# csmile-1006/ARP

Measured on AMD Instinct MI355X. Metric: frames/sec CLIP reward-labelled (256x256 ViT-B/32), higher is better.
Workload: dtype f16; 1 GPU; CLIP ViT-B/32 reward labelling, batch 1024 synthetic 256x256x3 uint8 frames per GPU resident in HBM (BASELINE.json configs[1]), random-init weights, text tower cached; parallelism=shard1 (no collective), streams_per_gpu=2

## Files before the change

arp_amd/_ffi.py:

```python
import ctypes as C
import os

_HERE = os.path.dirname(os.path.abspath(__file__))
LIB_PATH = os.path.join(_HERE, "libarp_hip.so")
if os.environ.get("ARP_LIB"):
    LIB_PATH = os.environ["ARP_LIB"] if os.path.isabs(os.environ["ARP_LIB"]) else os.path.join(os.path.dirname(_HERE), os.environ["ARP_LIB"])

MODE_F32, MODE_BF16, MODE_F16, MODE_F16X3, MODE_F16C = 0, 1, 2, 3, 4
ACT_NONE, ACT_QGELU, ACT_RELU, ACT_TANH, ACT_GELU_TANH = 0, 1, 2, 3, 4
ATTN_OUT_PLAIN, ATTN_OUT_E4M3, ATTN_OUT_F16C, ATTN_OUT_SPLIT3 = 0, 1, 2, 3
LN_OUT_F32, LN_OUT_BF16, LN_OUT_F16, LN_OUT_E4M3, LN_OUT_SPLIT3, LN_OUT_F16C, LN_OUT_F16C2 = 0, 1, 2, 3, 4, 5, 6
ASM_LNPRE, ASM_LAT_LN1, ASM_LAT_STATS = 0, 1, 2


class ArpError(RuntimeError):
    pass


class ClipCfg(C.Structure):
    _fields_ = [(n, C.c_int32) for n in (
        "patch", "width", "layers", "heads", "embed", "img_res", "txt_width", "txt_layers", "txt_heads", "ctx",
        "vocab", "mode", "device", "max_batch", "attn_impl", "n_streams")]


class DtCfg(C.Structure):
    _fields_ = [(n, C.c_int32) for n in (
        "emb", "depth", "heads", "mlp_ratio", "n_actions", "window", "enc_tokens", "enc_dim", "use_adapter", "mode",
        "device", "world", "rank")] + [(n, C.c_float) for n in ("lambda_ret", "weight_decay", "clip_norm", "b1", "b2", "eps")] + [("alibi_bias", C.c_int32), ("model", C.c_int32)]


DT_MODELS = {"ARPDT": 0, "BC": 1}


class FtCfg(C.Structure):
    _fields_ = [(n, C.c_int32) for n in ("layers", "width_v", "width_t", "embed", "hidden", "n_actions", "mode", "device", "use_vip", "use_id")] + [
        (n, C.c_float) for n in ("gamma", "logit_scale", "weight_decay", "b1", "b2", "eps")] + [("goal_conditioned", C.c_int32)]


class GemmSite(C.Structure):
    _fields_ = [("name", C.c_char_p)] + [(n, C.c_int32) for n in ("mode", "force", "M", "N", "K", "lda", "ldr", "ldo")] + [
        (n, C.c_void_p) for n in ("A", "W", "bias", "resid", "out", "ln_stats", "ln_c")] + [("ln_parts", C.c_int32), ("ln_eps", C.c_float)] + [
        ("xb_out", C.c_void_p), ("ldxb", C.c_int32), ("split3", C.c_int32), ("stats_out", C.c_void_p)] + [
        (n, C.c_int32) for n in ("plan", "sd", "sw")] + [("x4_out", C.c_void_p), ("dx4_out", C.c_void_p), ("ld4", C.c_int32)]


class EncCfg(C.Structure):
    _fields_ = [(n, C.c_int32) for n in ("patch", "width", "layers", "heads", "mlp_ratio", "img_res", "mode", "device", "max_frames",
                                          "attn_impl")]


os.environ.setdefault("GPU_MAX_HW_QUEUES", "8")


def _load():
    if not os.path.exists(LIB_PATH):
        raise ImportError(
            f"{LIB_PATH} is missing: the HIP extension is not built. Run `make -C arp_amd/csrc` "
            "(or `python -c 'import __graft_entry__ as g; g.build()'`). There is no CPU fallback.")
    return C.CDLL(LIB_PATH, mode=C.RTLD_GLOBAL)


lib = _load()

_vp, _i, _f = C.c_void_p, C.c_int, C.c_float
_fp = C.POINTER(C.c_float)
_u8p = C.POINTER(C.c_uint8)
_i32p = C.POINTER(C.c_int32)
_i64p = C.POINTER(C.c_int64)

SIGNATURES = {
    "arp_last_error": (C.c_char_p, []),
    "arp_version": (_i, []),
    "arp_debug_live": (_i, [_i64p]),
    "arp_device_count": (_i, []),
    "arp_dev_malloc": (_i, [C.POINTER(_vp), C.c_size_t]),
    "arp_dev_free": (_i, [_vp]),
    "arp_memcpy_h2d": (_i, [_vp, _vp, C.c_size_t]),
    "arp_memcpy_d2h": (_i, [_vp, _vp, C.c_size_t]),
    "arp_set_device": (_i, [_i]),
    "arp_dev_synchronize": (_i, []),
    "arp_host_register": (_i, [_vp, C.c_size_t]),
    "arp_host_unregister": (_i, [_vp]),
    "arp_clip_create": (_i, [C.POINTER(ClipCfg), C.POINTER(_vp)]),
    "arp_clip_destroy": (_i, [_vp]),
    "arp_clip_load_weight": (_i, [_vp, C.c_char_p, _fp, _i64p, _i]),
    "arp_clip_set_fp8_mlp": (_i, [_vp, _i]),
    "arp_clip_finalize_weights": (_i, [_vp]),
    "arp_clip_set_text": (_i, [_vp, _i32p, _i]),
    "arp_clip_get_text_features": (_i, [_vp, _fp]),
    "arp_clip_label": (_i, [_vp, _u8p, _i, _i, _i, _i, _fp]),
    "arp_clip_label_submit": (_i, [_vp, _i, _u8p, _i, _i, _i, _i]),
    "arp_clip_label_collect": (_i, [_vp, _i, _fp]),
    "arp_clip_label_dev_async": (_i, [_vp, _vp, _i, _i, _i, _i, _vp]),
    "arp_clip_sync": (_i, [_vp]),
    "arp_clip_set_streams": (_i, [_vp, _i]),
    "arp_clip_encode_image": (_i, [_vp, _u8p, _i, _i, _i, _i, _i, _fp]),
    "arp_preprocess": (_i, [_u8p, _i, _i, _i, _i, _i, _fp]),
    "arp_bicubic_coeffs": (_i, [_i, _i, _i32p, _i32p, _i32p, _i]),
    "arp_clip_clock_probe": (_i, [_vp, _i]),
    "arp_clip_clock_read": (_i, [_vp, C.POINTER(C.c_double)]),
    "arp_clip_profile_enable": (_i, [_vp, _i]),
    "arp_clip_profile_reset": (_i, [_vp]),
    "arp_clip_profile_json": (_i, [_vp, C.c_char_p, _i]),
    "arp_event_create": (_i, [C.POINTER(_vp)]),
    "arp_event_destroy": (_i, [_vp]),
    "arp_clip_event_record": (_i, [_vp, _vp]),
    "arp_event_elapsed_ms": (_i, [_vp, _vp, _fp]),
    "arp_dt_create": (_i, [C.POINTER(DtCfg), C.POINTER(_vp)]),
    "arp_dt_destroy": (_i, [_vp]),
    "arp_dt_num_params": (_i, [_vp, _i64p, _i32p]),
    "arp_dt_param_info": (_i, [_vp, _i, C.c_char_p, _i, _i64p, _i32p]),
    "arp_dt_set_tensor": (_i, [_vp, C.c_char_p, _i, _fp]),
    "arp_dt_get_tensor": (_i, [_vp, C.c_char_p, _i, _fp]),
    "arp_dt_set_step": (_i, [_vp, C.c_int64]),
    "arp_dt_get_step": (_i, [_vp, _i64p]),
    "arp_dt_set_batch": (_i, [_vp, _fp, _i32p, _fp, _i]),
    "arp_dt_forward": (_i, [_vp, _fp, _fp, _fp]),
    "arp_dt_backward": (_i, [_vp]),
    "arp_dt_train_step": (_i, [_vp, _f, _fp]),
    "arp_dt_train_step_async": (_i, [_vp, _f]),
    "arp_dt_val_step": (_i, [_vp, _fp]),
    "arp_dt_upload_batch_async": (_i, [_vp, _i, _fp, _i32p, _fp, _i]),
    "arp_dt_upload_batch_images_async": (_i, [_vp, _i, _fp, _i32p, _fp, _i]),
    "arp_dt_select_batch": (_i, [_vp, _i]),
    "arp_dt_bucket_plan": (_i, [C.POINTER(DtCfg), _i64p, _i64p]),
    "arp_dt_sync": (_i, [_vp]),
    "arp_dt_event_record": (_i, [_vp, _vp]),
    "arp_dt_comm_unique_id": (_i, [_vp]),
    "arp_dt_comm_init": (_i, [_vp, _vp, _i, _i]),
    "arp_dt_broadcast_state": (_i, [_vp]),
    "arp_dt_set_adapter_corrections": (_i, [_vp, _i]),
    "arp_dt_debug_read": (C.c_int64, [_vp, C.c_char_p, _vp, C.c_int64]),
    "arp_dt_comm_info": (_i, [_vp, _i32p]),
    "arp_dt_comm_selfcheck": (_i, [_vp, C.POINTER(C.c_double)]),
    "arp_dt_profile_enable": (_i, [_vp, _i]),
    "arp_dt_profile_reset": (_i, [_vp]),
    "arp_dt_profile_json": (_i, [_vp, C.c_char_p, _i]),
    "arp_clip_encode_image_multiscale": (_i, [_vp, _u8p, _i, _i, _i, _fp, _fp]),
    "arp_clip_encode_image_multiscale_pil": (_i, [_vp, _u8p, _i, _i, _i, _i, _fp, _fp]),
    "arp_clip_set_prompt_reduce": (_i, [_vp, _i]),
    "arp_clip_encode_text_multiscale": (_i, [_vp, _i32p, _i, _fp, _fp]),
    "arp_clip_encode_image_multiscale_dev": (_i, [_vp, _u8p, _i, _i, _i, _vp, _vp]),
    "arp_clip_encode_text_multiscale_dev": (_i, [_vp, _i32p, _i, _vp, _vp]),
    "arp_ft_set_batch_dev": (_i, [_vp, _vp, _vp, _vp, _vp, _fp, _i32p, _i]),
    "arp_ft_create": (_i, [C.POINTER(FtCfg), C.POINTER(_vp)]),
    "arp_ft_destroy": (_i, [_vp]),
    "arp_ft_num_params": (_i, [_vp, _i64p, _i32p]),
    "arp_ft_param_info": (_i, [_vp, _i, C.c_char_p, _i, _i64p, _i32p]),
    "arp_ft_set_tensor": (_i, [_vp, C.c_char_p, _i, _fp]),
    "arp_ft_get_tensor": (_i, [_vp, C.c_char_p, _i, _fp]),
    "arp_ft_set_step": (_i, [_vp, C.c_int64]),
    "arp_ft_get_step": (_i, [_vp, _i64p]),
    "arp_ft_dropped_gradients": (_i, [_vp, C.POINTER(C.c_uint64)]),
    "arp_ft_set_batch": (_i, [_vp, _fp, _fp, _fp, _fp, _fp, _i32p, _i]),
    "arp_ft_forward": (_i, [_vp, _fp, _fp, _fp]),
    "arp_ft_encode": (_i, [_vp, _i, _fp, _fp, _i, _fp]),
    "arp_ft_reward_set_text": (_i, [_vp, _vp, _i32p, _i]),
    "arp_ft_reward_set_reduce": (_i, [_vp, _i]),
    "arp_ft_reward_dev_async": (_i, [_vp, _vp, _vp, _i, _i, _i, _i, _i, _vp]),
    "arp_ft_reward": (_i, [_vp, _vp, _u8p, _i, _i, _i, _i, _i, _fp]),
    "arp_ft_reward_set_rows": (_i, [_vp, _i]),
    "arp_ft_reward_stats": (_i, [_vp, _i64p]),
    "arp_op_ft_rows_gemm": (_i, [_i, _i, _fp, _i, _fp, _i, _fp, _fp, _i, _i, _i, _i, _i, _i, _i]),
    "arp_op_ft_reward":(_i, [_fp, _fp, _f, _fp, _i, _i, _f, _fp, _i, _i]),
    "arp_ft_backward": (_i, [_vp]),
# ... 107 lines not shown
```

arp_amd/csrc/arp_clip.hip:

```cpp
#include <algorithm>
#include <cmath>
#include <cstdio>
#include <cstdlib>
#include <cstring>
#include <map>
#include <memory>
#include <string>
#include <vector>

#include "../../include/arp_hip.h"
#include "attention.h"
#include "enc_internal.h"
#include "common.h"
#include "gemm.h"
#include "gemm256.h"
#include "clip_internal.h"
#include "tower.h"
#include "preprocess.h"
#include "preprocess_host.h"
#include "rowops.h"
#include "runtime.h"

namespace arp {

static thread_local std::string g_err;
void set_error(const std::string& msg) { g_err = msg; }
int fail(const std::string& msg) {
    g_err = msg;
    return -1;
}

struct HostTensor {
    std::vector<float> data;
    std::vector<int64_t> shape;
};

}

using namespace arp;

struct ClipModel {
    arp_clip_cfg cfg;
    bool finalized = false;

    TowerW vis, txt;
    void* conv_w = nullptr;
    float *cls = nullptr, *pos = nullptr, *lnpre_w = nullptr, *lnpre_b = nullptr, *lnpost_w = nullptr, *lnpost_b = nullptr;
    void* proj_t = nullptr;
    float *tok_emb = nullptr, *tpos = nullptr, *lnf_w = nullptr, *lnf_b = nullptr;
    void* tproj_t = nullptr;
    TowerW txt32;
    void* tproj_t32 = nullptr;
    float* lut = nullptr;

    int gemm_force = 0;
    bool ln_fold = false;
    bool fp8_mlp = false;
    bool fp8_attn = false;
    bool qkv_fused = true;
    bool cls_only_last = true;
    bool lat_fold = true;
    bool skinny = true;
    int lat_rows = 1024;
    bool lat_graph = true;
    bool lat_pinned = true;

    int ntok() const { return (cfg.img_res / cfg.patch) * (cfg.img_res / cfg.patch) + 1; }
    size_t esz() const { return cfg.mode == ARP_MODE_F32 ? 4 : 2; }
};

struct arp_clip : ClipModel {
    Stream stream;
    std::map<std::string, HostTensor> staged;
    std::vector<DevBuf> owned;

    arp_clip* primary = nullptr;
    arp_clip* shared() { return primary ? primary : this; }
    float logit_scale = 0.f;
    DevBuf txt_feat;
    int n_prompts = 0;
    DevBuf txt_mean;
    int prompt_reduce = 0;
    DevBuf clock_buf;
    unsigned long long* clock_acc = nullptr;
    std::map<long long, std::unique_ptr<ResizePlan>> plans;

    DevBuf ms_keep;
    DevBuf ms_res, crop_buf;
    uint64_t res_gen = 0;

    int ws_frames = 0;
    DevBuf patches, pe, x, h, qkv, ao, fc, cls_h, feat, frames_in, rewards;
    Profiler prof;
    float* ms_out = nullptr;
    int ms_ld = 0;
    const int* ms_rows = nullptr;
    int pre_bilinear = 0;
    std::vector<std::unique_ptr<arp_clip>> siblings;
    Event ev_fork;
    std::vector<Event> ev_join;
    Stream copy_stream;
    std::vector<Event> ev_copy;
    struct LabelSlot {
        DevBuf frames, rewards;
        PinBuf host;
        Event done;
        int n = 0;
        bool busy = false;
    } lslot[2];
    bool shared_chip = false;
    DevBuf stats;
    DevBuf part;
    DevBuf lat_stats;
    bool lat_f0 = false;
    bool lat_h0 = false;
    bool lat_now = false;
    struct LatGraph {
        const uint8_t* frames;
        float* rewards;
        int n, H, W, crop;
        hipGraph_t graph;
        hipGraphExec_t exec;
    };
    std::vector<LatGraph> lat_graphs;
    PinBuf pin_frames, pin_rewards;

    arp_clip() = default;
    explicit arp_clip(const ClipModel& m) : ClipModel(m) {}
};
static_assert(!std::is_copy_constructible_v<arp_clip> && std::is_copy_constructible_v<ClipModel>);

namespace arp {

static TowerCtx ctx_of(arp_clip* c) {
    TowerCtx t;
    t.stream = c->stream;
    t.prof = &c->prof;
    t.attn_impl = c->cfg.attn_impl;
    t.gemm_force = c->gemm_force;
    t.qkv_fused = c->qkv_fused;
    t.shared_chip = c->shared_chip;
    t.clock_acc = c->shared()->clock_acc;
    t.fp8_mlp = c->fp8_mlp; t.fp8_attn = c->fp8_attn;
    t.ms_out = c->ms_out; t.ms_ld = c->ms_ld; t.ms_rows = c->ms_rows;
    t.skinny = c->lat_now; t.h_ready0 = c->lat_now && c->lat_h0; t.lat_stats = c->lat_stats.as<float>(); t.lat_fold0 = c->lat_now && c->lat_f0; t.part = c->part.as<float>(); t.part_floats = c->part.bytes / 4;
    return t;
}

static int upload_f32(arp_clip* c, const std::vector<float>& v, float** out) {
    return upload_owned(c->owned, v.data(), v.size() * 4, std::max<size_t>(v.size() * 4, 16), reinterpret_cast<void**>(out));
}

static int upload_mat(arp_clip* c, const float* src, int rows, int cols, bool transpose, void** out, int wmode = -1) {
    const int mode = wmode >= 0 ? wmode : c->cfg.mode;
    const size_t esz = mode == ARP_MODE_F32 ? 4 : 2;
    const size_t n = (size_t)rows * cols;
    std::vector<float> tmp;
    const float* s = src;
    if (transpose) {
        tmp.resize(n);
        for (int r = 0; r < rows; ++r)
            for (int q = 0; q < cols; ++q) tmp[(size_t)q * rows + r] = src[(size_t)r * cols + q];
        s = tmp.data();
    }
    const size_t alloc = std::max<size_t>(n * esz, 16);
    if (mode == ARP_MODE_BF16) {
        std::vector<bf16_t> hb(n);
        for (size_t i = 0; i < n; ++i) hb[i] = host_f2bf(s[i]);
        return upload_owned(c->owned, hb.data(), n * 2, alloc, out);
    }
    if (mode == ARP_MODE_F16) {
        std::vector<f16_t> hb(n);
        for (size_t i = 0; i < n; ++i) hb[i] = host_f2h(s[i]);
        return upload_owned(c->owned, hb.data(), n * 2, alloc, out);
    }
    return upload_owned(c->owned, s, n * 4, alloc, out);
}

static int get_staged(arp_clip* c, const std::string& name, std::vector<int64_t> shape, const HostTensor** out) {
    auto it = c->staged.find(name);
    if (it == c->staged.end()) return fail("missing weight: " + name);
    if (it->second.shape != shape) {
        std::string s = "weight " + name + " has shape [";
        for (auto d : it->second.shape) s += std::to_string(d) + ",";
        s += "], expected [";
        for (auto d : shape) s += std::to_string(d) + ",";
        return fail(s + "]");
    }
    *out = &it->second;
    return 0;
}

static int load_tower(arp_clip* c, const std::string& prefix, int d, int layers, int heads, TowerW& tw, bool fold, int wmode = -1, int ntok = 0) {
    tw.width = d; tw.layers = layers; tw.heads = heads;
    const int emode = wmode >= 0 ? wmode : c->cfg.mode;
    const bool hm = c->qkv_fused && ntok > 0 && qkv_attn_supported(ntok, d, heads, emode == ARP_MODE_F32 ? 4 : 2);
    tw.L.resize(layers);
    for (int i = 0; i < layers; ++i) {
        const std::string p = prefix + "resblocks." + std::to_string(i) + ".";
        LayerW& L = tw.L[i];
        const HostTensor* t;
        ARP_TRY(get_staged(c, p + "ln_1.weight", {d}, &t)); ARP_TRY(upload_f32(c, t->data, &L.ln1_w));
        ARP_TRY(get_staged(c, p + "ln_1.bias", {d}, &t)); ARP_TRY(upload_f32(c, t->data, &L.ln1_b));
        ARP_TRY(get_staged(c, p + "ln_2.weight", {d}, &t)); ARP_TRY(upload_f32(c, t->data, &L.ln2_w));
        ARP_TRY(get_staged(c, p + "ln_2.bias", {d}, &t)); ARP_TRY(upload_f32(c, t->data, &L.ln2_b));
        ARP_TRY(get_staged(c, p + "attn.in_proj_weight", {3 * d, d}, &t)); ARP_TRY(upload_mat(c, t->data.data(), 3 * d, d, false, &L.w_in, wmode));
        ARP_TRY(get_staged(c, p + "attn.in_proj_bias", {3 * d}, &t)); ARP_TRY(upload_f32(c, t->data, &L.b_in));
        if (hm) {
            const HostTensor *w, *b;
            ARP_TRY(get_staged(c, p + "attn.in_proj_weight", {3 * d, d}, &w)); ARP_TRY(get_staged(c, p + "attn.in_proj_bias", {3 * d}, &b));
            std::vector<float> wp((size_t)3 * d * d), bp((size_t)3 * d);
            qkv_head_major(w->data.data(), b->data.data(), d, heads, wp.data(), bp.data());
            ARP_TRY(upload_mat(c, wp.data(), 3 * d, d, false, &L.w_in_hm, wmode)); ARP_TRY(upload_f32(c, bp, &L.b_in_hm));
        }
        ARP_TRY(get_staged(c, p + "attn.out_proj.weight", {d, d}, &t)); ARP_TRY(upload_mat(c, t->data.data(), d, d, false, &L.w_out, wmode));
        ARP_TRY(get_staged(c, p + "attn.out_proj.bias", {d}, &t)); ARP_TRY(upload_f32(c, t->data, &L.b_out));
        ARP_TRY(get_staged(c, p + "mlp.c_fc.weight", {4 * d, d}, &t)); ARP_TRY(upload_mat(c, t->data.data(), 4 * d, d, false, &L.w_fc, wmode));
        ARP_TRY(get_staged(c, p + "mlp.c_fc.bias", {4 * d}, &t)); ARP_TRY(upload_f32(c, t->data, &L.b_fc));
        ARP_TRY(get_staged(c, p + "mlp.c_proj.weight", {d, 4 * d}, &t)); ARP_TRY(upload_mat(c, t->data.data(), d, 4 * d, false, &L.w_proj, wmode));
        ARP_TRY(get_staged(c, p + "mlp.c_proj.bias", {d}, &t)); ARP_TRY(upload_f32(c, t->data, &L.b_proj));
        if (c->fp8_mlp && ntok > 0 && emode != ARP_MODE_F32 && d % 128 == 0) {
            auto put8 = [&](const std::vector<float>& w, void** out, float* scale) -> int {
                float mx = 0.f;
                for (float v : w) mx = std::max(mx, fabsf(v));
                const float sc = mx > 0.f ? exp2f(floorf(log2f(240.f / mx))) : 1.f;
                std::vector<fp8_t> q(w.size());
                for (size_t i = 0; i < w.size(); ++i) q[i] = host_f2fp8(w[i] * sc);
                *scale = sc;
                return upload_owned(c->owned, q.data(), q.size(), q.size(), out);
            };
            const HostTensor *w1, *w2, *lw, *lb;
            float s1 = 1.f, s2 = 1.f;
            ARP_TRY(get_staged(c, p + "mlp.c_fc.weight", {4 * d, d}, &w1)); ARP_TRY(put8(w1->data, &L.w_fc8, &s1));
            ARP_TRY(get_staged(c, p + "mlp.c_proj.weight", {d, 4 * d}, &w2)); ARP_TRY(put8(w2->data, &L.w_proj8, &s2));
            L.a_fc = 1.0f / (FP8_S_H * s1);
            L.a_proj = 1.0f / (FP8_S_G * s2);
            ARP_TRY(get_staged(c, p + "ln_2.weight", {d}, &lw)); ARP_TRY(get_staged(c, p + "ln_2.bias", {d}, &lb));
            std::vector<float> g8(lw->data), b8(lb->data);
            for (auto& v : g8) v *= FP8_S_H;
            for (auto& v : b8) v *= FP8_S_H;
            ARP_TRY(upload_f32(c, g8, &L.ln2_w8)); ARP_TRY(upload_f32(c, b8, &L.ln2_b8));
            if (c->fp8_attn) {
                const HostTensor *wi, *wo;
                float si = 1.f, so = 1.f;
                ARP_TRY(get_staged(c, p + "attn.in_proj_weight", {3 * d, d}, &wi)); ARP_TRY(put8(wi->data, &L.w_in8, &si));
                ARP_TRY(get_staged(c, p + "attn.out_proj.weight", {d, d}, &wo)); ARP_TRY(put8(wo->data, &L.w_out8, &so));
                L.a_in = 1.0f / (FP8_S_H * si);
                L.a_out = 1.0f / (FP8_S_A * so);
                ARP_TRY(get_staged(c, p + "ln_1.weight", {d}, &lw)); ARP_TRY(get_staged(c, p + "ln_1.bias", {d}, &lb));
                std::vector<float> g1(lw->data), b1(lb->data);
                for (auto& v : g1) v *= FP8_S_H;
                for (auto& v : b1) v *= FP8_S_H;
                ARP_TRY(upload_f32(c, g1, &L.ln1_w8)); ARP_TRY(upload_f32(c, b1, &L.ln1_b8));
            }
        }
        if (fold) {
            const HostTensor *w, *b, *lw, *lb;
            std::vector<bf16_t> wf;
            std::vector<float> cc, dd;
            auto put = [&](const std::vector<bf16_t>& m, void** out) -> int {
                return upload_owned(c->owned, m.data(), m.size() * 2, m.size() * 2, out);
            };
            ARP_TRY(get_staged(c, p + "attn.in_proj_weight", {3 * d, d}, &w)); ARP_TRY(get_staged(c, p + "attn.in_proj_bias", {3 * d}, &b));
            ARP_TRY(get_staged(c, p + "ln_1.weight", {d}, &lw)); ARP_TRY(get_staged(c, p + "ln_1.bias", {d}, &lb));
            fold_layernorm(w->data.data(), lw->data.data(), lb->data.data(), b->data.data(), 3 * d, d, wf, cc, dd, emode == ARP_MODE_F16);
            ARP_TRY(put(wf, &L.w_in_f)); ARP_TRY(upload_f32(c, cc, &L.c_in)); ARP_TRY(upload_f32(c, dd, &L.d_in));
            ARP_TRY(get_staged(c, p + "mlp.c_fc.weight", {4 * d, d}, &w)); ARP_TRY(get_staged(c, p + "mlp.c_fc.bias", {4 * d}, &b));
            ARP_TRY(get_staged(c, p + "ln_2.weight", {d}, &lw)); ARP_TRY(get_staged(c, p + "ln_2.bias", {d}, &lb));
            fold_layernorm(w->data.data(), lw->data.data(), lb->data.data(), b->data.data(), 4 * d, d, wf, cc, dd, emode == ARP_MODE_F16);
            ARP_TRY(put(wf, &L.w_fc_f)); ARP_TRY(upload_f32(c, cc, &L.c_fc)); ARP_TRY(upload_f32(c, dd, &L.d_fc));
        }
    }
    tw.folded = fold;
    if (!fold && ntok > 0 && c->lat_fold && c->skinny && emode != ARP_MODE_F32 && (d & 15) == 0) {
        for (int i = 0; i < layers; ++i) {
            LayerW& L = tw.L[i];
            const std::string p = prefix + "resblocks." + std::to_string(i) + ".";
            const HostTensor *w, *b, *lw, *lb;
            std::vector<bf16_t> wf;
            std::vector<float> cc, dd;
            auto put = [&](const std::vector<bf16_t>& m, void** out) -> int {
                return upload_owned(c->owned, m.data(), m.size() * 2, m.size() * 2, out);
            };
            const bool half = emode == ARP_MODE_F16;
            ARP_TRY(get_staged(c, p + "attn.in_proj_weight", {3 * d, d}, &w)); ARP_TRY(get_staged(c, p + "attn.in_proj_bias", {3 * d}, &b));
            ARP_TRY(get_staged(c, p + "ln_1.weight", {d}, &lw)); ARP_TRY(get_staged(c, p + "ln_1.bias", {d}, &lb));
            fold_layernorm(w->data.data(), lw->data.data(), lb->data.data(), b->data.data(), 3 * d, d, wf, cc, dd, half);
            ARP_TRY(put(wf, &L.w_in_f)); ARP_TRY(upload_f32(c, cc, &L.c_in)); ARP_TRY(upload_f32(c, dd, &L.d_in));
            ARP_TRY(get_staged(c, p + "mlp.c_fc.weight", {4 * d, d}, &w)); ARP_TRY(get_staged(c, p + "mlp.c_fc.bias", {4 * d}, &b));
            ARP_TRY(get_staged(c, p + "ln_2.weight", {d}, &lw)); ARP_TRY(get_staged(c, p + "ln_2.bias", {d}, &lb));
            fold_layernorm(w->data.data(), lw->data.data(), lb->data.data(), b->data.data(), 4 * d, d, wf, cc, dd, half);
            ARP_TRY(put(wf, &L.w_fc_f)); ARP_TRY(upload_f32(c, cc, &L.c_fc)); ARP_TRY(upload_f32(c, dd, &L.d_fc));
        }
        tw.lat_folded = true;
    }
    return 0;
}

template <typename T, typename OutT, int ACT, bool RESID, int SITE>
static int gemm(arp_clip* c, const char* site, const void* A, const void* W, const float* bias, const float* resid, void* out,
                int M, int N, int K) {
    TowerCtx t = ctx_of(c);
    return tower_gemm<T, OutT, ACT, RESID, SITE>(t, site, A, W, bias, resid, out, M, N, K);
}
template <typename OutT>
static int layernorm(arp_clip* c, const char* site, const float* in, size_t in_stride, OutT* out, int out_stride,
                     const float* w, const float* b, int rows, int D, float eps) {
    TowerCtx t = ctx_of(c);
    return tower_layernorm<OutT>(t, site, in, in_stride, out, out_stride, w, b, rows, D, eps);
}
template <typename T>
static int run_blocks(arp_clip* c, const TowerW& tw, const char* tag, float* x, T* h, T* qkv, T* ao, T* fc, int B, int N,
                      int causal, float* stats = nullptr) {
    TowerCtx t = ctx_of(c);
    t.cls_only_last = (&tw == &c->vis) && c->cls_only_last && !(t.ms_out && t.ms_rows);
    return run_blocks<T, ACT_QGELU, 0>(t, tw, tag, x, h, qkv, ao, fc, B, N, causal, 1e-5f, stats);
}


static void drop_lat_graphs(arp_clip* c) {
    for (auto& g : c->lat_graphs) {
        (void)hipGraphExecDestroy(g.exec);
        (void)hipGraphDestroy(g.graph);
    }
    c->lat_graphs.clear();
}

static int ensure_workspace(arp_clip* c, int frames) {
    if (frames <= c->ws_frames) return 0;
    if (!c->lat_graphs.empty()) {
        ARP_HIP_OK(hipStreamSynchronize(c->stream));
        drop_lat_graphs(c);
    }
    const arp_clip_cfg& k = c->cfg;
    const size_t e = c->esz();
    const int G = k.img_res / k.patch, N = c->ntok(), D = k.width;
    const size_t B = frames, M = B * N;
    ARP_TRY(c->patches.ensure(B * G * G * 3 * k.patch * k.patch * e));
    ARP_TRY(c->pe.ensure(B * G * G * D * 4));
    ARP_TRY(c->x.ensure(M * D * 4));
    ARP_TRY(c->h.ensure(M * D * e));
    ARP_TRY(c->qkv.ensure(M * 3 * D * e));
    ARP_TRY(c->ao.ensure(M * D * e));
    ARP_TRY(c->fc.ensure(M * 4 * D * e));
    ARP_TRY(c->cls_h.ensure(B * D * e));
    ARP_TRY(c->feat.ensure(B * k.embed * 4));
    ARP_TRY(c->stats.ensure(M * (size_t)std::max(D >> 7, 1) * 8));
    c->ws_frames = frames;
    c->res_gen += 1;
    return 0;
}

static int get_plan(arp_clip* c, int H, int W, int use_crop, ResizePlan** out, bool small = false) {
    const long long key = ((long long)H << 32) | ((long long)W << 2) | (small ? 2 : 0) | (use_crop ? 1 : 0);
    auto it = c->plans.find(key);
    if (it != c->plans.end()) {
        *out = it->second.get();
        return 0;
    }
    auto p = std::make_unique<ResizePlan>();
    ARP_TRY(build_plan(H, W, use_crop, c->cfg.img_res, *p, small ? 8 : 32));
    *out = p.get();
    c->plans[key] = std::move(p);
    return 0;
}

template <typename T>
static int forward_chunk(arp_clip* c, const uint8_t* frames_dev, int nb, ResizePlan* plan) {
    const arp_clip_cfg& k = c->cfg;
    const int G = k.img_res / k.patch, N = c->ntok(), D = k.width, KP = 3 * k.patch * k.patch;
    c->lat_now = c->skinny && sizeof(T) == 2 && (long)nb * N <= c->lat_rows;
    struct LatGuard {
        arp_clip* c;
        ~LatGuard() { c->lat_now = false; c->lat_h0 = false; c->lat_f0 = false; }
    } lat_guard{c};
    if (c->pre_bilinear) {
        ProfScope ps(c->prof, c->stream, "preprocess_bilinear");
        const int H = c->pre_bilinear >> 16, W = c->pre_bilinear & 0xffff, R = k.img_res;
        const size_t total = (size_t)nb * 3 * R * (R / 4);
        hipLaunchKernelGGL((preprocess_bilinear_kernel<T>), dim3((unsigned)((total + 255) / 256)), dim3(256), 0, c->stream, frames_dev, c->patches.as<T>(), nb,
                           H, W, R, k.patch, (H != R && W != R) ? 1 : 0);
        ARP_HIP_OK(hipGetLastError());
    } else {
        ProfScope ps(c->prof, c->stream, "preprocess");
        ARP_TRY((launch_preprocess<T, PRE_PATCH>(*plan, frames_dev, nb, k.patch, c->lut, c->patches.p, c->stream)));
    }
    c->lat_h0 = false;
    c->lat_f0 = false;
    bool assembled = false;
    if constexpr (sizeof(T) == 2) {
        const int Mp = nb * G * G, S = c->lat_now ? tower_split_of(Mp, D, KP) : 0;
        if (S && (size_t)S * Mp * D * 4 <= c->part.bytes && c->vis.layers > 0 && D % 4 == 0 && D <= ROW_MAX_V4 * 256) {
            const int tcode = __is_same(T, bf16_t) ? 1 : 2;
            SkinnyArgs q;
            q.A = c->patches.p; q.W = c->conv_w; q.out = c->part.p; q.M = Mp; q.N = D; q.K = KP; q.lda = KP; q.ldw = KP; q.ldo = D; q.out_f32 = 1;
            q.ksplit = S; q.slice_stride = (size_t)Mp * D;
            {
                ProfScope ps(c->prof, c->stream, "vit.patch_embed");
                ARP_TRY(launch_skinny_gemm(tcode, q, c->stream));
            }
            ProfScope ps(c->prof, c->stream, "vit.assemble_ln_pre_ln_1");
            const bool f0 = c->vis.lat_folded && c->lat_stats.p && (D & 15) == 0;
            ARP_TRY(launch_vit_assemble_lat<T>(c->stream, c->part.as<float>(), S, (size_t)Mp * D, c->cls, c->pos, c->lnpre_w, c->lnpre_b, c->x.as<float>(),
                                               c->h.as<T>(), c->vis.L[0].ln1_w, c->vis.L[0].ln1_b, nb * N, N, D, 1e-5f,
                                               f0 ? c->lat_stats.as<float>() : nullptr, D >> 4));
            assembled = true;
            c->lat_h0 = !f0;
            c->lat_f0 = f0;
        }
    }
    if (!assembled) {
    ARP_TRY((gemm<T, float, ACT_NONE, false, SITE_PATCH>(c, "vit.patch_embed", c->patches.p, c->conv_w, nullptr, nullptr, c->pe.p,
                                                         nb * G * G, D, KP)));
    {
        ProfScope ps(c->prof, c->stream, "vit.assemble_ln_pre");
        ARP_TRY(launch_vit_assemble_lnpre(c->stream, c->pe.as<float>(), c->cls, c->pos, c->lnpre_w, c->lnpre_b, c->x.as<float>(), nb * N, N, D, 1e-5f));
    }
    }
    ARP_TRY(run_blocks<T>(c, c->vis, "vit", c->x.as<float>(), c->h.as<T>(), c->qkv.as<T>(), c->ao.as<T>(), c->fc.as<T>(), nb, N, 0, c->stats.as<float>()));
    ARP_TRY(layernorm<T>(c, "vit.ln_post", c->x.as<float>(), (size_t)N * D, c->cls_h.as<T>(), D, c->lnpost_w, c->lnpost_b, nb, D, 1e-5f));
    ARP_TRY((gemm<T, float, ACT_NONE, false, SITE_PROJ>(c, "vit.proj", c->cls_h.p, c->proj_t, nullptr, nullptr, c->feat.p, nb, k.embed, D)));
    return 0;
}

static int forward_chunk_dispatch(arp_clip* c, const uint8_t* frames_dev, int nb, ResizePlan* plan) {
    if (c->cfg.mode == ARP_MODE_BF16) return forward_chunk<bf16_t>(c, frames_dev, nb, plan);
    if (c->cfg.mode == ARP_MODE_F16) return forward_chunk<f16_t>(c, frames_dev, nb, plan);
    return forward_chunk<float>(c, frames_dev, nb, plan);
}

template <typename T> static int run_text(arp_clip* c, const int32_t* tokens, int np, float* out_host = nullptr, bool normalize = true,
                                          float* ms_host = nullptr, bool dev_out = false, bool w32 = false) {
    const TowerW& txt = w32 ? c->txt32 : c->txt;
    const void* tproj = w32 ? c->tproj_t32 : c->tproj_t;
    const arp_clip_cfg& k = c->cfg;
    const int Tw = k.txt_width, ctx = k.ctx, M = np * ctx;
    const size_t e = sizeof(T);
    DevBuf tok, eot, x, h, qkv, ao, fc, hs, ms, feat_tmp;
    DevBuf& feat = out_host ? feat_tmp : c->txt_feat;
    std::vector<int> eot_rows(np);
    for (int p = 0; p < np; ++p) {
        int best = 0;
        for (int t = 1; t < ctx; ++t)
            if (tokens[p * ctx + t] > tokens[p * ctx + best]) best = t;
        eot_rows[p] = p * ctx + best;
        for (int t = 0; t < ctx; ++t)
            if (tokens[p * ctx + t] < 0 || tokens[p * ctx + t] >= k.vocab) return fail("set_text: token id out of range");
    }
    ARP_TRY(tok.ensure((size_t)M * 4)); ARP_TRY(eot.ensure((size_t)np * 4));
    ARP_TRY(x.ensure((size_t)M * Tw * 4)); ARP_TRY(h.ensure((size_t)M * Tw * e)); ARP_TRY(qkv.ensure((size_t)M * 3 * Tw * e));
    ARP_TRY(ao.ensure((size_t)M * Tw * e)); ARP_TRY(fc.ensure((size_t)M * 4 * Tw * e)); ARP_TRY(hs.ensure((size_t)np * Tw * e));
    ARP_TRY(feat.ensure((size_t)np * k.embed * 4));
    if (ms_host) ARP_TRY(ms.ensure((size_t)np * c->txt.layers * Tw * 4));
    ARP_HIP_OK(hipMemcpyAsync(tok.p, tokens, (size_t)M * 4, hipMemcpyHostToDevice, c->stream));
    ARP_HIP_OK(hipMemcpyAsync(eot.p, eot_rows.data(), (size_t)np * 4, hipMemcpyHostToDevice, c->stream));
    ARP_TRY(launch_text_embed(c->stream, tok.as<int>(), c->tok_emb, c->tpos, x.as<float>(), M, ctx, Tw));
    if (ms_host) { c->ms_out = ms.as<float>(); c->ms_ld = c->txt.layers * Tw; c->ms_rows = eot.as<int>(); }
    const int rb = run_blocks<T>(c, txt, "text", x.as<float>(), h.as<T>(), qkv.as<T>(), ao.as<T>(), fc.as<T>(), np, ctx, 1);
    c->ms_out = nullptr; c->ms_rows = nullptr;
    ARP_TRY(rb);
    ARP_TRY(launch_layernorm_gather<T>(c->stream, x.as<float>(), (size_t)Tw, eot.as<int>(), hs.as<T>(), Tw, c->lnf_w, c->lnf_b, np, Tw, 1e-5f));
    ARP_TRY((gemm<T, float, ACT_NONE, false, SITE_PROJ>(c, "text.proj", hs.p, tproj, nullptr, nullptr, feat.p, np,
                                                        k.embed, Tw)));
    if (normalize) {
        ARP_TRY(launch_l2_normalize(c->stream, feat.as<float>(), np, k.embed));
    }
    const hipMemcpyKind okind = dev_out ? hipMemcpyDeviceToDevice : hipMemcpyDeviceToHost;
    if (out_host) ARP_HIP_OK(hipMemcpyAsync(out_host, feat.p, (size_t)np * k.embed * 4, okind, c->stream));
    if (ms_host) ARP_HIP_OK(hipMemcpyAsync(ms_host, ms.p, (size_t)np * c->txt.layers * Tw * 4, okind, c->stream));
    ARP_HIP_OK(hipStreamSynchronize(c->stream));
    if (!out_host) c->n_prompts = np;
    return 0;
}

static int check_ready(arp_clip* c, bool need_text) {
    if (!c) return fail("null handle");
    if (!c->finalized) return fail("weights not finalized: call arp_clip_finalize_weights first");
    if (need_text && c->n_prompts <= 0) return fail("no prompt set: call arp_clip_set_text first");
    return 0;
}

static int label_dev_single(arp_clip* c, const uint8_t* frames_dev, int n, int H, int W, int use_crop, float* rewards_dev) {
    arp_clip* o = c->shared();
    ARP_TRY(check_ready(o, true));
    if (n < 0) return fail("negative frame count");
    if (n == 0) return 0;
    ARP_HIP_OK(hipSetDevice(c->cfg.device));
    ResizePlan* plan;
    const int mb = c->cfg.max_batch;
    const bool small = !c->primary && n <= mb && (long)n * c->ntok() <= c->lat_rows;
    ARP_TRY(get_plan(o, H, W, use_crop, &plan, small));
    ARP_TRY(ensure_workspace(c, std::min(n, mb)));
    const float scale = expf(o->logit_scale);
    auto pass = [&](const uint8_t* fr, int nb, float* rw) -> int {
        ARP_TRY(forward_chunk_dispatch(c, fr, nb, plan));
        ProfScope ps(c->prof, c->stream, "reward");
        return launch_reward(c->stream, c->feat.as<float>(), o->prompt_reduce ? o->txt_mean.as<float>() : o->txt_feat.as<float>(), scale, rw, nb, c->cfg.embed);
    };
    if (c->lat_graph && small && !c->prof.on && !c->ms_out && !c->pre_bilinear) {
        for (auto& g : c->lat_graphs)
            if (g.frames == frames_dev && g.rewards == rewards_dev && g.n == n && g.H == H && g.W == W && g.crop == ((use_crop ? 1 : 0) | (c->prompt_reduce << 1))) {
                ARP_HIP_OK(hipGraphLaunch(g.exec, c->stream));
                return 0;
            }
        arp_clip::LatGraph g{frames_dev, rewards_dev, n, H, W, (use_crop ? 1 : 0) | (c->prompt_reduce << 1), nullptr, nullptr};
        ARP_HIP_OK(hipStreamBeginCapture(c->stream, hipStreamCaptureModeRelaxed));
        const int rc = pass(frames_dev, n, rewards_dev);
        const hipError_t ec = hipStreamEndCapture(c->stream, &g.graph);
        if (rc != 0 || ec != hipSuccess || !g.graph || hipGraphInstantiate(&g.exec, g.graph, nullptr, nullptr, 0) != hipSuccess) {
            if (g.graph) (void)hipGraphDestroy(g.graph);
            for (int k = 0; k < 4 && hipGetLastError() != hipSuccess; ++k) {}
            c->lat_graph = false;
            return pass(frames_dev, n, rewards_dev);
        }
        if (c->lat_graphs.size() >= 8) {
            (void)hipGraphExecDestroy(c->lat_graphs.front().exec);
            (void)hipGraphDestroy(c->lat_graphs.front().graph);
            c->lat_graphs.erase(c->lat_graphs.begin());
        }
        c->lat_graphs.push_back(g);
        ARP_HIP_OK(hipGraphLaunch(g.exec, c->stream));
        return 0;
    }
    for (int off = 0; off < n; off += mb) {
        const int nb = std::min(mb, n - off);
        ARP_TRY(pass(frames_dev + (size_t)off * H * W * 3, nb, rewards_dev + off));
    }
    return 0;
}

static int make_sibling(arp_clip* c) {
    auto s = std::make_unique<arp_clip>(static_cast<const ClipModel&>(*c));
    s->primary = c;
    s->prof.on = c->prof.on;
    ARP_TRY(s->stream.create());
    if (!c->ev_fork) ARP_TRY(c->ev_fork.create());
    Event ej;
    ARP_TRY(ej.create());
    c->ev_join.push_back(std::move(ej));
    c->siblings.push_back(std::move(s));
    return 0;
}

static int label_dev(arp_clip* c, const uint8_t* frames_dev, int n, int H, int W, int use_crop, float* rewards_dev, const uint8_t* host_src = nullptr,
                     int lead = 0) {
    ARP_TRY(check_ready(c, true));
    int ns = c->cfg.n_streams;
    while (ns > 1 && n / ns < 128) --ns;
    const size_t fbytes = (size_t)H * W * 3;
    if (ns < 2) {
        if (host_src) ARP_HIP_OK(hipMemcpyAsync(const_cast<uint8_t*>(frames_dev), host_src, (size_t)n * fbytes, hipMemcpyHostToDevice, c->stream));
        return label_dev_single(c, frames_dev, n, H, W, use_crop, rewards_dev);
    }
    ARP_HIP_OK(hipSetDevice(c->cfg.device));
    int parts = ns;
    if (host_src) {
        static const int env_parts = getenv("ARP_CLIP_HOST_PARTS") ? atoi(getenv("ARP_CLIP_HOST_PARTS")) : 0;
        parts = env_parts > 0 ? env_parts : ns;
        while (parts > ns && n / parts < 128) --parts;
        if (parts < ns) parts = ns;
        if (!c->copy_stream) ARP_TRY(c->copy_stream.create());
        while ((int)c->ev_copy.size() < parts + 1) {
            Event e;
            ARP_TRY(e.create());
            c->ev_copy.push_back(std::move(e));
        }
    }
    while ((int)c->siblings.size() < ns - 1) ARP_TRY(make_sibling(c));
    ResizePlan* plan;
    ARP_TRY(get_plan(c, H, W, use_crop, &plan));
    ARP_HIP_OK(hipEventRecord(c->ev_fork, c->stream));
    for (int i = 1; i < ns; ++i) ARP_HIP_OK(hipStreamWaitEvent(c->siblings[i - 1]->stream, c->ev_fork, 0));
    if (!host_src || lead <= 0 || n < 8 * lead) lead = 0;
    const int per = (n - lead + parts - 1) / parts;
// ... 45 lines not shown
}

static int ms_finetune_geometry(const arp_clip* c, int H, int W, int use_crop, int* h, int* w, int* y0, int* x0) {
    const int R = c->cfg.img_res;
    *h = H; *w = W; *y0 = 0; *x0 = 0;
    if (use_crop) {
        const int cs = W / 2;
        if (cs <= 0 || cs > H) return fail("use_crop: the centre crop of side W / 2 does not fit the frame");
        *h = *w = cs;
        *y0 = (int)((H - cs) / 2); *x0 = (int)((W - cs) / 2);
    }
    if ((*h != R) != (*w != R)) return fail("the reference resizes only when BOTH sides differ from 224 (clip_multiscale_adapter.py:127): "
                                            "a frame with exactly one side at 224 cannot enter the tower");
    return 0;
}

int clip_ms_prepare(arp_clip* c, int nb, int H, int W, int use_crop, int transform, uint64_t* generation, int* capturable) {
    ARP_TRY(check_ready(c, false));
    if (c->primary) return fail("a part stream's sibling is not a handle of its own");
    if (nb <= 0 || nb > c->cfg.max_batch) return fail("clip_ms_prepare: 1 .. max_batch frames per pass");
    if (H <= 0 || W <= 0 || H > 0xffff || W > 0xffff) return fail("bad frame geometry");
    if (transform != CLIP_TF_FINETUNE && transform != CLIP_TF_LABEL) return fail("transform is 0 (fine-tune: bilinear) or 1 (label: Pillow bicubic)");
    ARP_HIP_OK(hipSetDevice(c->cfg.device));
    const bool small = (long)nb * c->ntok() <= c->lat_rows;
    size_t crop_bytes = 0;
    if (transform == CLIP_TF_LABEL) {
        ResizePlan* plan;
        ARP_TRY(get_plan(c, H, W, use_crop, &plan, small));
    } else {
        int h, w, y0, x0;
        ARP_TRY(ms_finetune_geometry(c, H, W, use_crop, &h, &w, &y0, &x0));
        if (use_crop) crop_bytes = (size_t)nb * h * w * 3;
    }
    const size_t ms_bytes = (size_t)nb * c->vis.layers * c->cfg.width * 4;
    if (ms_bytes > c->ms_res.bytes || crop_bytes > c->crop_buf.bytes) {
        ARP_HIP_OK(hipStreamSynchronize(c->stream));
        ARP_TRY(c->ms_res.ensure(ms_bytes));
        ARP_TRY(c->crop_buf.ensure(crop_bytes));
        c->res_gen += 1;
    }
    ARP_TRY(ensure_workspace(c, nb));
    *generation = c->res_gen;
    *capturable = c->lat_graph && small && !c->prof.on ? 1 : 0;
    return 0;
}

int clip_ms_enqueue(arp_clip* c, const uint8_t* frames_dev, int nb, int H, int W, int use_crop, int transform, const float** inter, const float** final_feat) {
    if (!c || !frames_dev || !inter || !final_feat) return fail("null argument");
    if (nb <= 0 || nb > c->ws_frames || (size_t)nb * c->vis.layers * c->cfg.width * 4 > c->ms_res.bytes) return fail("clip_ms_enqueue: call clip_ms_prepare first");
    ResizePlan* plan = nullptr;
    const uint8_t* src = frames_dev;
    int pre = 0;
    if (transform == CLIP_TF_LABEL) {
        ARP_TRY(get_plan(c, H, W, use_crop, &plan, (long)nb * c->ntok() <= c->lat_rows));
    } else {
        int h, w, y0, x0;
        ARP_TRY(ms_finetune_geometry(c, H, W, use_crop, &h, &w, &y0, &x0));
        if (use_crop) {
            const size_t total = (size_t)nb * h * w * 3;
            if (total > c->crop_buf.bytes) return fail("clip_ms_enqueue: call clip_ms_prepare first");
            ProfScope ps(c->prof, c->stream, "crop");
            hipLaunchKernelGGL(crop_u8_kernel, dim3((unsigned)std::min<size_t>((total + 255) / 256, 4096)), dim3(256), 0, c->stream, frames_dev,
                               c->crop_buf.as<uint8_t>(), nb, H, W, y0, x0, h);
            ARP_HIP_OK(hipGetLastError());
            src = c->crop_buf.as<uint8_t>();
        }
        pre = (h << 16) | w;
    }
    c->ms_out = c->ms_res.as<float>(); c->ms_ld = c->vis.layers * c->cfg.width; c->ms_rows = nullptr; c->pre_bilinear = pre;
    const int r = forward_chunk_dispatch(c, src, nb, plan);
    c->ms_out = nullptr; c->pre_bilinear = 0;
    ARP_TRY(r);
    *inter = c->ms_res.as<float>();
    *final_feat = c->feat.as<float>();
    return 0;
}

}

extern "C" {

const char* arp_last_error(void) { return g_err.c_str(); }
int arp_version(void) { return 100; }

int arp_debug_live(int64_t out5[5]) {
    if (!out5) return fail("null out");
    out5[0] = live.dev_bytes; out5[1] = live.dev_bufs; out5[2] = live.streams; out5[3] = live.events; out5[4] = live.pin_bytes;
    return 0;
}

int arp_device_count(void) {
    int n = 0;
    if (hipGetDeviceCount(&n) != hipSuccess) return 0;
    return n;
}

int arp_dev_malloc(void** out, size_t bytes) {
    if (!out) return fail("null out");
    ARP_HIP_OK(hipMalloc(out, bytes ? bytes : 16));
    return 0;
}
int arp_dev_free(void* p) {
    if (p) ARP_HIP_OK(hipFree(p));
    return 0;
}
int arp_memcpy_h2d(void* dst, const void* src, size_t bytes) {
    ARP_HIP_OK(hipMemcpy(dst, src, bytes, hipMemcpyHostToDevice));
    return 0;
}
int arp_memcpy_d2h(void* dst, const void* src, size_t bytes) {
    ARP_HIP_OK(hipMemcpy(dst, src, bytes, hipMemcpyDeviceToHost));
    return 0;
}
int arp_host_register(void* p, size_t bytes) {
    if (!p || !bytes) return fail("bad argument");
    ARP_HIP_OK(hipHostRegister(p, bytes, hipHostRegisterDefault));
    return 0;
}
int arp_host_unregister(void* p) {
    if (!p) return 0;
    ARP_HIP_OK(hipHostUnregister(p));
    return 0;
}
int arp_set_device(int device) {
    ARP_HIP_OK(hipSetDevice(device));
    return 0;
}
int arp_dev_synchronize(void) {
    ARP_HIP_OK(hipDeviceSynchronize());
    return 0;
}

int arp_clip_create(const arp_clip_cfg* cfg, arp_clip** out) {
    if (!cfg || !out) return fail("null argument");
    const arp_clip_cfg& k = *cfg;
    if (k.mode != ARP_MODE_F32 && k.mode != ARP_MODE_BF16 && k.mode != ARP_MODE_F16) return fail("bad mode");
    if (k.patch <= 0 || k.img_res % k.patch || k.patch % 4 || k.img_res % 4) return fail("bad patch / img_res");
    if (k.width % k.heads || k.txt_width % k.txt_heads) return fail("width not divisible by heads");
    const int kq = (k.mode == ARP_MODE_F32) ? 32 : 64;
    if (k.width % kq || k.txt_width % kq || (3 * k.patch * k.patch) % kq)
        return fail("width / txt_width / 3*patch^2 must be multiples of " + std::to_string(kq));
    if (k.embed % 4) return fail("embed must be a multiple of 4");
    int ndev = 0;
    ARP_HIP_OK(hipGetDeviceCount(&ndev));
    if (k.device < 0 || k.device >= ndev) return fail("no such HIP device: " + std::to_string(k.device));
    ARP_HIP_OK(hipSetDevice(k.device));
    ARP_TRY(prime_runtime(k.device));
    arp_clip* c = new arp_clip();
    c->cfg = k;
    if (c->cfg.max_batch <= 0) c->cfg.max_batch = 1024;
    if (const char* e = getenv("ARP_GEMM")) c->gemm_force = atoi(e);
    if (const char* e = getenv("ARP_LN_FOLD")) c->ln_fold = atoi(e) != 0;
    if (const char* e = getenv("ARP_CLS_ONLY")) c->cls_only_last = atoi(e) != 0;
    if (const char* e = getenv("ARP_QKV_FUSED")) c->qkv_fused = atoi(e) != 0;
    if (const char* e = getenv("ARP_SKINNY")) c->skinny = atoi(e) != 0;
    if (const char* e = getenv("ARP_LAT_FOLD")) c->lat_fold = atoi(e) != 0;
    if (const char* e = getenv("ARP_CLIP_GRAPH")) c->lat_graph = atoi(e) != 0;
    if (const char* e = getenv("ARP_SKINNY_ROWS")) c->lat_rows = std::min(std::max(atoi(e), 1), SKINNY_MAX_M);
    if (const char* e = getenv("ARP_CLIP_PINNED")) c->lat_pinned = atoi(e) != 0;
    if (c->stream.create() != 0) {
        delete c;
        return fail("hipStreamCreate failed");
    }
    *out = c;
    return 0;
}

int arp_clip_destroy(arp_clip* c) {
    if (!c) return 0;
    (void)hipSetDevice(c->cfg.device);
    (void)hipStreamSynchronize(c->stream);
    for (auto& s : c->siblings) (void)hipStreamSynchronize(s->stream);
    drop_lat_graphs(c);
    delete c;
    return 0;
}

int arp_clip_load_weight(arp_clip* c, const char* name, const float* data, const int64_t* shape, int ndim) {
    if (!c || !name || !data || (ndim > 0 && !shape)) return fail("null argument");
    if (c->finalized) return fail("weights already finalized");
    HostTensor t;
    size_t n = 1;
    for (int i = 0; i < ndim; ++i) {
        if (shape[i] < 0) return fail("negative dimension");
        t.shape.push_back(shape[i]);
        n *= (size_t)shape[i];
    }
    t.data.assign(data, data + n);
    c->staged[name] = std::move(t);
    return 0;
}

int arp_clip_finalize_weights(arp_clip* c) {
    if (!c) return fail("null handle");
    if (c->finalized) return 0;
    ARP_HIP_OK(hipSetDevice(c->cfg.device));
    const arp_clip_cfg& k = c->cfg;
    const int D = k.width, P = k.patch, E = k.embed, Tw = k.txt_width, N = c->ntok();
    const HostTensor* t;
    ARP_TRY(get_staged(c, "visual.conv1.weight", {D, 3, P, P}, &t)); ARP_TRY(upload_mat(c, t->data.data(), D, 3 * P * P, false, &c->conv_w));
    ARP_TRY(get_staged(c, "visual.class_embedding", {D}, &t)); ARP_TRY(upload_f32(c, t->data, &c->cls));
    ARP_TRY(get_staged(c, "visual.positional_embedding", {N, D}, &t)); ARP_TRY(upload_f32(c, t->data, &c->pos));
    ARP_TRY(get_staged(c, "visual.ln_pre.weight", {D}, &t)); ARP_TRY(upload_f32(c, t->data, &c->lnpre_w));
    ARP_TRY(get_staged(c, "visual.ln_pre.bias", {D}, &t)); ARP_TRY(upload_f32(c, t->data, &c->lnpre_b));
    ARP_TRY(get_staged(c, "visual.ln_post.weight", {D}, &t)); ARP_TRY(upload_f32(c, t->data, &c->lnpost_w));
    ARP_TRY(get_staged(c, "visual.ln_post.bias", {D}, &t)); ARP_TRY(upload_f32(c, t->data, &c->lnpost_b));
    ARP_TRY(get_staged(c, "visual.proj", {D, E}, &t)); ARP_TRY(upload_mat(c, t->data.data(), D, E, true, &c->proj_t));
    ARP_TRY(load_tower(c, "visual.transformer.", D, k.layers, k.heads, c->vis, c->ln_fold && (k.mode == ARP_MODE_BF16 || k.mode == ARP_MODE_F16) && (D & 127) == 0, -1, c->ntok()));
    ARP_TRY(get_staged(c, "token_embedding.weight", {k.vocab, Tw}, &t)); ARP_TRY(upload_f32(c, t->data, &c->tok_emb));
    ARP_TRY(get_staged(c, "positional_embedding", {k.ctx, Tw}, &t)); ARP_TRY(upload_f32(c, t->data, &c->tpos));
    ARP_TRY(get_staged(c, "ln_final.weight", {Tw}, &t)); ARP_TRY(upload_f32(c, t->data, &c->lnf_w));
    ARP_TRY(get_staged(c, "ln_final.bias", {Tw}, &t)); ARP_TRY(upload_f32(c, t->data, &c->lnf_b));
    ARP_TRY(get_staged(c, "text_projection", {Tw, E}, &t)); ARP_TRY(upload_mat(c, t->data.data(), Tw, E, true, &c->tproj_t));
    ARP_TRY(load_tower(c, "transformer.", Tw, k.txt_layers, k.txt_heads, c->txt, false));
    if (k.mode != ARP_MODE_F32) {
        ARP_TRY(get_staged(c, "text_projection", {Tw, E}, &t)); ARP_TRY(upload_mat(c, t->data.data(), Tw, E, true, &c->tproj_t32, ARP_MODE_F32));
        ARP_TRY(load_tower(c, "transformer.", Tw, k.txt_layers, k.txt_heads, c->txt32, false, ARP_MODE_F32));
    }
    if (c->staged.count("logit_scale") && c->staged["logit_scale"].shape == std::vector<int64_t>{1}) c->staged["logit_scale"].shape.clear();
    ARP_TRY(get_staged(c, "logit_scale", {}, &t));
    c->logit_scale = t->data[0];
    std::vector<float> lut(768);
    build_lut(lut.data());
    ARP_TRY(upload_f32(c, lut, &c->lut));
    ARP_TRY(c->part.ensure((size_t)4 * SKINNY_MAX_M * std::max(D, Tw) * 4));
    ARP_TRY(c->lat_stats.ensure((size_t)SKINNY_MAX_M * std::max(D >> 4, 1) * 8));
    c->staged.clear();
    c->finalized = true;
    return 0;
}

static __global__ __launch_bounds__(256) void prompt_mean_kernel(const float* __restrict__ txt, float* __restrict__ out, int np, int E) {
    const int c = blockIdx.x * 256 + threadIdx.x;
    if (c >= E) return;
    float s = 0.f;
    for (int p = 0; p < np; ++p) s += txt[(size_t)p * E + c];
    out[c] = s / (float)np;
}

int arp_clip_set_text(arp_clip* c, const int32_t* tokens, int n_prompts) {
    ARP_TRY(check_ready(c, false));
    if (!tokens || n_prompts <= 0) return fail("set_text: need at least one prompt");
    ARP_HIP_OK(hipSetDevice(c->cfg.device));
    if (!c->lat_graphs.empty()) {
        ARP_HIP_OK(hipStreamSynchronize(c->stream));
        drop_lat_graphs(c);
    }
    if (c->cfg.mode != ARP_MODE_F32) ARP_TRY(run_text<float>(c, tokens, n_prompts, nullptr, true, nullptr, false, true));
    else ARP_TRY(run_text<float>(c, tokens, n_prompts));
    ARP_TRY(c->txt_mean.ensure((size_t)c->cfg.embed * 4));
    hipLaunchKernelGGL(prompt_mean_kernel, dim3((c->cfg.embed + 255) / 256), dim3(256), 0, c->stream, c->txt_feat.as<float>(), c->txt_mean.as<float>(),
                       n_prompts, c->cfg.embed);
    ARP_HIP_OK(hipGetLastError());
    ARP_HIP_OK(hipStreamSynchronize(c->stream));
    return 0;
}

int arp_clip_set_prompt_reduce(arp_clip* c, int mode) {
    ARP_TRY(check_ready(c, false));
    if (mode != 0 && mode != 1) return fail("set_prompt_reduce: mode is 0 (prompt 0) or 1 (mean over the prompts)");
    c->prompt_reduce = mode;
    return 0;
}

int arp_clip_get_text_features(arp_clip* c, float* out) {
    ARP_TRY(check_ready(c, true));
    if (!out) return fail("null out");
    ARP_HIP_OK(hipMemcpy(out, c->txt_feat.p, (size_t)c->n_prompts * c->cfg.embed * 4, hipMemcpyDeviceToHost));
    return 0;
}

int arp_clip_label_dev_async(arp_clip* c, const uint8_t* frames_dev, int n, int H, int W, int use_crop, float* rewards_dev) {
    if (n > 0 && (!frames_dev || !rewards_dev)) return fail("null buffer");
    return label_dev(c, frames_dev, n, H, W, use_crop, rewards_dev);
}

int arp_clip_sync(arp_clip* c) {
    if (!c) return fail("null handle");
    ARP_HIP_OK(hipStreamSynchronize(c->stream));
    return 0;
}

int arp_clip_label(arp_clip* c, const uint8_t* frames, int n, int H, int W, int use_crop, float* rewards) {
    ARP_TRY(check_ready(c, true));
    if (n < 0) return fail("negative frame count");
    if (n == 0) return 0;
    if (!frames || !rewards) return fail("null buffer");
    ARP_HIP_OK(hipSetDevice(c->cfg.device));
    const size_t fb = (size_t)H * W * 3;
    const int mb = c->cfg.max_batch;
    if (c->lat_pinned && n <= mb && (long)n * c->ntok() <= c->lat_rows) {
        if (c->pin_frames.bytes < (size_t)n * fb) {
            ARP_HIP_OK(hipStreamSynchronize(c->stream));
            ARP_TRY(c->pin_frames.ensure((size_t)n * fb));
        }
        if (c->pin_rewards.bytes < (size_t)n * 4) {
            ARP_HIP_OK(hipStreamSynchronize(c->stream));
            ARP_TRY(c->pin_rewards.ensure((size_t)std::max(n, 16) * 4));
        }
        memcpy(c->pin_frames.p, frames, (size_t)n * fb);
        ARP_TRY(label_dev_single(c, c->pin_frames.as<uint8_t>(), n, H, W, use_crop, c->pin_rewards.as<float>()));
        ARP_HIP_OK(hipStreamSynchronize(c->stream));
        memcpy(rewards, c->pin_rewards.p, (size_t)n * 4);
        return 0;
    }
    ARP_TRY(c->frames_in.ensure((size_t)std::min(n, mb) * fb));
// ... 228 lines not shown
    }
    const std::string s = c->prof.json();
    if ((int)s.size() + 1 > buf_len) return fail("profile buffer too small");
    memcpy(buf, s.c_str(), s.size() + 1);
    return (int)s.size();
}

int arp_event_create(arp_event** out) {
    if (!out) return fail("null out");
    arp_event* ev = new arp_event();
    if (hipEventCreate(&ev->e) != hipSuccess) {
        delete ev;
        return fail("hipEventCreate failed");
    }
    *out = ev;
    return 0;
}
int arp_event_destroy(arp_event* e) {
    if (e) {
        (void)hipEventDestroy(e->e);
        delete e;
    }
    return 0;
}
int arp_clip_event_record(arp_clip* c, arp_event* e) {
    if (!c || !e) return fail("null argument");
    ARP_HIP_OK(hipEventRecord(e->e, c->stream));
    return 0;
}
int arp_event_elapsed_ms(arp_event* a, arp_event* b, float* ms) {
    if (!a || !b || !ms) return fail("null argument");
    ARP_HIP_OK(hipEventSynchronize(b->e));
    ARP_HIP_OK(hipEventElapsedTime(ms, a->e, b->e));
    return 0;
}

}

template <typename T> static int to_dev(const float* src, size_t n, DevBuf& d) {
    ARP_TRY(d.ensure(std::max<size_t>(n * sizeof(T), 16)));
    if constexpr (std::is_same_v<T, f16_t>) {
        std::vector<f16_t> hb(n);
        for (size_t i = 0; i < n; ++i) hb[i] = host_f2h(src[i]);
        ARP_HIP_OK(hipMemcpy(d.p, hb.data(), n * 2, hipMemcpyHostToDevice));
    } else if constexpr (sizeof(T) == 2) {
        std::vector<bf16_t> hb(n);
        for (size_t i = 0; i < n; ++i) hb[i] = host_f2bf(src[i]);
        ARP_HIP_OK(hipMemcpy(d.p, hb.data(), n * 2, hipMemcpyHostToDevice));
    } else {
        ARP_HIP_OK(hipMemcpy(d.p, src, n * 4, hipMemcpyHostToDevice));
    }
    return 0;
}
template <typename T> static int from_dev(float* dst, size_t n, const DevBuf& d) {
    if constexpr (std::is_same_v<T, f16_t>) {
        std::vector<uint16_t> hb(n);
        ARP_HIP_OK(hipMemcpy(hb.data(), d.p, n * 2, hipMemcpyDeviceToHost));
        for (size_t i = 0; i < n; ++i) dst[i] = (float)__builtin_bit_cast(_Float16, hb[i]);
    } else if constexpr (sizeof(T) == 2) {
        std::vector<bf16_t> hb(n);
        ARP_HIP_OK(hipMemcpy(hb.data(), d.p, n * 2, hipMemcpyDeviceToHost));
        for (size_t i = 0; i < n; ++i) {
            const uint32_t u = (uint32_t)hb[i] << 16;
            memcpy(&dst[i], &u, 4);
        }
    } else {
        ARP_HIP_OK(hipMemcpy(dst, d.p, n * 4, hipMemcpyDeviceToHost));
    }
    return 0;
}

template <typename T> static int op_gemm(int act, const float* A, const float* W, const float* bias, const float* resid, float* out,
                                         int M, int N, int K) {
    DevBuf dA, dW, dB, dR, dO;
    ARP_TRY(to_dev<T>(A, (size_t)M * K, dA)); ARP_TRY(to_dev<T>(W, (size_t)N * K, dW));
    if (bias) ARP_TRY(to_dev<float>(bias, N, dB));
    ARP_TRY(dO.ensure((size_t)M * N * 4));
    if (resid) ARP_TRY(to_dev<float>(resid, (size_t)M * N, dR));
    GemmArgs g;
    g.A = dA.p; g.W = dW.p; g.bias = bias ? dB.as<float>() : nullptr; g.resid = resid ? dR.as<float>() : nullptr; g.out = dO.p;
    g.M = M; g.N = N; g.K = K; g.lda = K; g.ldw = K; g.ldr = N; g.ldo = N;
    int rc = -1;
    const char* fe = getenv("ARP_GEMM");
    const int force = fe ? atoi(fe) : 0;
#define ARP_OP_CASE(a)                                                                                            \
case a: rc = resid ? launch_gemm_auto<T, float, a, true, SITE_OP>(g, nullptr, force) : launch_gemm_auto<T, float, a, false, SITE_OP>(g, nullptr, force); break;
    switch (act) {
        ARP_OP_CASE(ACT_NONE) ARP_OP_CASE(ACT_QGELU) ARP_OP_CASE(ACT_RELU) ARP_OP_CASE(ACT_TANH) ARP_OP_CASE(ACT_GELU_TANH)
        default: return fail("bad activation");
    }
#undef ARP_OP_CASE
    ARP_TRY(rc);
    ARP_HIP_OK(hipDeviceSynchronize());
    return from_dev<float>(out, (size_t)M * N, dO);
}

template <typename T> static int op_skinny(int act, const float* A, const float* W, const float* bias, const float* resid, float* out, int M, int N, int K,
                                           int ksplit, const float* ln_w, const float* ln_b, float eps, float* h_out) {
    DevBuf dA, dW, dB, dR, dO, dP, dH, dLw, dLb;
    const int tcode = __is_same(T, bf16_t) ? 1 : 2;
    ARP_TRY(to_dev<T>(A, (size_t)M * K, dA)); ARP_TRY(to_dev<T>(W, (size_t)N * K, dW));
    if (bias) ARP_TRY(to_dev<float>(bias, N, dB));
    SkinnyArgs k;
    k.A = dA.p; k.W = dW.p; k.M = M; k.N = N; k.K = K; k.lda = K; k.ldw = K; k.ldr = N; k.ldo = N; k.out_f32 = 1;
    if (ksplit == 0) {
        ARP_TRY(dO.ensure((size_t)M * N * 4));
        if (resid) ARP_TRY(to_dev<float>(resid, (size_t)M * N, dR));
        k.bias = bias ? dB.as<float>() : nullptr; k.resid = resid ? dR.as<float>() : nullptr; k.out = dO.p; k.act = act;
        ARP_TRY(launch_skinny_gemm(tcode, k, nullptr));
        ARP_HIP_OK(hipDeviceSynchronize());
        return from_dev<float>(out, (size_t)M * N, dO);
    }
    if (!resid || act != ACT_NONE) return fail("skinny split: needs the residual, takes no activation");
    ARP_TRY(to_dev<float>(resid, (size_t)M * N, dR));
    ARP_TRY(dP.ensure((size_t)ksplit * M * N * 4));
    if (ln_w) {
        if (!ln_b || !h_out) return fail("skinny split: ln_w needs ln_b and h_out");
        ARP_TRY(to_dev<float>(ln_w, N, dLw)); ARP_TRY(to_dev<float>(ln_b, N, dLb)); ARP_TRY(dH.ensure((size_t)M * N * sizeof(T)));
    }
    k.out = dP.p; k.ksplit = ksplit; k.slice_stride = (size_t)M * N;
    ARP_TRY(launch_skinny_gemm(tcode, k, nullptr));
    ARP_TRY(launch_skinny_reduce_ln(tcode, dP.as<float>(), ksplit, (size_t)M * N, bias ? dB.as<float>() : nullptr, dR.as<float>(), N, dH.p, N,
                                    ln_w ? dLw.as<float>() : nullptr, ln_w ? dLb.as<float>() : nullptr, M, N, eps, nullptr));
    ARP_HIP_OK(hipDeviceSynchronize());
    ARP_TRY(from_dev<float>(out, (size_t)M * N, dR));
    if (ln_w) ARP_TRY(from_dev<T>(h_out, (size_t)M * N, dH));
    return 0;
}

extern "C" {

int arp_op_skinny_gemm(int mode, int act, const float* A, const float* W, const float* bias, const float* resid, float* out, int M, int N, int K, int ksplit,
                       const float* ln_w, const float* ln_b, float eps, float* h_out) {
    if (!A || !W || !out || M <= 0 || N <= 0 || K <= 0 || ksplit < 0) return fail("bad argument");
    if (mode == ARP_MODE_BF16) return op_skinny<bf16_t>(act, A, W, bias, resid, out, M, N, K, ksplit, ln_w, ln_b, eps, h_out);
    if (mode == ARP_MODE_F16) return op_skinny<f16_t>(act, A, W, bias, resid, out, M, N, K, ksplit, ln_w, ln_b, eps, h_out);
    return fail("skinny gemm: 16-bit modes only");
}

int arp_op_gemm_nt(int mode, int act, const float* A, const float* W, const float* bias, const float* resid, float* out, int M, int N,
                   int K) {
    if (!A || !W || !out || M <= 0 || N <= 0 || K <= 0) return fail("bad argument");
    if (mode == ARP_MODE_F16) return op_gemm<f16_t>(act, A, W, bias, resid, out, M, N, K);
    return mode == ARP_MODE_BF16 ? op_gemm<bf16_t>(act, A, W, bias, resid, out, M, N, K) : op_gemm<float>(act, A, W, bias, resid, out, M, N, K);
}

}

template <typename T> static int op_gemm_site_vit(const arp_gemm_site& d, const std::string& s) {
    if (s == "vit.qkv") return tower_gemm_site<T, T, ACT_NONE, false, SITE_QKV>(d);
    if (s == "vit.c_fc") return tower_gemm_site<T, T, ACT_QGELU, false, SITE_FC1>(d);
    if (s == "vit.out_proj") return tower_gemm_site<T, float, ACT_NONE, true, SITE_OUT>(d);
    if (s == "vit.c_proj") return tower_gemm_site<T, float, ACT_NONE, true, SITE_FC2>(d);
    return fail("gemm_site: unknown instance " + s);
}

extern "C" {

int arp_op_gemm_site(const arp_gemm_site* d) {
    if (!d || !d->name || !d->A || !d->W || d->M <= 0 || d->N <= 0 || d->K <= 0) return fail("bad argument");
    const std::string s(d->name);
    int rc;
    if (s.rfind("m3ae.", 0) == 0) rc = enc_op_gemm_site(*d);
    else if (d->mode == ARP_MODE_F16) rc = op_gemm_site_vit<f16_t>(*d, s);
    else if (d->mode == ARP_MODE_BF16) rc = op_gemm_site_vit<bf16_t>(*d, s);
    else return fail("gemm_site: 16-bit modes only");
    ARP_TRY(rc);
    ARP_HIP_OK(hipDeviceSynchronize());
    return 0;
}

}

static float host_fp82f(uint8_t b) {
    const int sign = b >> 7, e = (b >> 3) & 15, m = b & 7;
    float v;
    if (e == 15 && m == 7) v = NAN;
    else if (e == 0) v = ldexpf((float)m, -9);
    else v = ldexpf(1.0f + m / 8.0f, e - 7);
    return sign ? -v : v;
}

extern "C" {

int arp_op_gemm_fp8(int act, const float* A, const float* W, const float* bias, const float* resid, float* out, int M, int N, int K, float alpha,
                    int out_fp8, float out_scale) {
    if (!A || !W || !out || M <= 0 || N <= 0 || K <= 0 || K % 128 || N % 16) return fail("bad argument (K % 128, N % 16)");
    if (out_fp8 && resid) return fail("fp8 output has no residual epilogue");
    DevBuf dA, dW, dB, dR, dO;
    std::vector<fp8_t> qa((size_t)M * K), qw((size_t)N * K);
    for (size_t i = 0; i < qa.size(); ++i) qa[i] = host_f2fp8(A[i]);
    for (size_t i = 0; i < qw.size(); ++i) qw[i] = host_f2fp8(W[i]);
    ARP_TRY(dA.ensure(qa.size())); ARP_TRY(dW.ensure(qw.size()));
    ARP_HIP_OK(hipMemcpy(dA.p, qa.data(), qa.size(), hipMemcpyHostToDevice));
    ARP_HIP_OK(hipMemcpy(dW.p, qw.data(), qw.size(), hipMemcpyHostToDevice));
    if (bias) ARP_TRY(to_dev<float>(bias, N, dB));
    if (resid) ARP_TRY(to_dev<float>(resid, (size_t)M * N, dR));
    ARP_TRY(dO.ensure((size_t)M * N * 4));
    GemmArgs g;
    g.A = dA.p; g.W = dW.p; g.bias = bias ? dB.as<float>() : nullptr; g.resid = resid ? dR.as<float>() : nullptr; g.out = dO.p;
    g.M = M; g.N = N; g.K = K; g.lda = K; g.ldw = K; g.ldr = N; g.ldo = N; g.alpha = alpha; g.out_scale = out_scale;
    int rc;
    if (out_fp8 == 2) {
        if (act != ACT_NONE || resid) return fail("f16 output: no activation, no residual");
        rc = launch_gemm256_nt<fp8_t, f16_t, ACT_NONE, false, SITE_OP>(g, nullptr);
        ARP_TRY(rc);
        ARP_HIP_OK(hipDeviceSynchronize());
        return from_dev<f16_t>(out, (size_t)M * N, dO);
    }
    if (out_fp8) rc = act == ACT_QGELU ? launch_gemm256_nt<fp8_t, fp8_t, ACT_QGELU, false, SITE_OP>(g, nullptr) : launch_gemm256_nt<fp8_t, fp8_t, ACT_NONE, false, SITE_OP>(g, nullptr);
    else if (act != ACT_NONE) return fail("f32 output: act must be ACT_NONE");
    else rc = resid ? launch_gemm256_nt<fp8_t, float, ACT_NONE, true, SITE_OP>(g, nullptr) : launch_gemm256_nt<fp8_t, float, ACT_NONE, false, SITE_OP>(g, nullptr);
    ARP_TRY(rc);
    ARP_HIP_OK(hipDeviceSynchronize());
    if (out_fp8) {
        std::vector<uint8_t> hb((size_t)M * N);
        ARP_HIP_OK(hipMemcpy(hb.data(), dO.p, hb.size(), hipMemcpyDeviceToHost));
        for (size_t i = 0; i < hb.size(); ++i) out[i] = host_fp82f(hb[i]);
        return 0;
    }
    return from_dev<float>(out, (size_t)M * N, dO);
}

}

template <typename T> static int op_gemm_bench(int kernel, int act, int resid, int out_f32, int M, int N, int K, int iters, float* avg_ms) {
    DevBuf dA, dW, dB, dR, dO;
    Event e0, e1;
    std::vector<float> hA((size_t)M * K), hW((size_t)N * K), hb(N);
    uint32_t s = 12345u;
    auto rnd = [&]() { s = s * 1664525u + 1013904223u; return ((s >> 8) & 0xffff) / 32768.0f - 1.0f; };
    for (auto& v : hA) v = rnd();
    for (auto& v : hW) v = rnd() * 0.05f;
    for (auto& v : hb) v = rnd();
    ARP_TRY(to_dev<T>(hA.data(), hA.size(), dA)); ARP_TRY(to_dev<T>(hW.data(), hW.size(), dW)); ARP_TRY(to_dev<float>(hb.data(), N, dB));
    ARP_TRY(dO.ensure((size_t)M * N * 4)); ARP_TRY(dR.ensure((size_t)M * N * 4));
    ARP_HIP_OK(hipMemset(dR.p, 0, (size_t)M * N * 4));
    GemmArgs g;
    g.A = dA.p; g.W = dW.p; g.bias = dB.as<float>(); g.resid = resid ? dR.as<float>() : nullptr; g.out = resid ? dR.p : dO.p;
    g.M = M; g.N = N; g.K = K; g.lda = K; g.ldw = K; g.ldr = N; g.ldo = N;
    if (const char* fe = getenv("ARP_GEMM_GROUP_M")) g.group_m = atoi(fe);
    auto run = [&]() -> int {
        if (resid) return launch_gemm_auto<T, float, ACT_NONE, true, SITE_OP>(g, nullptr, kernel);
        if (out_f32) return launch_gemm_auto<T, float, ACT_NONE, false, SITE_OP>(g, nullptr, kernel);
        if (act == ACT_QGELU) return launch_gemm_auto<T, T, ACT_QGELU, false, SITE_OP>(g, nullptr, kernel);
        return launch_gemm_auto<T, T, ACT_NONE, false, SITE_OP>(g, nullptr, kernel);
    };
    ARP_TRY(e0.create(hipEventDefault)); ARP_TRY(e1.create(hipEventDefault));
    for (int i = 0; i < 3; ++i) ARP_TRY(run());
    ARP_HIP_OK(hipEventRecord(e0, nullptr));
    for (int i = 0; i < iters; ++i) ARP_TRY(run());
    ARP_HIP_OK(hipEventRecord(e1, nullptr));
    ARP_HIP_OK(hipEventSynchronize(e1));
    float ms = 0.f;
    ARP_HIP_OK(hipEventElapsedTime(&ms, e0, e1));
    *avg_ms = ms / iters;
    return 0;
}

extern "C" {

int arp_op_gemm_bench(int mode, int kernel, int act, int resid, int out_f32, int M, int N, int K, int iters, float* avg_ms) {
    if (!avg_ms || M <= 0 || N <= 0 || K <= 0 || iters <= 0) return fail("bad argument");
    if (mode == ARP_MODE_F16) return op_gemm_bench<f16_t>(kernel, act, resid, out_f32, M, N, K, iters, avg_ms);
    return mode == ARP_MODE_BF16 ? op_gemm_bench<bf16_t>(kernel, act, resid, out_f32, M, N, K, iters, avg_ms)
                                 : op_gemm_bench<float>(kernel, act, resid, out_f32, M, N, K, iters, avg_ms);
}

int arp_op_layernorm(const float* x, const float* w, const float* b, float* out, int rows, int D, float eps) {
    if (!x || !w || !b || !out || rows <= 0 || D <= 0) return fail("bad argument");
    if (D % 4 || D > ROW_MAX_V4 * 256) return fail("layernorm: unsupported width");
    DevBuf dx, dw, db, dout;
    ARP_TRY(to_dev<float>(x, (size_t)rows * D, dx)); ARP_TRY(to_dev<float>(w, D, dw)); ARP_TRY(to_dev<float>(b, D, db));
    ARP_TRY(dout.ensure((size_t)rows * D * 4));
#define ARP_LN_CALL(NV)                                                                                                  \
hipLaunchKernelGGL((layernorm_kernel<float, NV>), dim3((rows + 3) / 4), dim3(256), 0, nullptr, dx.as<float>(), (size_t)D, \
                   dout.as<float>(), D, dw.as<float>(), db.as<float>(), rows, D, eps)
    ARP_NV_DISPATCH(D, ARP_LN_CALL);
#undef ARP_LN_CALL
    ARP_HIP_OK(hipGetLastError());
    ARP_HIP_OK(hipDeviceSynchronize());
    return from_dev<float>(out, (size_t)rows * D, dout);
}

}

template <typename T> static int op_attn(int impl, const float* qkv, float* out, int B, int N, int D, int heads, int causal) {
    DevBuf dq, dout;
    ARP_TRY(to_dev<T>(qkv, (size_t)B * N * 3 * D, dq));
    ARP_TRY(dout.ensure((size_t)B * N * D * sizeof(T)));
    ARP_TRY(launch_attention<T>(nullptr, impl, dq.as<T>(), dout.as<T>(), B, N, D, heads, causal));
    ARP_HIP_OK(hipDeviceSynchronize());
    return from_dev<T>(out, (size_t)B * N * D, dout);
}

extern "C" {

int arp_op_attention(int mode, int impl, const float* qkv, float* out, int B, int N, int D, int heads, int causal) {
    if (!qkv || !out || B <= 0 || N <= 0 || D <= 0 || heads <= 0 || D % heads) return fail("bad argument");
    if (mode == ARP_MODE_F16) return op_attn<f16_t>(impl, qkv, out, B, N, D, heads, causal);
    return mode == ARP_MODE_BF16 ? op_attn<bf16_t>(impl, qkv, out, B, N, D, heads, causal)
                                 : op_attn<float>(impl, qkv, out, B, N, D, heads, causal);
}

}

// ... 39 lines not shown
    DevBuf dA, dW, dB, dout;
    std::vector<float> wp((size_t)3 * D * K), bp((size_t)3 * D);
    qkv_head_major(W, bias, K, heads, wp.data(), bp.data());
    ARP_TRY(to_dev<T>(A, rows * K, dA)); ARP_TRY(to_dev<T>(wp.data(), wp.size(), dW)); ARP_TRY(to_dev<float>(bp.data(), bp.size(), dB));
    ARP_TRY(dout.ensure(std::max<size_t>(out_bytes, 16)));
    ARP_HIP_OK(hipMemcpy(dout.p, out, out_bytes, hipMemcpyHostToDevice));
    QkvAttnArgs q;
    q.A = dA.p; q.W = dW.p; q.bias = dB.as<float>(); q.out = dout.p;
    q.B = B; q.N = N; q.K = K; q.heads = heads; q.lda = K; q.ldw = K; q.ldo = D; q.fpt = 0; q.nq = nq; q.causal = causal; q.scale = 0.f;
    const int rc = launch_qkv_attn<T>(q, nullptr);
    ARP_HIP_OK(hipDeviceSynchronize());
    ARP_HIP_OK(hipMemcpy(out, dout.p, out_bytes, hipMemcpyDeviceToHost));
    return rc;
}

extern "C" {

int arp_op_attention_forms(int mode, int impl, const float* qkv, void* out, size_t out_bytes, int B, int N, int D, int heads, int causal, int nq, int form,
                           float out_scale, int outc) {
    if (!qkv || !out || B <= 0 || N <= 0 || D <= 0 || heads <= 0 || D % heads) return fail("bad argument");
    uint8_t* o = static_cast<uint8_t*>(out);
    if (mode == ARP_MODE_F16) return op_attn_forms<f16_t>(impl, qkv, o, out_bytes, B, N, D, heads, causal, nq, form, out_scale, outc);
    if (mode == ARP_MODE_BF16) return op_attn_forms<bf16_t>(impl, qkv, o, out_bytes, B, N, D, heads, causal, nq, form, out_scale, outc);
    if (mode == ARP_MODE_F32) return op_attn_forms<float>(impl, qkv, o, out_bytes, B, N, D, heads, causal, nq, form, out_scale, outc);
    return fail("attention_forms: mode must be f32, bf16 or f16");
}

int arp_op_qkv_attention(int mode, const float* A, const float* W, const float* bias, void* out, size_t out_bytes, int B, int N, int K, int heads, int causal,
                         int nq) {
    if (!A || !W || !bias || !out || B <= 0 || N <= 0 || K <= 0 || heads <= 0) return fail("bad argument");
    uint8_t* o = static_cast<uint8_t*>(out);
    if (mode == ARP_MODE_F16) return op_qkv_attn<f16_t>(A, W, bias, o, out_bytes, B, N, K, heads, causal, nq);
    if (mode == ARP_MODE_BF16) return op_qkv_attn<bf16_t>(A, W, bias, o, out_bytes, B, N, K, heads, causal, nq);
    return fail("qkv_attention: 16-bit modes only");
}

}

namespace {
struct CallerBuf {
    DevBuf d;
    void* host = nullptr;
    size_t n = 0;
    int up(void* h, size_t bytes) {
        host = h; n = bytes;
        ARP_TRY(d.ensure(std::max<size_t>(bytes, 16)));
        if (bytes) ARP_HIP_OK(hipMemcpy(d.p, h, bytes, hipMemcpyHostToDevice));
        return 0;
    }
    int down() {
        if (n) ARP_HIP_OK(hipMemcpy(host, d.p, n, hipMemcpyDeviceToHost));
        return 0;
    }
};
int up_i32(const int32_t* src, size_t n, DevBuf& d) {
    ARP_TRY(d.ensure(std::max<size_t>(n * 4, 16)));
    ARP_HIP_OK(hipMemcpy(d.p, src, n * 4, hipMemcpyHostToDevice));
    return 0;
}
int finish(int rc, std::initializer_list<CallerBuf*> bufs) {
    const hipError_t e = hipDeviceSynchronize();
    for (CallerBuf* b : bufs) {
        const int r = b->down();
        if (rc == 0 && r != 0) rc = r;
    }
    ARP_TRY(rc);
    ARP_HIP_OK(e);
    return 0;
}

template <typename OutT>
int op_ln_form(const float* x, size_t in_stride, const int* idx, void* out, int out_stride, const float* w, const float* b, int rows, int D, float eps) {
    if (idx) {
        if constexpr (std::is_same_v<OutT, float> || std::is_same_v<OutT, bf16_t> || std::is_same_v<OutT, f16_t>)
            return launch_layernorm_gather<OutT>(nullptr, x, in_stride, idx, static_cast<OutT*>(out), out_stride, w, b, rows, D, eps);
        else
            return fail("layernorm_forms: the gathered kernel is instantiated for the f32, bf16 and binary16 outputs only (run_text)");
    }
    Profiler prof;
    TowerCtx c;
    c.prof = &prof;
    return tower_layernorm<OutT>(c, "op.layernorm", x, in_stride, static_cast<OutT*>(out), out_stride, w, b, rows, D, eps);
}

template <typename T>
int op_assemble_lat(const float* patch, int S, size_t slice_stride, const float* cls, const float* pos, const float* w, const float* b, float* x, void* h,
                    const float* w1, const float* b1, int rows, int ntok, int D, float eps, float* stats) {
    return launch_vit_assemble_lat<T>(nullptr, patch, S, slice_stride, cls, pos, w, b, x, static_cast<T*>(h), w1, b1, rows, ntok, D, eps, stats, D >> 4);
}
}

extern "C" {

int arp_op_layernorm_forms(int form, const float* x, size_t x_floats, size_t in_stride, const int32_t* row_idx, const float* w, const float* b, void* out,
                           size_t out_bytes, int out_stride, int rows, int D, float eps) {
    if (!x || !w || !b || !out || rows <= 0 || D <= 0 || out_stride <= 0) return fail("layernorm_forms: bad argument");
    size_t esz, row_elems;
    switch (form) {
        case ARP_LN_OUT_F32: esz = 4; row_elems = D; break;
        case ARP_LN_OUT_BF16: case ARP_LN_OUT_F16: esz = 2; row_elems = D; break;
        case ARP_LN_OUT_E4M3: esz = 1; row_elems = D; break;
        case ARP_LN_OUT_SPLIT3: esz = 2; row_elems = (size_t)3 * D; break;
        case ARP_LN_OUT_F16C: case ARP_LN_OUT_F16C2: esz = 2; row_elems = (size_t)3 * D / 2; break;
        default: return fail("layernorm_forms: unknown output form");
    }
    if ((form == ARP_LN_OUT_F16C || form == ARP_LN_OUT_F16C2) && D % 256)
        return fail("layernorm_forms: [hi | x4 | dx4] rows feed gemm_c (\"f16c: widths must be multiples of 256\")");
    if (form == ARP_LN_OUT_SPLIT3 && (3 * D) % 64)
        return fail("layernorm_forms: (hi, lo, hi) rows are the A operand of a K = 3 D binary16 product (gemm_nt / gemm256_nt: K % 64 == 0)");
    if ((in_stride & 3) || (out_stride & 3) || in_stride < (size_t)D || (size_t)out_stride < row_elems)
        return fail("layernorm_forms: strides must be multiples of 4 elements and cover a row");
    if (row_idx) {
        for (int r = 0; r < rows; ++r)
            if (row_idx[r] < 0 || (size_t)row_idx[r] * in_stride + D > x_floats) return fail("layernorm_forms: row index outside x");
    } else if ((size_t)(rows - 1) * in_stride + D > x_floats) {
        return fail("layernorm_forms: x shorter than the rows it is read as");
    }
    if (out_bytes < ((size_t)(rows - 1) * out_stride + row_elems) * esz) return fail("layernorm_forms: output buffer shorter than its rows");
    DevBuf dx, dw, db, di;
    CallerBuf o;
    ARP_TRY(to_dev<float>(x, x_floats, dx)); ARP_TRY(to_dev<float>(w, D, dw)); ARP_TRY(to_dev<float>(b, D, db));
    if (row_idx) ARP_TRY(up_i32(row_idx, rows, di));
    ARP_TRY(o.up(out, out_bytes));
    const int* idx = row_idx ? di.as<int>() : nullptr;
    int rc;
#define ARP_LNF_CASE(F, OutT) \
    case F: rc = op_ln_form<OutT>(dx.as<float>(), in_stride, idx, o.d.p, out_stride, dw.as<float>(), db.as<float>(), rows, D, eps); break;
    switch (form) {
        ARP_LNF_CASE(ARP_LN_OUT_F32, float) ARP_LNF_CASE(ARP_LN_OUT_BF16, bf16_t) ARP_LNF_CASE(ARP_LN_OUT_F16, f16_t) ARP_LNF_CASE(ARP_LN_OUT_E4M3, fp8_t)
        ARP_LNF_CASE(ARP_LN_OUT_SPLIT3, f16x3_t) ARP_LNF_CASE(ARP_LN_OUT_F16C, f16c_t)
        default: rc = op_ln_form<f16c2_t>(dx.as<float>(), in_stride, idx, o.d.p, out_stride, dw.as<float>(), db.as<float>(), rows, D, eps); break;
    }
#undef ARP_LNF_CASE
    return finish(rc, {&o});
}

int arp_op_row_stats(int mode, const float* x, void* xb, size_t xb_bytes, void* stats, size_t stats_bytes, int rows, int D) {
    if (!x || !xb || !stats || rows <= 0 || D <= 0) return fail("row_stats: bad argument");
    if (mode != ARP_MODE_BF16 && mode != ARP_MODE_F16) return fail("row_stats: 16-bit modes only");
    if (D & 127) return fail("row_stats: the folded towers need a width that is a multiple of 128 (run_blocks: one (sum, sum of squares) pair per 128 columns)");
    if (xb_bytes < (size_t)rows * D * 2 || stats_bytes < (size_t)rows * (D >> 7) * 8) return fail("row_stats: output buffer too short");
    DevBuf dx;
    CallerBuf b, s;
    ARP_TRY(to_dev<float>(x, (size_t)rows * D, dx));
    ARP_TRY(b.up(xb, xb_bytes)); ARP_TRY(s.up(stats, stats_bytes));
    const int rc = mode == ARP_MODE_BF16 ? launch_row_stats<bf16_t>(nullptr, dx.as<float>(), b.d.as<bf16_t>(), s.d.as<float>(), rows, D)
                                         : launch_row_stats<f16_t>(nullptr, dx.as<float>(), b.d.as<f16_t>(), s.d.as<float>(), rows, D);
    return finish(rc, {&b, &s});
}

int arp_op_vit_assemble(int mode, int tail, const float* patch, size_t patch_floats, int S, size_t slice_stride, const float* cls, size_t cls_floats,
                        const float* pos, const float* w, const float* b, const float* w1, const float* b1, void* x, size_t x_bytes, void* h, size_t h_bytes,
                        void* stats, size_t stats_bytes, int B, int ntok, int D, float eps) {
    if (!patch || !cls || !pos || !w || !b || !x || B <= 0 || ntok <= 0 || D <= 0 || tail < ARP_ASM_LNPRE || tail > ARP_ASM_LAT_STATS)
        return fail("vit_assemble: bad argument");
    const size_t rows = (size_t)B * ntok, prow = (size_t)B * (ntok - 1) * D;
    if (cls_floats < (size_t)D || x_bytes < rows * D * 4) return fail("vit_assemble: cls or x too short");
    DevBuf dp, dc, dpos, dw, db, dw1, db1;
    CallerBuf ox, oh, os;
    if (tail == ARP_ASM_LNPRE) {
        if (patch_floats < prow) return fail("vit_assemble: patch matrix too short");
    } else {
        if (mode != ARP_MODE_BF16 && mode != ARP_MODE_F16) return fail("vit_assemble: the latency kernel exists in the 16-bit modes only");
        if (S >= 1 && patch_floats < (size_t)(S - 1) * slice_stride + prow) return fail("vit_assemble: patch slabs too short");
        if ((slice_stride & 3) && S > 1) return fail("vit_assemble: slab stride must be a multiple of 4 floats");
        if (!h || h_bytes < rows * D * 2) return fail("vit_assemble: h too short");
        if (tail == ARP_ASM_LAT_LN1 && (!w1 || !b1)) return fail("vit_assemble: the ln_1 tail needs w1 and b1");
        if (tail == ARP_ASM_LAT_STATS && (!stats || stats_bytes < rows * (size_t)(D >> 4) * 8)) return fail("vit_assemble: stats too short");
    }
    ARP_TRY(to_dev<float>(patch, patch_floats, dp)); ARP_TRY(to_dev<float>(cls, cls_floats, dc));
    ARP_TRY(to_dev<float>(pos, (size_t)ntok * D, dpos)); ARP_TRY(to_dev<float>(w, D, dw)); ARP_TRY(to_dev<float>(b, D, db));
    if (w1) ARP_TRY(to_dev<float>(w1, D, dw1));
    if (b1) ARP_TRY(to_dev<float>(b1, D, db1));
    ARP_TRY(ox.up(x, x_bytes));
    int rc;
    if (tail == ARP_ASM_LNPRE) {
        rc = launch_vit_assemble_lnpre(nullptr, dp.as<float>(), dc.as<float>(), dpos.as<float>(), dw.as<float>(), db.as<float>(), ox.d.as<float>(), (int)rows, ntok,
                                       D, eps);
        return finish(rc, {&ox});
    }
    ARP_TRY(oh.up(h, h_bytes));
    if (tail == ARP_ASM_LAT_STATS) ARP_TRY(os.up(stats, stats_bytes));
    float* st = tail == ARP_ASM_LAT_STATS ? os.d.as<float>() : nullptr;
    if (mode == ARP_MODE_BF16)
        rc = op_assemble_lat<bf16_t>(dp.as<float>(), S, slice_stride, dc.as<float>(), dpos.as<float>(), dw.as<float>(), db.as<float>(), ox.d.as<float>(), oh.d.p,
                                     dw1.as<float>(), db1.as<float>(), (int)rows, ntok, D, eps, st);
    else
        rc = op_assemble_lat<f16_t>(dp.as<float>(), S, slice_stride, dc.as<float>(), dpos.as<float>(), dw.as<float>(), db.as<float>(), ox.d.as<float>(), oh.d.p,
                                    dw1.as<float>(), db1.as<float>(), (int)rows, ntok, D, eps, st);
    if (tail == ARP_ASM_LAT_STATS) return finish(rc, {&ox, &oh, &os});
    return finish(rc, {&ox, &oh});
}

int arp_op_text_embed(const int32_t* tokens, const float* emb, int vocab, const float* pos, void* x, size_t x_bytes, int rows, int ctx, int D) {
    if (!tokens || !emb || !pos || !x || vocab <= 0 || rows <= 0 || ctx <= 0 || D <= 0) return fail("text_embed: bad argument");
    if (D & 3) return fail("text_embed: the width must be a multiple of 4 (float4 accesses)");
    for (int r = 0; r < rows; ++r)
        if (tokens[r] < 0 || tokens[r] >= vocab) return fail("text_embed: token id out of range");
    if (x_bytes < (size_t)rows * D * 4) return fail("text_embed: output buffer too short");
    DevBuf dt, de, dp;
    CallerBuf o;
    ARP_TRY(up_i32(tokens, rows, dt)); ARP_TRY(to_dev<float>(emb, (size_t)vocab * D, de)); ARP_TRY(to_dev<float>(pos, (size_t)ctx * D, dp));
    ARP_TRY(o.up(x, x_bytes));
    return finish(launch_text_embed(nullptr, dt.as<int>(), de.as<float>(), dp.as<float>(), o.d.as<float>(), rows, ctx, D), {&o});
}

int arp_op_rows_gather(const float* x, size_t x_floats, int D, const int32_t* rows, int row_stride, void* out, size_t out_bytes, int ld, int col0, int B) {
    if (!x || !out || D <= 0 || B <= 0 || col0 < 0 || ld < col0 + D || (!rows && row_stride < 0)) return fail("rows_gather: bad argument");
    for (int i = 0; i < B; ++i) {
        if (rows && rows[i] < 0) return fail("rows_gather: negative row index");
        const size_t r = rows ? (size_t)rows[i] : (size_t)i * row_stride;
        if ((r + 1) * D > x_floats) return fail("rows_gather: row outside x");
    }
    if (out_bytes < ((size_t)(B - 1) * ld + col0 + D) * 4) return fail("rows_gather: output buffer too short");
    DevBuf dx, dr;
    CallerBuf o;
    ARP_TRY(to_dev<float>(x, x_floats, dx));
    if (rows) ARP_TRY(up_i32(rows, B, dr));
    ARP_TRY(o.up(out, out_bytes));
    return finish(launch_rows_gather(nullptr, dx.as<float>(), D, rows ? dr.as<int>() : nullptr, row_stride, o.d.as<float>(), ld, col0, B), {&o});
}

int arp_op_l2_normalize(void* f, size_t f_bytes, int rows, int E) {
    if (!f || rows <= 0 || E <= 0 || f_bytes < (size_t)rows * E * 4) return fail("l2_normalize: bad argument");
    CallerBuf o;
    ARP_TRY(o.up(f, f_bytes));
    return finish(launch_l2_normalize(nullptr, o.d.as<float>(), rows, E), {&o});
}

int arp_op_reward(const float* img, const float* txt_n, float scale, void* reward, size_t reward_bytes, int rows, int E) {
    if (!img || !txt_n || !reward || rows <= 0 || E <= 0 || reward_bytes < (size_t)rows * 4) return fail("reward: bad argument");
    DevBuf di, dt;
    CallerBuf o;
    ARP_TRY(to_dev<float>(img, (size_t)rows * E, di)); ARP_TRY(to_dev<float>(txt_n, E, dt));
    ARP_TRY(o.up(reward, reward_bytes));
    return finish(launch_reward(nullptr, di.as<float>(), dt.as<float>(), scale, o.d.as<float>(), rows, E), {&o});
}

}
```

arp_amd/csrc/rowops.h:

```cpp
#pragma once
#include "common.h"

namespace arp {

constexpr int ROW_MAX_V4 = 8;
#define ARP_NV_DISPATCH(D, CALL)                   \
    do {                                           \
        const int _nv = ((D) + 255) / 256;         \
        if (_nv <= 1) { CALL(1); }                 \
        else if (_nv == 2) { CALL(2); }            \
        else if (_nv == 3) { CALL(3); }            \
        else if (_nv == 4) { CALL(4); }            \
        else { CALL(8); }                          \
    } while (0)

template <typename OutT, int NV>
__device__ __forceinline__ void ln_row_store(float (&v)[NV][4], int D, int lane, const float* __restrict__ w,
                                             const float* __restrict__ b, float eps, OutT* __restrict__ orow) {
    float s = 0.f;
#pragma unroll
    for (int i = 0; i < NV; ++i) {
        const int c = (i * 64 + lane) * 4;
        if (c < D) s += (v[i][0] + v[i][1]) + (v[i][2] + v[i][3]);
    }
    const float mean = wave_sum(s) / (float)D;
    float q = 0.f;
#pragma unroll
    for (int i = 0; i < NV; ++i) {
        const int c = (i * 64 + lane) * 4;
        if (c < D) {
#pragma unroll
            for (int j = 0; j < 4; ++j) {
                const float d = v[i][j] - mean;
                q += d * d;
            }
        }
    }
    const float rstd = 1.0f / sqrtf(wave_sum(q) / (float)D + eps);
#pragma unroll
    for (int i = 0; i < NV; ++i) {
        const int c = (i * 64 + lane) * 4;
        if (c < D) {
            const float4 ww = *reinterpret_cast<const float4*>(w + c);
            const float4 bb = *reinterpret_cast<const float4*>(b + c);
            if constexpr (__is_same(OutT, f16c_t) || __is_same(OutT, f16c2_t))
                store_f16c<__is_same(OutT, f16c2_t)>(reinterpret_cast<f16_t*>(orow), c, D, (v[i][0] - mean) * rstd * ww.x + bb.x, (v[i][1] - mean) * rstd * ww.y + bb.y,
                                                      (v[i][2] - mean) * rstd * ww.z + bb.z, (v[i][3] - mean) * rstd * ww.w + bb.w);
            else if constexpr (__is_same(OutT, f16x3_t))
                store_split3(reinterpret_cast<f16_t*>(orow) + c, (size_t)D, (v[i][0] - mean) * rstd * ww.x + bb.x, (v[i][1] - mean) * rstd * ww.y + bb.y,
                             (v[i][2] - mean) * rstd * ww.z + bb.z, (v[i][3] - mean) * rstd * ww.w + bb.w);
            else
            store4(orow + c, (v[i][0] - mean) * rstd * ww.x + bb.x, (v[i][1] - mean) * rstd * ww.y + bb.y,
                   (v[i][2] - mean) * rstd * ww.z + bb.z, (v[i][3] - mean) * rstd * ww.w + bb.w);
        }
    }
}

template <typename OutT, int NV>
__global__ __launch_bounds__(256) void layernorm_kernel(const float* __restrict__ in, size_t in_stride, OutT* __restrict__ out,
                                                        int out_stride, const float* __restrict__ w,
                                                        const float* __restrict__ b, int rows, int D, float eps) {
    const int lane = threadIdx.x & 63;
    const int row = blockIdx.x * 4 + (threadIdx.x >> 6);
    if (row >= rows) return;
    const float* irow = in + (size_t)row * in_stride;
    float v[NV][4];
#pragma unroll
    for (int i = 0; i < NV; ++i) {
        const int c = (i * 64 + lane) * 4;
        if (c < D) load4(irow + c, v[i]);
    }
    ln_row_store<OutT, NV>(v, D, lane, w, b, eps, out + (size_t)row * out_stride);
}

template <typename OutT, int NV>
__global__ __launch_bounds__(256) void layernorm_gather_kernel(const float* __restrict__ in, size_t in_stride,
                                                               const int* __restrict__ row_idx, OutT* __restrict__ out,
                                                               int out_stride, const float* __restrict__ w,
                                                               const float* __restrict__ b, int rows, int D, float eps) {
    const int lane = threadIdx.x & 63;
    const int row = blockIdx.x * 4 + (threadIdx.x >> 6);
    if (row >= rows) return;
    const float* irow = in + (size_t)row_idx[row] * in_stride;
    float v[NV][4];
#pragma unroll
    for (int i = 0; i < NV; ++i) {
        const int c = (i * 64 + lane) * 4;
        if (c < D) load4(irow + c, v[i]);
    }
    ln_row_store<OutT, NV>(v, D, lane, w, b, eps, out + (size_t)row * out_stride);
}

template <typename OutT>
static int launch_layernorm_gather(hipStream_t stream, const float* in, size_t in_stride, const int* row_idx, OutT* out, int out_stride, const float* w,
                                   const float* b, int rows, int D, float eps) {
    if (D % 4 || D > ROW_MAX_V4 * 256) return fail("layernorm_gather: unsupported width " + std::to_string(D));
#define ARP_LNG_CALL(NV)                                                                                                                         \
    hipLaunchKernelGGL((layernorm_gather_kernel<OutT, NV>), dim3((rows + 3) / 4), dim3(256), 0, stream, in, in_stride, row_idx, out, out_stride, w, b, \
                       rows, D, eps)
    ARP_NV_DISPATCH(D, ARP_LNG_CALL);
#undef ARP_LNG_CALL
    ARP_HIP_OK(hipGetLastError());
    return 0;
}

template <int NV>
__global__ __launch_bounds__(256) void vit_assemble_lnpre_kernel(const float* __restrict__ patch, const float* __restrict__ cls,
                                                                 const float* __restrict__ pos, const float* __restrict__ w,
                                                                 const float* __restrict__ b, float* __restrict__ x, int rows,
                                                                 int ntok, int D, float eps) {
    const int lane = threadIdx.x & 63;
    const int row = blockIdx.x * 4 + (threadIdx.x >> 6);
    if (row >= rows) return;
    const int bi = row / ntok, t = row - bi * ntok;
    const float* src = (t == 0) ? cls : patch + ((size_t)bi * (ntok - 1) + (t - 1)) * D;
    const float* prow = pos + (size_t)t * D;
    float v[NV][4];
#pragma unroll
    for (int i = 0; i < NV; ++i) {
        const int c = (i * 64 + lane) * 4;
        if (c < D) {
            float p4[4];
            load4(src + c, v[i]);
            load4(prow + c, p4);
#pragma unroll
            for (int j = 0; j < 4; ++j) v[i][j] += p4[j];
        }
    }
    ln_row_store<float, NV>(v, D, lane, w, b, eps, x + (size_t)row * D);
}

static int launch_vit_assemble_lnpre(hipStream_t stream, const float* patch, const float* cls, const float* pos, const float* w, const float* b, float* x,
                                     int rows, int ntok, int D, float eps) {
    if (D % 4 || D > ROW_MAX_V4 * 256) return fail("vit_assemble_lnpre: unsupported width " + std::to_string(D));
#define ARP_ASM_CALL(NV) \
    hipLaunchKernelGGL((vit_assemble_lnpre_kernel<NV>), dim3((rows + 3) / 4), dim3(256), 0, stream, patch, cls, pos, w, b, x, rows, ntok, D, eps)
    ARP_NV_DISPATCH(D, ARP_ASM_CALL);
#undef ARP_ASM_CALL
    ARP_HIP_OK(hipGetLastError());
    return 0;
}

template <typename T, int NV>
__global__ __launch_bounds__(64) void vit_assemble_lat_kernel(const float* __restrict__ patch, int S, size_t slice_stride, const float* __restrict__ cls,
                                                              const float* __restrict__ pos, const float* __restrict__ w, const float* __restrict__ b,
                                                              float* __restrict__ x, T* __restrict__ h, const float* __restrict__ w1,
                                                              const float* __restrict__ b1, int ntok, int D, float eps,
                                                              float* __restrict__ stats = nullptr, int parts = 0) {
    const int lane = threadIdx.x, row = blockIdx.x;
    const int bi = row / ntok, t = row - bi * ntok;
    const float* src = (t == 0) ? cls : patch + ((size_t)bi * (ntok - 1) + (t - 1)) * D;
    const float* prow = pos + (size_t)t * D;
    float v[NV][4];
    float s = 0.f;
#pragma unroll
    for (int i = 0; i < NV; ++i) {
        const int c = (i * 64 + lane) * 4;
        if (c < D) {
            float p4[4], sl[3][4];
            load4(src + c, v[i]);
            load4(prow + c, p4);
            const int nsl = t != 0 ? S - 1 : 0;
#pragma unroll
            for (int k = 0; k < 3; ++k)
                if (k < nsl) load4(src + (size_t)(k + 1) * slice_stride + c, sl[k]);
#pragma unroll
            for (int j = 0; j < 4; ++j) v[i][j] += p4[j];
#pragma unroll
            for (int k = 0; k < 3; ++k)
                if (k < nsl) {
#pragma unroll
                    for (int j = 0; j < 4; ++j) v[i][j] += sl[k][j];
                }
            s += (v[i][0] + v[i][1]) + (v[i][2] + v[i][3]);
        }
    }
    const float mean = wave_sum(s) / (float)D;
    float q = 0.f;
#pragma unroll
    for (int i = 0; i < NV; ++i) {
        const int c = (i * 64 + lane) * 4;
        if (c < D) {
#pragma unroll
            for (int j = 0; j < 4; ++j) {
                const float d = v[i][j] - mean;
                q += d * d;
            }
        }
    }
    const float rstd = 1.0f / sqrtf(wave_sum(q) / (float)D + eps);
#pragma unroll
    for (int i = 0; i < NV; ++i) {
        const int c = (i * 64 + lane) * 4;
        if (c < D) {
            const float4 ww = *reinterpret_cast<const float4*>(w + c);
            const float4 bb = *reinterpret_cast<const float4*>(b + c);
            v[i][0] = (v[i][0] - mean) * rstd * ww.x + bb.x; v[i][1] = (v[i][1] - mean) * rstd * ww.y + bb.y;
            v[i][2] = (v[i][2] - mean) * rstd * ww.z + bb.z; v[i][3] = (v[i][3] - mean) * rstd * ww.w + bb.w;
            store4(x + (size_t)row * D + c, v[i][0], v[i][1], v[i][2], v[i][3]);
        }
    }
    if (stats) {
        float su = 0.f, sq = 0.f;
#pragma unroll
        for (int i = 0; i < NV; ++i) {
            const int c = (i * 64 + lane) * 4;
            if (c < D) {
                store4(h + (size_t)row * D + c, v[i][0], v[i][1], v[i][2], v[i][3]);
                su += (v[i][0] + v[i][1]) + (v[i][2] + v[i][3]);
                sq += (v[i][0] * v[i][0] + v[i][1] * v[i][1]) + (v[i][2] * v[i][2] + v[i][3] * v[i][3]);
            }
        }
        su = wave_sum(su);
        sq = wave_sum(sq);
        float* st = stats + (size_t)row * parts * 2;
        for (int p = lane; p < parts; p += 64) {
            st[2 * p] = p == 0 ? su : 0.f;
            st[2 * p + 1] = p == 0 ? sq : 0.f;
        }
        return;
    }
    ln_row_store<T, NV>(v, D, lane, w1, b1, eps, h + (size_t)row * D);
}

template <typename T>
static int launch_vit_assemble_lat(hipStream_t stream, const float* patch, int S, size_t slice_stride, const float* cls, const float* pos, const float* w,
                                   const float* b, float* x, T* h, const float* w1, const float* b1, int rows, int ntok, int D, float eps, float* stats,
                                   int parts) {
    if (D % 4 || D > ROW_MAX_V4 * 256) return fail("vit_assemble_lat: unsupported width " + std::to_string(D));
    if (S < 1 || S > 4) return fail("vit_assemble_lat: the kernel sums 1 to 4 split-K slabs, not " + std::to_string(S));
#define ARP_ASML_CALL(NV)                                                                                                                             \
    hipLaunchKernelGGL((vit_assemble_lat_kernel<T, NV>), dim3(rows), dim3(64), 0, stream, patch, S, slice_stride, cls, pos, w, b, x, h, w1, b1, ntok, D, eps, \
                       stats, parts)
    ARP_NV_DISPATCH(D, ARP_ASML_CALL);
#undef ARP_ASML_CALL
    ARP_HIP_OK(hipGetLastError());
    return 0;
}

static __global__ __launch_bounds__(256) void text_embed_kernel(const int* __restrict__ tokens, const float* __restrict__ emb,
                                                         const float* __restrict__ pos, float* __restrict__ x, int rows, int ctx,
                                                         int D) {
    const int lane = threadIdx.x & 63;
    const int row = blockIdx.x * 4 + (threadIdx.x >> 6);
    if (row >= rows) return;
    const int t = row % ctx;
    const float* e = emb + (size_t)tokens[row] * D;
    for (int c = lane * 4; c < D; c += 256) {
        float a[4], p4[4];
        load4(e + c, a);
        load4(pos + (size_t)t * D + c, p4);
        store4(x + (size_t)row * D + c, a[0] + p4[0], a[1] + p4[1], a[2] + p4[2], a[3] + p4[3]);
    }
}

static int launch_text_embed(hipStream_t stream, const int* tokens, const float* emb, const float* pos, float* x, int rows, int ctx, int D) {
    hipLaunchKernelGGL(text_embed_kernel, dim3((rows + 3) / 4), dim3(256), 0, stream, tokens, emb, pos, x, rows, ctx, D);
    ARP_HIP_OK(hipGetLastError());
    return 0;
}

static __global__ __launch_bounds__(256) void l2_normalize_kernel(float* __restrict__ f, int rows, int E) {
    const int lane = threadIdx.x & 63;
    const int row = blockIdx.x * 4 + (threadIdx.x >> 6);
    if (row >= rows) return;
    float* r = f + (size_t)row * E;
    float s = 0.f;
    for (int c = lane; c < E; c += 64) s += r[c] * r[c];
    const float inv = 1.0f / sqrtf(wave_sum(s));
    for (int c = lane; c < E; c += 64) r[c] *= inv;
}

static int launch_l2_normalize(hipStream_t stream, float* f, int rows, int E) {
    hipLaunchKernelGGL(l2_normalize_kernel, dim3((rows + 3) / 4), dim3(256), 0, stream, f, rows, E);
    ARP_HIP_OK(hipGetLastError());
    return 0;
}

static __global__ __launch_bounds__(256) void reward_kernel(const float* __restrict__ img, const float* __restrict__ txt_n,
                                                     float scale, float* __restrict__ reward, int rows, int E) {
    const int lane = threadIdx.x & 63;
    const int row = blockIdx.x * 4 + (threadIdx.x >> 6);
    if (row >= rows) return;
    const float* r = img + (size_t)row * E;
    float ss = 0.f, dt = 0.f;
    for (int c = lane; c < E; c += 64) {
        const float a = r[c];
        ss += a * a;
        dt += a * txt_n[c];
    }
    ss = wave_sum(ss);
// ... 12 lines not shown
```

arp_amd/csrc/tower.h:

```cpp
#pragma once
#include <string>
#include <vector>

#include "attention.h"
#include "common.h"
#include "gemm.h"
#include "gemm256.h"
#include "qkvattn.h"
#include "rowops.h"
#include "skinny.h"
#include "runtime.h"

namespace arp {

enum Site { SITE_PATCH = 0, SITE_QKV = 1, SITE_OUT = 2, SITE_FC1 = 3, SITE_FC2 = 4, SITE_PROJ = 5, SITE_OP = 6 };

struct LayerW {
    float *ln1_w, *ln1_b, *ln2_w, *ln2_b, *b_in, *b_out, *b_fc, *b_proj;
    void *w_in, *w_out, *w_fc, *w_proj;
    void *w_fc8 = nullptr, *w_proj8 = nullptr;
    float *ln2_w8 = nullptr, *ln2_b8 = nullptr;
    float a_fc = 1.f, a_proj = 1.f;
    void *w_in8 = nullptr, *w_out8 = nullptr;
    float *ln1_w8 = nullptr, *ln1_b8 = nullptr;
    float a_in = 1.f, a_out = 1.f;
    void* w_in_hm = nullptr;
    float* b_in_hm = nullptr;
    void *w_in_f = nullptr, *w_fc_f = nullptr;
    float *c_in = nullptr, *d_in = nullptr, *c_fc = nullptr, *d_fc = nullptr;
};
struct TowerW {
    int width = 0, layers = 0, heads = 0;
    bool folded = false;
    bool lat_folded = false;
    std::vector<LayerW> L;
};

inline void fold_layernorm(const float* W, const float* gamma, const float* beta, const float* bias, int N, int K,
                           std::vector<bf16_t>& Wf, std::vector<float>& c, std::vector<float>& d, bool half = false) {
    Wf.resize((size_t)N * K);
    c.assign(N, 0.f);
    d.assign(N, 0.f);
    for (int n = 0; n < N; ++n) {
        double cs = 0.0, ds = bias ? (double)bias[n] : 0.0;
        for (int k = 0; k < K; ++k) {
            const float w = W[(size_t)n * K + k];
            float wf;
            if (half) {
                const f16_t wh = host_f2h(w * gamma[k]);
                Wf[(size_t)n * K + k] = __builtin_bit_cast(bf16_t, wh);
                wf = (float)__builtin_bit_cast(_Float16, wh);
            } else {
                const bf16_t wb = host_f2bf(w * gamma[k]);
                Wf[(size_t)n * K + k] = wb;
                uint32_t u = (uint32_t)wb << 16;
                memcpy(&wf, &u, 4);
            }
            cs += (double)wf;
            ds += (double)w * (double)beta[k];
        }
        c[n] = (float)cs;
        d[n] = (float)ds;
    }
}

template <typename T>
__global__ __launch_bounds__(256) void row_stats_kernel(const float* __restrict__ x, T* __restrict__ xb, float* __restrict__ stats,
                                                        int rows, int D) {
    const int lane = threadIdx.x & 63;
    const int row = blockIdx.x * 4 + (threadIdx.x >> 6);
    if (row >= rows) return;
    const int parts = D >> 7;
    for (int c0 = 0; c0 < D; c0 += 256) {
        const int c = c0 + lane * 4;
        float v[4] = {0.f, 0.f, 0.f, 0.f};
        if (c < D) {
            load4(x + (size_t)row * D + c, v);
            store4(xb + (size_t)row * D + c, v[0], v[1], v[2], v[3]);
        }
        float s = (v[0] + v[1]) + (v[2] + v[3]);
        float q = (v[0] * v[0] + v[1] * v[1]) + (v[2] * v[2] + v[3] * v[3]);
#pragma unroll
        for (int o = 16; o > 0; o >>= 1) {
            s += __shfl_xor(s, o, 64);
            q += __shfl_xor(q, o, 64);
        }
        const int seg = (c0 >> 7) + (lane >> 5);
        if ((lane & 31) == 0 && seg < parts) {
            stats[((size_t)row * parts + seg) * 2] = s;
            stats[((size_t)row * parts + seg) * 2 + 1] = q;
        }
    }
}

template <typename T>
static int launch_row_stats(hipStream_t stream, const float* x, T* xb, float* stats, int rows, int D) {
    hipLaunchKernelGGL((row_stats_kernel<T>), dim3((rows + 3) / 4), dim3(256), 0, stream, x, xb, stats, rows, D);
    ARP_HIP_OK(hipGetLastError());
    return 0;
}

struct GemmFold {
    const float* stats = nullptr;
    const float* c = nullptr;
    int parts = 0;
    float inv_d = 0.f, eps = 0.f;
    void* xb_out = nullptr;
    int ldxb = 0;
    float* stats_out = nullptr;
    int split3 = 0;
};

struct TowerCtx {
    hipStream_t stream = nullptr;
    Profiler* prof = nullptr;
    bool cls_only_last = false;
    int attn_impl = 0;
    int gemm_force = 0;
    bool fp8_mlp = false;
    bool fp8_attn = false;
    bool qkv_fused = true;
    unsigned long long* clock_acc = nullptr;
    bool shared_chip = false;
    bool skinny = false;
    bool h_ready0 = false;
    float* lat_stats = nullptr;
    bool lat_fold0 = false;
    float* part = nullptr;
    size_t part_floats = 0;
    float* ms_out = nullptr;
    int ms_ld = 0;
    const int* ms_rows = nullptr;
};

static __global__ __launch_bounds__(256) void rows_gather_kernel(const float* __restrict__ x, int D, const int* __restrict__ rows, int row_stride,
                                                                 float* __restrict__ out, int ld, int col0, int B) {
    const size_t i = (size_t)blockIdx.x * 256 + threadIdx.x;
    if (i >= (size_t)B * D) return;
    const int b = (int)(i / D), d = (int)(i - (size_t)b * D);
    const size_t row = rows ? (size_t)rows[b] : (size_t)b * row_stride;
    out[(size_t)b * ld + col0 + d] = x[row * D + d];
}
static int launch_rows_gather(hipStream_t stream, const float* x, int D, const int* rows, int row_stride, float* out, int ld, int col0, int B) {
    hipLaunchKernelGGL(rows_gather_kernel, dim3((unsigned)(((size_t)B * D + 255) / 256)), dim3(256), 0, stream, x, D, rows, row_stride, out, ld, col0, B);
    ARP_HIP_OK(hipGetLastError());
    return 0;
}
static int tower_export_rows(TowerCtx& c, const float* x, int D, int layer, int B, int N) {
    if (!c.ms_out) return 0;
    return launch_rows_gather(c.stream, x, D, c.ms_rows, N, c.ms_out, c.ms_ld, layer * D, B);
}

template <typename T, typename OutT, int ACT, bool RESID, int SITE>
static int tower_gemm(TowerCtx& c, const char* site, const void* A, const void* W, const float* bias, const float* resid, void* out,
                int M, int N, int K, const GemmFold* f = nullptr, int lda = 0, int ldr = 0, int ldo = 0) {
    GemmArgs g;
    if (f) {
        g.ln_stats = f->stats; g.ln_c = f->c; g.ln_parts = f->parts; g.ln_inv_d = f->inv_d; g.ln_eps = f->eps;
        g.xb_out = f->xb_out; g.ldxb = f->ldxb; g.stats_out = f->stats_out; g.split3 = f->split3;
    }
    g.A = A; g.W = W; g.bias = bias; g.resid = resid; g.out = out;
    g.M = M; g.N = N; g.K = K; g.lda = lda ? lda : K; g.ldw = K; g.ldr = ldr ? ldr : N; g.ldo = ldo ? ldo : N;
    ProfScope ps(*c.prof, c.stream, site);
    int force = c.gemm_force;
    if constexpr (sizeof(T) == 2 && (sizeof(OutT) == 4 || sizeof(OutT) == 2)) {
        if (c.skinny && force == 0 && !f && skinny_supported(M, N, K, g.lda, g.ldw) && !(g.ldo & 3) && !(RESID && (g.ldr & 3))) {
            SkinnyArgs k;
            k.A = A; k.W = W; k.bias = bias; k.resid = RESID ? resid : nullptr; k.out = out;
            k.M = M; k.N = N; k.K = K; k.lda = g.lda; k.ldw = g.ldw; k.ldr = g.ldr; k.ldo = g.ldo;
            k.act = ACT; k.out_f32 = sizeof(OutT) == 4;
            return launch_skinny_gemm(__is_same(T, bf16_t) ? 1 : 2, k, c.stream);
        }
    }
    if constexpr (SITE == SITE_FC1 && sizeof(T) == 2 && sizeof(OutT) == 2 && ACT == ACT_QGELU && !RESID) {
        if (c.clock_acc && !f && !c.skinny && force != 1 && force != 3 && (long)((M + 255) / 256) * ((N + 255) / 256) >= 192) {
            g.clock_acc = c.clock_acc;
            return launch_gemm256_nt<T, OutT, ACT, RESID, SITE, (ARP_G2_MFMA32 != 0), ARP_G2_KV, false, true>(g, c.stream);
        }
    }
    static const int out_g256_env = [] { const char* e = getenv("ARP_OUT_G256"); return e ? (atoi(e) != 0 ? 1 : 0) : -1; }();
    const bool out_g256 = out_g256_env >= 0 ? out_g256_env == 1 : c.shared_chip;
    if (force == 0 && (SITE & 7) == SITE_OUT && M >= 4096) force = out_g256 ? 2 : 3;
    return launch_gemm_auto<T, OutT, ACT, RESID, SITE>(g, c.stream, force);
}
template <typename T, typename OutT, int ACT, bool RESID, int SITE, typename Site>
static int tower_gemm_site(const Site& d) {
    Profiler prof;
    TowerCtx c;
    c.prof = &prof;
    c.gemm_force = d.force;
    GemmFold f;
    f.stats = d.ln_stats; f.c = d.ln_c; f.parts = d.ln_parts; f.inv_d = 1.0f / (float)d.K; f.eps = d.ln_eps;
    f.xb_out = d.xb_out; f.ldxb = d.ldxb; f.stats_out = d.stats_out; f.split3 = d.split3;
    const bool fold = d.ln_stats || d.xb_out || d.stats_out;
    return tower_gemm<T, OutT, ACT, RESID, SITE>(c, "op.gemm_site", d.A, d.W, d.bias, RESID ? d.resid : nullptr, d.out, d.M, d.N, d.K, fold ? &f : nullptr,
                                                 d.lda, d.ldr, d.ldo);
}

template <typename OutT>
static int tower_layernorm(TowerCtx& c, const char* site, const float* in, size_t in_stride, OutT* out, int out_stride,
                     const float* w, const float* b, int rows, int D, float eps) {
    if (D % 4 || D > ROW_MAX_V4 * 256) return fail("layernorm: unsupported width " + std::to_string(D));
    ProfScope ps(*c.prof, c.stream, site);
#define ARP_LN_CALL(NV)                                                                                                   \
    hipLaunchKernelGGL((layernorm_kernel<OutT, NV>), dim3((rows + 3) / 4), dim3(256), 0, c.stream, in, in_stride, out, \
                       out_stride, w, b, rows, D, eps)
    ARP_NV_DISPATCH(D, ARP_LN_CALL);
#undef ARP_LN_CALL
    ARP_HIP_OK(hipGetLastError());
    return 0;
}

template <typename T>
static int launch_attention(hipStream_t stream, int impl, const T* qkv, T* out, int B, int N, int D, int heads, int causal, int nq = 0, float out8 = 0.f,
                            f16_t* out3 = nullptr, int outc = 0) {
    const int hd = D / heads;
    if (nq <= 0 || nq > N) nq = N;
    const float scale = 1.0f / sqrtf((float)hd);
    if constexpr (sizeof(T) == 2) {
        if (impl == 0 && hd == 64) {
            const int NT = ((N + 31) / 32) * 2;
#define ARP_ATTN_CASE(nt)                                                                                                   \
    case nt: {                                                                                                              \
        auto kern = attn_mfma_kernel<T, nt>;                                                                                  \
        const int lds = nt * 16 * 256;                                                                 \
        ARP_HIP_OK(hipFuncSetAttribute(reinterpret_cast<const void*>(kern), hipFuncAttributeMaxDynamicSharedMemorySize, lds)); \
        const int nqb_ = (nq + 15) / 16;                                                                                    \
        const int qsplit_ = (B * heads < 128 && nqb_ > 4) ? std::min((nqb_ + 3) / 4, 4) : 1;                                   \
        hipLaunchKernelGGL(kern, dim3(B* heads, qsplit_), dim3(256), lds, stream, qkv, out, N, D, heads, scale, causal, nq, out8, outc);  \
        ARP_HIP_OK(hipGetLastError());                                                                                      \
        return 0;                                                                                                           \
    }
            switch (NT) {
                ARP_ATTN_CASE(2)
                ARP_ATTN_CASE(4)
                ARP_ATTN_CASE(6)
                ARP_ATTN_CASE(8)
                ARP_ATTN_CASE(14)
                ARP_ATTN_CASE(18)
                default: break;
            }
#undef ARP_ATTN_CASE
        }
    }
    if (out8 != 0.f || outc) return fail("attention: the e4m3 / [hi | x4 | dx4] outputs exist on the MFMA kernel only");
    if constexpr (sizeof(T) == 4) {
        if (impl == 3 && hd == 64 && N <= 288 && (D & 3) == 0) {
            const int need = 2 * ((N - 1) / 32) + (((N - 1) % 32) >= 4 ? 2 : 1);
#define ARP_ATTNX3_CASE(nt)                                                                                                        \
    if (need <= nt) {                                                                                                              \
        const int ldsx = attn_x3_lds_bytes(nt);                                                                                    \
        auto kern = attn_x3_kernel<nt>;                                                                                            \
        ARP_HIP_OK(hipFuncSetAttribute(reinterpret_cast<const void*>(kern), hipFuncAttributeMaxDynamicSharedMemorySize, ldsx));    \
        hipLaunchKernelGGL(kern, dim3(B* heads), dim3(512), ldsx, stream, qkv, out, N, D, heads, scale, causal, nq, out3);          \
        ARP_HIP_OK(hipGetLastError());                                                                                             \
        return 0;                                                                                                                  \
    }
            ARP_ATTNX3_CASE(2)
            ARP_ATTNX3_CASE(4)
            ARP_ATTNX3_CASE(6)
            ARP_ATTNX3_CASE(14)
            ARP_ATTNX3_CASE(17)
            ARP_ATTNX3_CASE(18)
#undef ARP_ATTNX3_CASE
        }
        if (impl == 3) impl = 0;
        if (impl == 0 && hd == 64 && N <= 288 && (D & 3) == 0) {
            const int need = (N + 15) / 16;
#define ARP_ATTN32_CASE(nt)                                                                                                        \
    if (need <= nt) {                                                                                                              \
        const int lds32 = 2 * nt * 16 * 68 * 4;                                                                                    \
        auto kern = attn_f32_mfma_kernel<nt>;                                                                                      \
        ARP_HIP_OK(hipFuncSetAttribute(reinterpret_cast<const void*>(kern), hipFuncAttributeMaxDynamicSharedMemorySize, lds32));   \
        hipLaunchKernelGGL(kern, dim3(B* heads), dim3(256), lds32, stream, qkv, out, N, D, heads, scale, causal, nq, out3);         \
        ARP_HIP_OK(hipGetLastError());                                                                                             \
        return 0;                                                                                                                  \
    }
            ARP_ATTN32_CASE(1)
            ARP_ATTN32_CASE(4)
            ARP_ATTN32_CASE(5)
            ARP_ATTN32_CASE(13)
            ARP_ATTN32_CASE(17)
            ARP_ATTN32_CASE(18)
#undef ARP_ATTN32_CASE
        }
    }
    if (out3) return fail("attention: the (hi, lo, hi) output exists on the f32-MFMA kernel only (head_dim 64, <= 288 tokens)");
    const size_t lds = (size_t)2 * N * hd * 4;
    if (lds > 160 * 1024) return fail("attention: sequence too long for the LDS-resident kernel");
    const int threads = N <= 64 ? 64 : (N <= 128 ? 128 : 256);
    if (hd == 64) {
        auto kern = attn_valu_kernel<T, 64>;
        ARP_HIP_OK(hipFuncSetAttribute(reinterpret_cast<const void*>(kern), hipFuncAttributeMaxDynamicSharedMemorySize, (int)lds));
        hipLaunchKernelGGL(kern, dim3(B * heads), dim3(threads), lds, stream, qkv, out, N, D, heads, scale, causal, nq, (const float*)nullptr);
    } else if (hd == 32) {
        auto kern = attn_valu_kernel<T, 32>;
        ARP_HIP_OK(hipFuncSetAttribute(reinterpret_cast<const void*>(kern), hipFuncAttributeMaxDynamicSharedMemorySize, (int)lds));
        hipLaunchKernelGGL(kern, dim3(B * heads), dim3(threads), lds, stream, qkv, out, N, D, heads, scale, causal, nq, (const float*)nullptr);
    } else if (hd == 16) {
        auto kern = attn_valu_kernel<T, 16>;
        ARP_HIP_OK(hipFuncSetAttribute(reinterpret_cast<const void*>(kern), hipFuncAttributeMaxDynamicSharedMemorySize, (int)lds));
        hipLaunchKernelGGL(kern, dim3(B * heads), dim3(threads), lds, stream, qkv, out, N, D, heads, scale, causal, nq, (const float*)nullptr);
    } else {
        return fail("attention: unsupported head_dim " + std::to_string(hd));
    }
    ARP_HIP_OK(hipGetLastError());
    return 0;
}

static inline bool attn_mfma_has(int N, int hd) {
    const int NT = ((N + 31) / 32) * 2;
    return hd == 64 && (NT == 2 || NT == 4 || NT == 6 || NT == 8 || NT == 14 || NT == 18);
}
static inline bool attn_vperm_applies(int N, int hd) { return hd == 64 && N > 64; }
static inline int attn_vperm_col(int o, int D) { return o < 2 * D ? o : (o & ~63) | ((o >> 2) & 3) << 4 | ((o >> 4) & 3) << 2 | (o & 3); }
constexpr float FP8_S_A = 16.f;

template <typename T, int SB>
static int tower_attn_fp8(TowerCtx& c, const TowerW& tw, const LayerW& L, const char* s_ln1, const char* s_qkv, const char* s_attn, const char* s_out, float* x,
                          T* h, T* qkv, T* ao, int B, int N, int causal, float eps) {
    const int D = tw.width, M = B * N;
    fp8_t* h8 = reinterpret_cast<fp8_t*>(h);
    ARP_TRY(tower_layernorm<fp8_t>(c, s_ln1, x, D, h8, D, L.ln1_w8, L.ln1_b8, M, D, eps));
    GemmArgs g;
    g.A = h8; g.W = L.w_in8; g.bias = L.b_in; g.out = qkv;
    g.M = M; g.N = 3 * D; g.K = D; g.lda = D; g.ldw = D; g.ldr = 3 * D; g.ldo = 3 * D;
    g.alpha = L.a_in;
    {
        ProfScope ps(*c.prof, c.stream, s_qkv);
        ARP_TRY((launch_gemm256_nt<fp8_t, T, ACT_NONE, false, SB + SITE_QKV>(g, c.stream)));
    }
    {
        ProfScope ps(*c.prof, c.stream, s_attn);
        ARP_TRY(launch_attention<T>(c.stream, 0, qkv, ao, B, N, D, tw.heads, causal, 0, FP8_S_A));
    }
    GemmArgs q;
    q.A = ao; q.W = L.w_out8; q.bias = L.b_out; q.resid = x; q.out = x;
    q.M = M; q.N = D; q.K = D; q.lda = D; q.ldw = D; q.ldr = D; q.ldo = D;
    q.alpha = L.a_out;
    ProfScope ps(*c.prof, c.stream, s_out);
    return launch_gemm256_nt<fp8_t, float, ACT_NONE, true, SB + SITE_OUT>(q, c.stream);
}

template <typename T, int SITE>
static int tower_qkv_attention(TowerCtx& c, const TowerW& tw, const LayerW& L, const char* s_qkv, const char* s_attn, const char* s_fused, const T* h,
                               T* qkv, T* ao, int B, int N, int causal, int nq) {
    const int D = tw.width, M = B * N;
    if constexpr (sizeof(T) == 2) {
        if (c.qkv_fused && L.w_in_hm && c.attn_impl == 0 && qkv_attn_supported(N, D, tw.heads, (int)sizeof(T)) && !c.skinny) {
            QkvAttnArgs q;
            q.A = h; q.W = L.w_in_hm; q.bias = L.b_in_hm; q.out = ao;
            q.B = B; q.N = N; q.K = D; q.heads = tw.heads; q.lda = D; q.ldw = D; q.ldo = D; q.fpt = 0; q.nq = nq; q.causal = causal; q.scale = 0.f;
            ProfScope ps(*c.prof, c.stream, s_fused);
            return launch_qkv_attn<T>(q, c.stream);
        }
    }
    ARP_TRY((tower_gemm<T, T, ACT_NONE, false, SITE>(c, s_qkv, h, L.w_in, L.b_in, nullptr, qkv, M, 3 * D, D)));
    ProfScope ps(*c.prof, c.stream, s_attn);
    return launch_attention<T>(c.stream, c.attn_impl, qkv, ao, B, N, D, tw.heads, causal, nq);
}

constexpr float FP8_S_H = 32.f, FP8_S_G = 16.f;

template <typename T, int ACT, int SB>
static int tower_mlp_fp8(TowerCtx& c, const LayerW& L, const char* s_ln2, const char* s_fc1, const char* s_fc2, float* x, T* h, T* fc, int M, int D, float eps) {
    fp8_t* h8 = reinterpret_cast<fp8_t*>(h);
    fp8_t* fc8 = reinterpret_cast<fp8_t*>(fc);
    ARP_TRY(tower_layernorm<fp8_t>(c, s_ln2, x, D, h8, D, L.ln2_w8, L.ln2_b8, M, D, eps));
    GemmArgs g;
    g.A = h8; g.W = L.w_fc8; g.bias = L.b_fc; g.resid = nullptr; g.out = fc8;
    g.M = M; g.N = 4 * D; g.K = D; g.lda = D; g.ldw = D; g.ldr = 4 * D; g.ldo = 4 * D;
    g.alpha = L.a_fc; g.out_scale = FP8_S_G;
    {
        ProfScope ps(*c.prof, c.stream, s_fc1);
        ARP_TRY((launch_gemm256_nt<fp8_t, fp8_t, ACT, false, SB + SITE_FC1>(g, c.stream)));
    }
    GemmArgs q;
    q.A = fc8; q.W = L.w_proj8; q.bias = L.b_proj; q.resid = x; q.out = x;
    q.M = M; q.N = D; q.K = 4 * D; q.lda = 4 * D; q.ldw = 4 * D; q.ldr = D; q.ldo = D;
    q.alpha = L.a_proj;
    ProfScope ps(*c.prof, c.stream, s_fc2);
    return launch_gemm256_nt<fp8_t, float, ACT_NONE, true, SB + SITE_FC2>(q, c.stream);
}

template <typename T>
static int tower_gemm_split_ln(TowerCtx& c, const char* s_gemm, const char* s_red, const void* A, const void* W, const float* bias, float* x, int M, int D,
                               int K, int S, T* h, const float* ln_w, const float* ln_b, float eps) {
    const int tcode = __is_same(T, bf16_t) ? 1 : 2;
    const size_t slab = (size_t)M * D;
    if ((size_t)S * slab > c.part_floats) return fail("tower: split-K slab buffer too small");
    SkinnyArgs k;
    k.A = A; k.W = W; k.out = c.part; k.M = M; k.N = D; k.K = K; k.lda = K; k.ldw = K; k.ldo = D; k.out_f32 = 1;
    k.ksplit = S; k.slice_stride = slab;
    {
        ProfScope ps(*c.prof, c.stream, s_gemm);
        ARP_TRY(launch_skinny_gemm(tcode, k, c.stream));
    }
    ProfScope ps(*c.prof, c.stream, s_red);
    return launch_skinny_reduce_ln(tcode, c.part, S, slab, bias, x, D, h, D, ln_w, ln_b, M, D, eps, c.stream);
}
static inline int tower_split_of(int M, int D, int K) {
    for (int S = K >= 2048 ? 4 : (K >= 512 ? 2 : 1); S >= 1; S >>= 1)
        if (skinny_supported(M, D, K, K, K, S) && K / S >= 32) return S;
    return 0;
}

template <typename T, int ACT, int SB>
static int run_blocks(TowerCtx& c, const TowerW& tw, const char* tag, float* x, T* h, T* qkv, T* ao, T* fc, int B, int N, int causal,
                      float eps, float* stats = nullptr) {
    const int D = tw.width, M = B * N;
    const std::string t(tag);
    const std::string s_ln1 = t + ".ln_1", s_qkv = t + ".qkv", s_attn = t + ".attn", s_out = t + ".out_proj", s_ln2 = t + ".ln_2",
                      s_fc1 = t + ".c_fc", s_fc2 = t + ".c_proj", s_st = t + ".ln_stats", s_qa = t + ".qkv_attn", s_qa1 = t + ".qkv_attn_cls";
    if (stats && tw.folded && sizeof(T) == 2 && (D & 127) == 0) {
        GemmFold cons, prod;
        cons.stats = stats; cons.parts = D >> 7; cons.inv_d = 1.0f / (float)D; cons.eps = eps;
        prod.xb_out = h; prod.ldxb = D; prod.stats_out = stats;
        {
            ProfScope ps(*c.prof, c.stream, s_st.c_str());
            ARP_TRY(launch_row_stats<T>(c.stream, x, h, stats, M, D));
        }
        for (int i = 0; i < tw.layers; ++i) {
            const LayerW& L = tw.L[i];
            cons.c = L.c_in;
            ARP_TRY((tower_gemm<T, T, ACT_NONE, false, SB + SITE_QKV>(c, s_qkv.c_str(), h, L.w_in_f, L.d_in, nullptr, qkv, M, 3 * D, D, &cons)));
            {
                ProfScope ps(*c.prof, c.stream, s_attn.c_str());
                ARP_TRY(launch_attention<T>(c.stream, c.attn_impl, qkv, ao, B, N, D, tw.heads, causal));
            }
            ARP_TRY((tower_gemm<T, float, ACT_NONE, true, SB + SITE_OUT>(c, s_out.c_str(), ao, L.w_out, L.b_out, x, x, M, D, D, &prod)));
            cons.c = L.c_fc;
            ARP_TRY((tower_gemm<T, T, ACT, false, SB + SITE_FC1>(c, s_fc1.c_str(), h, L.w_fc_f, L.d_fc, nullptr, fc, M, 4 * D, D, &cons)));
            ARP_TRY((tower_gemm<T, float, ACT_NONE, true, SB + SITE_FC2>(c, s_fc2.c_str(), fc, L.w_proj, L.b_proj, x, x, M, D, 4 * D, &prod)));
            ARP_TRY(tower_export_rows(c, x, D, i, B, N));
        }
        return 0;
    }
    const int S_out = tower_split_of(M, D, D), S_proj = tower_split_of(M, D, 4 * D);
    const bool lat = sizeof(T) == 2 && c.skinny && c.gemm_force == 0 && !c.fp8_mlp && c.part && M <= SKINNY_MAX_M && S_out && S_proj &&
                     (size_t)std::max(S_out, S_proj) * M * D <= c.part_floats && skinny_supported(M, 3 * D, D, D, D) && skinny_supported(M, 4 * D, D, D, D);
    const std::string s_red2 = t + ".out_reduce_ln_2", s_red1 = t + ".proj_reduce_ln_1";
    const bool fold = lat && tw.lat_folded && c.lat_stats && c.lat_fold0 && (D & 15) == 0 && skinny_supported(M, D, 4 * D, 4 * D, 4 * D);
    bool h_ready = lat && !fold && c.h_ready0;
    bool qkv_ready = false;
    for (int i = 0; i < tw.layers; ++i) {
        const LayerW& L = tw.L[i];
        if constexpr (sizeof(T) == 2) {
            const bool cls_blk = c.cls_only_last && i == tw.layers - 1 && N > 1;
            if (fold && cls_blk && i > 0) {
                const int tcode = __is_same(T, bf16_t) ? 1 : 2;
                SkinnyArgs k;
                k.A = h; k.W = L.w_in_f; k.bias = L.d_in; k.out = qkv; k.M = M; k.N = 3 * D; k.K = D; k.lda = D; k.ldw = D; k.ldo = 3 * D;
                k.ln_stats = c.lat_stats; k.ln_c = L.c_in; k.ln_parts = D >> 4; k.ln_inv_d = 1.0f / (float)D; k.ln_eps = eps;
                {
                    ProfScope ps(*c.prof, c.stream, s_qkv.c_str());
                    ARP_TRY(launch_skinny_gemm(tcode, k, c.stream));
                }
                qkv_ready = true;
            }
            if (fold && !cls_blk) {
                const int tcode = __is_same(T, bf16_t) ? 1 : 2;
                auto consumer = [&](const char* site, const void* Wf, const float* dvec, const float* cvec, void* out, int Nout, int act) -> int {
                    SkinnyArgs k;
                    k.A = h; k.W = Wf; k.bias = dvec; k.out = out; k.M = M; k.N = Nout; k.K = D; k.lda = D; k.ldw = D; k.ldo = Nout; k.act = act;
                    k.ln_stats = c.lat_stats; k.ln_c = cvec; k.ln_parts = D >> 4; k.ln_inv_d = 1.0f / (float)D; k.ln_eps = eps;
                    ProfScope ps(*c.prof, c.stream, site);
                    return launch_skinny_gemm(tcode, k, c.stream);
                };
                auto producer = [&](const char* site, const void* A, const void* W, const float* bias, int K) -> int {
                    SkinnyArgs k;
                    k.A = A; k.W = W; k.bias = bias; k.resid = x; k.out = x; k.M = M; k.N = D; k.K = K; k.lda = K; k.ldw = K; k.ldr = D; k.ldo = D;
                    k.out_f32 = 1; k.strips = 1; k.xb = h; k.ldxb = D; k.stats_out = c.lat_stats;
                    ProfScope ps(*c.prof, c.stream, site);
                    return launch_skinny_gemm(tcode, k, c.stream);
                };
                ARP_TRY(consumer(s_qkv.c_str(), L.w_in_f, L.d_in, L.c_in, qkv, 3 * D, ACT_NONE));
                {
                    ProfScope ps(*c.prof, c.stream, s_attn.c_str());
                    ARP_TRY(launch_attention<T>(c.stream, c.attn_impl, qkv, ao, B, N, D, tw.heads, causal));
                }
                ARP_TRY(producer(s_out.c_str(), ao, L.w_out, L.b_out, D));
                ARP_TRY(consumer(s_fc1.c_str(), L.w_fc_f, L.d_fc, L.c_fc, fc, 4 * D, ACT));
                ARP_TRY(producer(s_fc2.c_str(), fc, L.w_proj, L.b_proj, 4 * D));
                ARP_TRY(tower_export_rows(c, x, D, i, B, N));
                continue;
            }
            if (lat && !(c.cls_only_last && i == tw.layers - 1 && N > 1)) {
                if (!h_ready) ARP_TRY(tower_layernorm<T>(c, s_ln1.c_str(), x, D, h, D, L.ln1_w, L.ln1_b, M, D, eps));
                ARP_TRY((tower_qkv_attention<T, SB + SITE_QKV>(c, tw, L, s_qkv.c_str(), s_attn.c_str(), s_qa.c_str(), h, qkv, ao, B, N, causal, 0)));
                ARP_TRY(tower_gemm_split_ln<T>(c, s_out.c_str(), s_red2.c_str(), ao, L.w_out, L.b_out, x, M, D, D, S_out, h, L.ln2_w, L.ln2_b, eps));
                ARP_TRY((tower_gemm<T, T, ACT, false, SB + SITE_FC1>(c, s_fc1.c_str(), h, L.w_fc, L.b_fc, nullptr, fc, M, 4 * D, D)));
                const LayerW* nx = i + 1 < tw.layers ? &tw.L[i + 1] : nullptr;
                ARP_TRY(tower_gemm_split_ln<T>(c, s_fc2.c_str(), s_red1.c_str(), fc, L.w_proj, L.b_proj, x, M, D, 4 * D, S_proj, h, nx ? nx->ln1_w : nullptr,
                                               nx ? nx->ln1_b : nullptr, eps));
                h_ready = nx != nullptr;
                ARP_TRY(tower_export_rows(c, x, D, i, B, N));
                continue;
            }
        }
        if (c.cls_only_last && i == tw.layers - 1 && N > 1) {
            const std::string s_attn1 = t + ".attn_cls", s_out1 = t + ".out_proj_cls", s_ln21 = t + ".ln_2_cls", s_fc11 = t + ".c_fc_cls",
                              s_fc21 = t + ".c_proj_cls";
            const int ND = N * D;
            if (qkv_ready) {
                ProfScope ps(*c.prof, c.stream, s_attn1.c_str());
                ARP_TRY(launch_attention<T>(c.stream, c.attn_impl, qkv, ao, B, N, D, tw.heads, causal, 1));
            } else {
                if (!h_ready) ARP_TRY(tower_layernorm<T>(c, s_ln1.c_str(), x, D, h, D, L.ln1_w, L.ln1_b, M, D, eps));
                ARP_TRY((tower_qkv_attention<T, SB + SITE_QKV>(c, tw, L, s_qkv.c_str(), s_attn1.c_str(), s_qa1.c_str(), h, qkv, ao, B, N, causal, 1)));
            }
            ARP_TRY((tower_gemm<T, float, ACT_NONE, true, SB + SITE_OUT>(c, s_out1.c_str(), ao, L.w_out, L.b_out, x, x, B, D, D, nullptr, ND, ND, ND)));
            ARP_TRY(tower_layernorm<T>(c, s_ln21.c_str(), x, ND, h, D, L.ln2_w, L.ln2_b, B, D, eps));
            ARP_TRY((tower_gemm<T, T, ACT, false, SB + SITE_FC1>(c, s_fc11.c_str(), h, L.w_fc, L.b_fc, nullptr, fc, B, 4 * D, D)));
            ARP_TRY((tower_gemm<T, float, ACT_NONE, true, SB + SITE_FC2>(c, s_fc21.c_str(), fc, L.w_proj, L.b_proj, x, x, B, D, 4 * D, nullptr, 0, ND, ND)));
            ARP_TRY(tower_export_rows(c, x, D, i, B, N));
            break;
        }
        bool attn_done = false;
        if constexpr (sizeof(T) == 2) {
            if (c.fp8_attn && L.w_in8 && c.attn_impl == 0 && (D % 128) == 0 && attn_mfma_has(N, D / tw.heads) &&
                !(c.qkv_fused && L.w_in_hm && qkv_attn_supported(N, D, tw.heads, (int)sizeof(T)))) {
                const std::string s_ln18 = t + ".ln_1_fp8", s_qkv8 = t + ".qkv_fp8", s_attn8 = t + ".attn_out8", s_out8 = t + ".out_proj_fp8";
                ARP_TRY((tower_attn_fp8<T, SB>(c, tw, L, s_ln18.c_str(), s_qkv8.c_str(), s_attn8.c_str(), s_out8.c_str(), x, h, qkv, ao, B, N, causal, eps)));
                attn_done = true;
            }
        }
        if (!attn_done) {
            ARP_TRY(tower_layernorm<T>(c, s_ln1.c_str(), x, D, h, D, L.ln1_w, L.ln1_b, M, D, eps));
            ARP_TRY((tower_qkv_attention<T, SB + SITE_QKV>(c, tw, L, s_qkv.c_str(), s_attn.c_str(), s_qa.c_str(), h, qkv, ao, B, N, causal, 0)));
            ARP_TRY((tower_gemm<T, float, ACT_NONE, true, SB + SITE_OUT>(c, s_out.c_str(), ao, L.w_out, L.b_out, x, x, M, D, D)));
        }
        if (sizeof(T) == 2 && c.fp8_mlp && L.w_fc8 && (D % 128) == 0) {
            const std::string s_fc18 = t + ".c_fc_fp8", s_fc28 = t + ".c_proj_fp8";
            ARP_TRY((tower_mlp_fp8<T, ACT, SB>(c, L, s_ln2.c_str(), s_fc18.c_str(), s_fc28.c_str(), x, h, fc, M, D, eps)));
        } else {
            ARP_TRY(tower_layernorm<T>(c, s_ln2.c_str(), x, D, h, D, L.ln2_w, L.ln2_b, M, D, eps));
            ARP_TRY((tower_gemm<T, T, ACT, false, SB + SITE_FC1>(c, s_fc1.c_str(), h, L.w_fc, L.b_fc, nullptr, fc, M, 4 * D, D)));
            ARP_TRY((tower_gemm<T, float, ACT_NONE, true, SB + SITE_FC2>(c, s_fc2.c_str(), fc, L.w_proj, L.b_proj, x, x, M, D, 4 * D)));
        }
        ARP_TRY(tower_export_rows(c, x, D, i, B, N));
    }
    return 0;
}

}
```

include/arp_hip.h:

```cpp
#ifndef ARP_HIP_H
#define ARP_HIP_H
#include <stddef.h>
#include <stdint.h>

#ifdef __cplusplus
extern "C" {
#endif

#define ARP_MODE_F32 0
#define ARP_MODE_BF16 1
#define ARP_MODE_F16 2

#define ARP_MODE_F16X3 3
#define ARP_MODE_F16C 4

#define ARP_ACT_NONE 0
#define ARP_ACT_QGELU 1
#define ARP_ACT_RELU 2
#define ARP_ACT_TANH 3
#define ARP_ACT_GELU_TANH 4

const char* arp_last_error(void);
int arp_version(void);
int arp_debug_live(int64_t out5[5]);
// ... 156 lines not shown
int arp_ft_get_tensor(arp_ft* h, const char* name, int which, float* out);
int arp_ft_dropped_gradients(arp_ft* h, uint64_t* count);
int arp_ft_set_step(arp_ft* h, int64_t step);
int arp_ft_get_step(arp_ft* h, int64_t* step);
int arp_ft_set_batch(arp_ft* h, const float* img_inter, const float* img_final, const float* txt_inter, const float* txt_final,
                     const float* r, const int32_t* action, int B);
int arp_ft_set_batch_dev(arp_ft* h, const float* img_inter_dev, const float* img_final_dev, const float* txt_inter_dev,
                         const float* txt_final_dev, const float* r , const int32_t* action , int B);
int arp_ft_forward(arp_ft* h, float* metrics4, float* scores, float* logits);
int arp_ft_encode(arp_ft* h, int which, const float* inter, const float* final_feat, int n, float* out);
int arp_ft_reward_set_text(arp_ft* h, arp_clip* towers, const int32_t* tokens , int n_prompts);
int arp_ft_reward_set_reduce(arp_ft* h, int mean);
int arp_ft_reward_dev_async(arp_ft* h, arp_clip* towers, const uint8_t* frames_dev, int n, int H, int W, int use_crop, int transform, float* rewards_dev);
int arp_ft_reward(arp_ft* h, arp_clip* towers, const uint8_t* frames, int n, int H, int W, int use_crop, int transform, float* rewards);
int arp_ft_reward_set_rows(arp_ft* h, int on);
int arp_ft_reward_stats(arp_ft* h, int64_t out4[4]);
int arp_op_ft_rows_gemm(int mode, int act, const float* A, int lda, const float* W, int ldw, const float* bias, float* out, int ldo, int out_rows, int out_f32,
                        int M, int N, int K, int ksplit);
int arp_op_ft_reward(const float* f, const float* A, float rw, const float* t, int n_prompts, int mean, float scale, float* reward, int rows, int F);
int arp_ft_backward(arp_ft* h);
int arp_ft_train_step(arp_ft* h, float lr, float* aux4);
int arp_ft_train_step_async(arp_ft* h, float lr);
int arp_ft_sync(arp_ft* h);
int arp_ft_event_record(arp_ft* h, arp_event* e);
int arp_ft_comm_init(arp_ft* h, const void* id128, int world, int rank);
int arp_ft_broadcast_state(arp_ft* h);
int arp_ft_comm_info(arp_ft* h, int32_t* info5);
int arp_ft_comm_selfcheck(arp_ft* h, double* sum);
int arp_ft_bucket_plan(const arp_ft_cfg* cfg, int64_t* ranges28, int64_t* total);
int arp_ft_profile_enable(arp_ft* h, int on);
int arp_ft_profile_reset(arp_ft* h);
int arp_ft_profile_json(arp_ft* h, char* buf, int buf_len);

typedef struct arp_enc arp_enc;
typedef struct arp_enc_cfg {
    int32_t patch;
    int32_t width;
    int32_t layers;
    int32_t heads;
    int32_t mlp_ratio;
    int32_t img_res;
    int32_t mode;
    int32_t device;
    int32_t max_frames;
    int32_t attn_impl;
} arp_enc_cfg;
int arp_enc_create(const arp_enc_cfg* cfg, arp_enc** out);
int arp_enc_destroy(arp_enc* h);
int arp_enc_load_weight(arp_enc* h, const char* name, const float* data, const int64_t* shape, int ndim);
int arp_enc_finalize_weights(arp_enc* h);
int arp_enc_forward(arp_enc* h, const float* images_host, int n, float* out_host);
int arp_enc_set_streams(arp_enc* h, int n_streams, int first_part_frames, int min_part_frames);
int arp_enc_set_latency(arp_enc* h, int rows, int host_calls);
int arp_enc_profile_enable(arp_enc* h, int on);
int arp_enc_profile_json(arp_enc* h, char* buf, int buf_len);
int arp_dt_attach_encoder(arp_dt* h, arp_enc* enc);
int arp_dt_set_batch_images(arp_dt* h, const float* images, const int32_t* action, const float* rtg, int B);
int arp_dt_encode_ahead(arp_dt* h, int slot);

typedef struct arp_ds arp_ds;
int arp_ds_create(int64_t n_rows, int res, int device, arp_ds** out);
int arp_ds_destroy(arp_ds* ds);
int arp_ds_upload_frames(arp_ds* ds, int64_t row0, int64_t n, const uint8_t* u8_host);
int arp_ds_set_labels(arp_ds* ds, const int32_t* action, const float* rtg, const int32_t* traj_start, int n_actions);
int arp_ds_set_lut(arp_ds* ds, const float* lut768);
int arp_ds_alloc_encodings(arp_ds* ds, int tokens, int dim);
int arp_ds_upload_encodings(arp_ds* ds, int64_t row0, int64_t n, const float* f32_host);
int arp_ds_encode(arp_ds* ds, arp_enc* enc, int chunk);
int arp_ds_gather_debug(arp_ds* ds, const int64_t* idx, int B, int window, float* frames_out, int32_t* action_out, float* rtg_out);
int64_t arp_ds_nbytes(arp_ds* ds);
int arp_dt_upload_batch_indices_async(arp_dt* h, int slot, arp_ds* ds, const int64_t* idx, int B, int use_encodings);
int arp_dt_set_batch_indices(arp_dt* h, arp_ds* ds, const int64_t* idx, int B, int use_encodings);

typedef struct arp_rollout arp_rollout;
int arp_rollout_create(arp_dt* policy, arp_clip* reward_or_null, int n_envs, int H, int W, float scale, arp_rollout** out);
int arp_rollout_create_with_encoder(arp_dt* policy, arp_enc* encoder, arp_clip* reward_or_null, int n_envs, int H, int W, float scale, arp_rollout** out);
int arp_rollout_create_ft(arp_dt* policy, arp_enc* encoder_or_null, arp_clip* towers, arp_ft* head, int n_envs, int H, int W, float scale, arp_rollout** out);
int arp_rollout_destroy(arp_rollout* h);
int arp_rollout_reset(arp_rollout* h, const int32_t* env_ids, int n, const float* rtg0);
int arp_rollout_set_lut(arp_rollout* h, const float* lut768);
int arp_rollout_set_reward_norm(arp_rollout* h, int use_normalize, float reward_min);
int arp_rollout_step(arp_rollout* h, const uint8_t* frames_host , const float* rewards_or_null , int use_crop,
                     int32_t* actions_out );
int arp_rollout_read(arp_rollout* h, const char* what, void* out, int64_t bytes);
int arp_rollout_debug_set_tail(arp_rollout* h, float value, int action);

int arp_h5_inflate_last_frames(int fd, int n, const uint64_t* addr, const uint64_t* size, const uint8_t* stored_raw,
                               uint64_t chunk_bytes, uint64_t frame_bytes, const uint64_t* dst_off, const uint32_t* cnt,
                               uint8_t* out, int threads);
int arp_h5_write_rows_deflated(void* write_chunk_fn, int64_t dset, int64_t dxpl, const void* rows, uint64_t row_bytes, uint64_t n_rows,
                               uint64_t first_row, int ndim, int level);

int arp_op_gemm_fp8(int act, const float* A, const float* W, const float* bias, const float* resid, float* out, int M, int N, int K, float alpha,
                    int out_fp8, float out_scale);
int arp_op_gemm_nt(int mode, int act, const float* A, const float* W, const float* bias, const float* resid,
                   float* out, int M, int N, int K);
int arp_op_skinny_gemm(int mode, int act, const float* A, const float* W, const float* bias, const float* resid, float* out, int M, int N, int K,
                       int ksplit, const float* ln_w, const float* ln_b, float eps, float* h_out);
int arp_op_gemm_tn(int mode, int tile256, int ksplit, const float* A, const float* B, float* out, int M, int N, int K, float alpha);
int arp_op_gemm_relu_bwd(int mode, const float* A, const float* W, const float* mask, float* out, float* colsum, int M, int N, int K);
int arp_op_splitk_reduce(int out_type, const float* part, int S, int M, int N, const float* bias, int act, const float* resid, float* out, int ldo,
                         float alpha);
int arp_op_gemm_bwd(int kind, int mode, int out_type, int ksplit, const float* A, int lda, const float* B, int ldb, const float* resid, float* out,
                    int ldo, float* slabs, int M, int N, int K, float alpha);
int arp_op_adapter_dy(int mode, const float* dz, const float* Wi, const float* A, const float* x, float rw, float* dApre, float* colsum,
                      float* dres, int R, int E, int tokens, int D);
int arp_op_gemm_f16c(int plan, const float* A, const float* W, const float* bias, float* out, int M, int N, int K, int* sd_sw);
typedef struct arp_gemm_site {
    const char* name;
    int mode, force;
    int M, N, K, lda, ldr, ldo;
    const void* A;
    const void* W;
    const float* bias;
    const float* resid;
    void* out;
    const float* ln_stats;
    const float* ln_c;
    int ln_parts;
    float ln_eps;
    void* xb_out;
    int ldxb, split3;
    float* stats_out;
    int plan, sd, sw;
    void* x4_out;
    void* dx4_out;
    int ld4;
} arp_gemm_site;
int arp_op_gemm_site(const arp_gemm_site* d);
int arp_op_gemm_bench(int mode, int kernel, int act, int resid, int out_f32, int M, int N, int K, int iters, float* avg_ms);
int arp_op_layernorm(const float* x, const float* w, const float* b, float* out, int rows, int D, float eps);
int arp_op_attention(int mode, int impl, const float* qkv, float* out, int B, int N, int D, int heads, int causal);
#define ARP_ATTN_OUT_PLAIN 0
#define ARP_ATTN_OUT_E4M3 1
#define ARP_ATTN_OUT_F16C 2
#define ARP_ATTN_OUT_SPLIT3 3
int arp_op_attention_forms(int mode, int impl, const float* qkv, void* out, size_t out_bytes, int B, int N, int D, int heads, int causal, int nq, int form,
                           float out_scale, int outc);
int arp_op_qkv_attention(int mode, const float* A, const float* W, const float* bias, void* out, size_t out_bytes, int B, int N, int K, int heads, int causal,
                         int nq);
#define ARP_LN_OUT_F32 0
#define ARP_LN_OUT_BF16 1
#define ARP_LN_OUT_F16 2
#define ARP_LN_OUT_E4M3 3
#define ARP_LN_OUT_SPLIT3 4
#define ARP_LN_OUT_F16C 5
#define ARP_LN_OUT_F16C2 6
int arp_op_layernorm_forms(int form, const float* x, size_t x_floats, size_t in_stride, const int32_t* row_idx, const float* w, const float* b, void* out,
                           size_t out_bytes, int out_stride, int rows, int D, float eps);
int arp_op_row_stats(int mode, const float* x, void* xb, size_t xb_bytes, void* stats, size_t stats_bytes, int rows, int D);
#define ARP_ASM_LNPRE 0
#define ARP_ASM_LAT_LN1 1
#define ARP_ASM_LAT_STATS 2
int arp_op_vit_assemble(int mode, int tail, const float* patch, size_t patch_floats, int S, size_t slice_stride, const float* cls, size_t cls_floats,
                        const float* pos, const float* w, const float* b, const float* w1, const float* b1, void* x, size_t x_bytes, void* h, size_t h_bytes,
                        void* stats, size_t stats_bytes, int B, int ntok, int D, float eps);
int arp_op_text_embed(const int32_t* tokens, const float* emb, int vocab, const float* pos, void* x, size_t x_bytes, int rows, int ctx, int D);
int arp_op_rows_gather(const float* x, size_t x_floats, int D, const int32_t* rows, int row_stride, void* out, size_t out_bytes, int ld, int col0, int B);
int arp_op_l2_normalize(void* f, size_t f_bytes, int rows, int E);
int arp_op_reward(const float* img, const float* txt_n, float scale, void* reward, size_t reward_bytes, int rows, int E);
int arp_op_convert_f16c(int with_dx, const float* x, void* xb, size_t xb_bytes, void* xc, size_t xc_bytes, int rows, int D);
int arp_op_extract_hi(const void* in, size_t in_bytes, int ld, void* out, size_t out_bytes, int rows, int D);
int arp_op_split3(const float* x, void* out, size_t out_bytes, int rows, int K);
int arp_op_rollout_decide(const float* logits, const int32_t* lens, int E, int T, int n_actions, int32_t* actions_out);

#ifdef __cplusplus
}
#endif
#endif
```

Baseline: 100,200 frames/s.

## Fuse first-layer ln_1 into ViT assemble and add class-row GEMM kernel

The patch-embedding assembly kernel can now also apply layer 0's ln_1 and write the 16-bit h buffer, so the throughput path skips a separate layernorm pass over all tokens. A new dedicated GEMM kernel for small-M class-token rows (multi-stage LDS pipeline with direct global-to-LDS loads and 32/64-row tiles) is used by default for the last-layer CLS-only out_proj, MLP and the final visual projection. This removes a full-tensor read/write and aims to raise utilisation on skinny M=1024 GEMMs, at the cost of a new kernel path with extra alignment constraints and hand-written waitcnt scheduling.

Result: no change. 100,800 frames/s, median of 6 (+0.6%).

```diff
diff --git a/arp_amd/_ffi.py b/arp_amd/_ffi.py
--- a/arp_amd/_ffi.py
+++ b/arp_amd/_ffi.py
@@ -10,7 +10,7 @@
 ACT_NONE, ACT_QGELU, ACT_RELU, ACT_TANH, ACT_GELU_TANH = 0, 1, 2, 3, 4
 ATTN_OUT_PLAIN, ATTN_OUT_E4M3, ATTN_OUT_F16C, ATTN_OUT_SPLIT3 = 0, 1, 2, 3
 LN_OUT_F32, LN_OUT_BF16, LN_OUT_F16, LN_OUT_E4M3, LN_OUT_SPLIT3, LN_OUT_F16C, LN_OUT_F16C2 = 0, 1, 2, 3, 4, 5, 6
-ASM_LNPRE, ASM_LAT_LN1, ASM_LAT_STATS = 0, 1, 2
+ASM_LNPRE, ASM_LAT_LN1, ASM_LAT_STATS, ASM_LNPRE_LN1 = 0, 1, 2, 3
 
 
 class ArpError(RuntimeError):
diff --git a/arp_amd/csrc/arp_clip.hip b/arp_amd/csrc/arp_clip.hip
--- a/arp_amd/csrc/arp_clip.hip
+++ b/arp_amd/csrc/arp_clip.hip
@@ -54,6 +54,7 @@
     float* lut = nullptr;
 
     int gemm_force = 0;
+    bool cls_rows = true;
     bool ln_fold = false;
     bool fp8_mlp = false;
     bool fp8_attn = false;
@@ -115,6 +116,7 @@
     bool lat_f0 = false;
     bool lat_h0 = false;
     bool lat_now = false;
+    bool asm_h0 = false;
     struct LatGraph {
         const uint8_t* frames;
         float* rewards;
@@ -138,12 +140,13 @@
     t.prof = &c->prof;
     t.attn_impl = c->cfg.attn_impl;
     t.gemm_force = c->gemm_force;
+    t.cls_rows = c->cls_rows;
     t.qkv_fused = c->qkv_fused;
     t.shared_chip = c->shared_chip;
     t.clock_acc = c->shared()->clock_acc;
     t.fp8_mlp = c->fp8_mlp; t.fp8_attn = c->fp8_attn;
     t.ms_out = c->ms_out; t.ms_ld = c->ms_ld; t.ms_rows = c->ms_rows;
-    t.skinny = c->lat_now; t.h_ready0 = c->lat_now && c->lat_h0; t.lat_stats = c->lat_stats.as<float>(); t.lat_fold0 = c->lat_now && c->lat_f0; t.part = c->part.as<float>(); t.part_floats = c->part.bytes / 4;
+    t.skinny = c->lat_now; t.h_ready0 = (c->lat_now && c->lat_h0) || c->asm_h0; t.lat_stats = c->lat_stats.as<float>(); t.lat_fold0 = c->lat_now && c->lat_f0; t.part = c->part.as<float>(); t.part_floats = c->part.bytes / 4;
     return t;
 }
 
@@ -372,7 +375,7 @@
     c->lat_now = c->skinny && sizeof(T) == 2 && (long)nb * N <= c->lat_rows;
     struct LatGuard {
         arp_clip* c;
-        ~LatGuard() { c->lat_now = false; c->lat_h0 = false; c->lat_f0 = false; }
+        ~LatGuard() { c->lat_now = false; c->lat_h0 = false; c->lat_f0 = false; c->asm_h0 = false; }
     } lat_guard{c};
     if (c->pre_bilinear) {
         ProfScope ps(c->prof, c->stream, "preprocess_bilinear");
@@ -414,12 +417,25 @@
                                                          nb * G * G, D, KP)));
     {
         ProfScope ps(c->prof, c->stream, "vit.assemble_ln_pre");
-        ARP_TRY(launch_vit_assemble_lnpre(c->stream, c->pe.as<float>(), c->cls, c->pos, c->lnpre_w, c->lnpre_b, c->x.as<float>(), nb * N, N, D, 1e-5f));
+        bool ln1_tail = false;
+        if constexpr (sizeof(T) == 2) ln1_tail = !c->lat_now && c->vis.layers > 0 && !c->vis.folded && !c->fp8_attn;
+        if constexpr (sizeof(T) == 2) {
+            if (ln1_tail)
+                ARP_TRY(launch_vit_assemble_lnpre_ln1<T>(c->stream, c->pe.as<float>(), c->cls, c->pos, c->lnpre_w, c->lnpre_b, c->x.as<float>(), c->h.as<T>(),
+                                                         c->vis.L[0].ln1_w, c->vis.L[0].ln1_b, nb * N, N, D, 1e-5f));
+        }
+        if (!ln1_tail)
+            ARP_TRY(launch_vit_assemble_lnpre(c->stream, c->pe.as<float>(), c->cls, c->pos, c->lnpre_w, c->lnpre_b, c->x.as<float>(), nb * N, N, D, 1e-5f));
+        c->asm_h0 = ln1_tail;
     }
     }
     ARP_TRY(run_blocks<T>(c, c->vis, "vit", c->x.as<float>(), c->h.as<T>(), c->qkv.as<T>(), c->ao.as<T>(), c->fc.as<T>(), nb, N, 0, c->stats.as<float>()));
     ARP_TRY(layernorm<T>(c, "vit.ln_post", c->x.as<float>(), (size_t)N * D, c->cls_h.as<T>(), D, c->lnpost_w, c->lnpost_b, nb, D, 1e-5f));
-    ARP_TRY((gemm<T, float, ACT_NONE, false, SITE_PROJ>(c, "vit.proj", c->cls_h.p, c->proj_t, nullptr, nullptr, c->feat.p, nb, k.embed, D)));
+    {
+        TowerCtx t = ctx_of(c);
+        if (t.cls_rows && !t.skinny && t.gemm_force == 0 && cls_rows_fit<T>(nb, k.embed, D)) t.gemm_force = 4;
+        ARP_TRY((tower_gemm<T, float, ACT_NONE, false, SITE_PROJ>(t, "vit.proj", c->cls_h.p, c->proj_t, nullptr, nullptr, c->feat.p, nb, k.embed, D)));
+    }
     return 0;
 }
 
@@ -771,6 +787,7 @@
     if (const char* e = getenv("ARP_GEMM")) c->gemm_force = atoi(e);
     if (const char* e = getenv("ARP_LN_FOLD")) c->ln_fold = atoi(e) != 0;
     if (const char* e = getenv("ARP_CLS_ONLY")) c->cls_only_last = atoi(e) != 0;
+    if (const char* e = getenv("ARP_CLS_ROWS")) c->cls_rows = atoi(e) != 0;
     if (const char* e = getenv("ARP_QKV_FUSED")) c->qkv_fused = atoi(e) != 0;
     if (const char* e = getenv("ARP_SKINNY")) c->skinny = atoi(e) != 0;
     if (const char* e = getenv("ARP_LAT_FOLD")) c->lat_fold = atoi(e) != 0;
@@ -1305,6 +1322,7 @@
     if (s == "vit.c_fc") return tower_gemm_site<T, T, ACT_QGELU, false, SITE_FC1>(d);
     if (s == "vit.out_proj") return tower_gemm_site<T, float, ACT_NONE, true, SITE_OUT>(d);
     if (s == "vit.c_proj") return tower_gemm_site<T, float, ACT_NONE, true, SITE_FC2>(d);
+    if (s == "vit.proj") return tower_gemm_site<T, float, ACT_NONE, false, SITE_PROJ>(d);
     return fail("gemm_site: unknown instance " + s);
 }
 
@@ -1650,7 +1668,7 @@
 int arp_op_vit_assemble(int mode, int tail, const float* patch, size_t patch_floats, int S, size_t slice_stride, const float* cls, size_t cls_floats,
                         const float* pos, const float* w, const float* b, const float* w1, const float* b1, void* x, size_t x_bytes, void* h, size_t h_bytes,
                         void* stats, size_t stats_bytes, int B, int ntok, int D, float eps) {
-    if (!patch || !cls || !pos || !w || !b || !x || B <= 0 || ntok <= 0 || D <= 0 || tail < ARP_ASM_LNPRE || tail > ARP_ASM_LAT_STATS)
+    if (!patch || !cls || !pos || !w || !b || !x || B <= 0 || ntok <= 0 || D <= 0 || tail < ARP_ASM_LNPRE || tail > ARP_ASM_LNPRE_LN1)
         return fail("vit_assemble: bad argument");
     const size_t rows = (size_t)B * ntok, prow = (size_t)B * (ntok - 1) * D;
     if (cls_floats < (size_t)D || x_bytes < rows * D * 4) return fail("vit_assemble: cls or x too short");
@@ -1658,6 +1676,10 @@
     CallerBuf ox, oh, os;
     if (tail == ARP_ASM_LNPRE) {
         if (patch_floats < prow) return fail("vit_assemble: patch matrix too short");
+    } else if (tail == ARP_ASM_LNPRE_LN1) {
+        if (patch_floats < prow) return fail("vit_assemble: patch matrix too short");
+        if (mode != ARP_MODE_BF16 && mode != ARP_MODE_F16) return fail("vit_assemble: the ln_1 tail exists in the 16-bit modes only");
+        if (!h || h_bytes < rows * D * 2 || !w1 || !b1) return fail("vit_assemble: the ln_1 tail needs h, w1 and b1");
     } else {
         if (mode != ARP_MODE_BF16 && mode != ARP_MODE_F16) return fail("vit_assemble: the latency kernel exists in the 16-bit modes only");
         if (S >= 1 && patch_floats < (size_t)(S - 1) * slice_stride + prow) return fail("vit_assemble: patch slabs too short");
@@ -1678,6 +1700,15 @@
         return finish(rc, {&ox});
     }
     ARP_TRY(oh.up(h, h_bytes));
+    if (tail == ARP_ASM_LNPRE_LN1) {
+        if (mode == ARP_MODE_BF16)
+            rc = launch_vit_assemble_lnpre_ln1<bf16_t>(nullptr, dp.as<float>(), dc.as<float>(), dpos.as<float>(), dw.as<float>(), db.as<float>(), ox.d.as<float>(),
+                                                       oh.d.as<bf16_t>(), dw1.as<float>(), db1.as<float>(), (int)rows, ntok, D, eps);
+        else
+            rc = launch_vit_assemble_lnpre_ln1<f16_t>(nullptr, dp.as<float>(), dc.as<float>(), dpos.as<float>(), dw.as<float>(), db.as<float>(), ox.d.as<float>(),
+                                                      oh.d.as<f16_t>(), dw1.as<float>(), db1.as<float>(), (int)rows, ntok, D, eps);
+        return finish(rc, {&ox, &oh});
+    }
     if (tail == ARP_ASM_LAT_STATS) ARP_TRY(os.up(stats, stats_bytes));
     float* st = tail == ARP_ASM_LAT_STATS ? os.d.as<float>() : nullptr;
     if (mode == ARP_MODE_BF16)
diff --git a/arp_amd/csrc/clsrows.h b/arp_amd/csrc/clsrows.h
--- /dev/null
+++ b/arp_amd/csrc/clsrows.h
@@ -0,0 +1,36 @@
+#pragma once
+#include "common.h"
+#include "gemm.h"
+
+namespace arp {
+
+constexpr int CR_BN = 32, CR_THREADS = 256, CR_STAGES = 6;
+constexpr int CR_MAX_M = 4096;
+constexpr int cr_stage_bytes(int mi) { return (32 * mi + CR_BN) * 128; }
+
+inline bool clsrows_supported(const GemmArgs& g, bool out_f32, bool resid) {
+    if (g.M < 1 || g.M > CR_MAX_M || g.N < 16 || (g.N & 15) || g.K < 64 || (g.K & 63)) return false;
+    if ((g.lda & 7) || (g.ldw & 7) || (g.ldo & 3) || (resid && (g.ldr & 3))) return false;
+    if ((reinterpret_cast<uintptr_t>(g.A) | reinterpret_cast<uintptr_t>(g.W)) & 15) return false;
+    if (reinterpret_cast<uintptr_t>(g.out) & (out_f32 ? 15 : 7)) return false;
+    if ((g.bias && (reinterpret_cast<uintptr_t>(g.bias) & 15)) || (resid && (reinterpret_cast<uintptr_t>(g.resid) & 15))) return false;
+    return g.ksplit <= 1 && !g.ln_stats && !g.xb_out && !g.stats_out && !g.split3 && g.alpha == 1.f && !g.mask && !g.colsum_part && !g.adam_p &&
+           !(g.flags & 3) && g.mix_nk16 == 0 && g.x8_shift < 0 && !g.dx4_out && !g.clock_acc && g.out;
+}
+
+int launch_clsrows_dyn(int tcode, int out_f32, int act, int resid, const GemmArgs& g, hipStream_t stream);
+bool clsrows_has(int tcode, int out_f32, int act, int resid);
+
+template <typename T, typename OutT, int ACT, bool RESID>
+inline bool try_clsrows(const GemmArgs& g, hipStream_t stream, int& rc) {
+    if constexpr (sizeof(T) != 2) return false;
+    else {
+        const int tcode = __is_same(T, bf16_t) ? 1 : 2, of = sizeof(OutT) == 4 ? 1 : 0;
+        if (sizeof(OutT) != 4 && !__is_same(OutT, T)) return false;
+        if (!clsrows_has(tcode, of, ACT, RESID ? 1 : 0) || !clsrows_supported(g, of != 0, RESID)) return false;
+        rc = launch_clsrows_dyn(tcode, of, ACT, RESID ? 1 : 0, g, stream);
+        return true;
+    }
+}
+
+}
diff --git a/arp_amd/csrc/clsrows.hip b/arp_amd/csrc/clsrows.hip
--- /dev/null
+++ b/arp_amd/csrc/clsrows.hip
@@ -0,0 +1,185 @@
+#include "clsrows.h"
+
+#include <type_traits>
+
+#include "../../include/arp_hip.h"
+#include "runtime.h"
+
+namespace arp {
+
+template <int N> __device__ __forceinline__ void cr_wait_vm() { asm volatile("s_waitcnt vmcnt(%0)" ::"n"(N) : "memory"); }
+template <int A, int PER> __device__ __forceinline__ void cr_wait_ahead(int ahead) {
+    if constexpr (A == 0) cr_wait_vm<0>();
+    else {
+        if (ahead >= A) cr_wait_vm<A * PER>();
+        else cr_wait_ahead<A - 1, PER>(ahead);
+    }
+}
+
+template <typename T, typename OutT, int ACT, bool RESID, int MI>
+__global__ __launch_bounds__(CR_THREADS) void clsrows_kernel(GemmArgs g) {
+    static_assert(sizeof(T) == 2, "16-bit operand types only");
+    static_assert(MI == 1 || MI == 2, "32 or 64 rows per workgroup");
+    extern __shared__ __attribute__((aligned(16))) char smem[];
+    constexpr int EPB = 64, EPC = 8;
+    constexpr int BM = 32 * MI;
+    constexpr int ACH = BM / 8;
+    constexpr int PER = (ACH + 4) / 4;
+    constexpr int STAGE = cr_stage_bytes(MI);
+
+    const int tid = threadIdx.x;
+    const int lane = tid & 63;
+    const int wave = __builtin_amdgcn_readfirstlane(tid >> 6);
+    const int m_tiles = (g.M + BM - 1) / BM, n_tiles = (g.N + CR_BN - 1) / CR_BN;
+    const int tile = xcd_remap(blockIdx.x, m_tiles * n_tiles);
+    const int m0 = (tile % m_tiles) * BM, n0 = (tile / m_tiles) * CR_BN;
+
+    const T* __restrict__ A = static_cast<const T*>(g.A);
+    const T* __restrict__ W = static_cast<const T*>(g.W);
+
+    const int wr = wave >> 1, wc = wave & 1;
+    const int fr = lane & 15, fg = lane >> 4;
+    const int sw = fr & 7;
+    int a_off[MI];
+#pragma unroll
+    for (int mi = 0; mi < MI; ++mi) a_off[mi] = (wr * 16 * MI + mi * 16 + fr) * 128;
+    const int w_off = BM * 128 + (wc * 16 + fr) * 128;
+
+    const int en = n0 + wc * 16 + fg * 4;
+    const int enc = min(en, g.N - 4);
+    const float4 b4 = *reinterpret_cast<const float4*>(g.bias ? g.bias + enc : reinterpret_cast<const float*>(g.A));
+    float4 r4[MI];
+    if constexpr (RESID) {
+#pragma unroll
+        for (int mi = 0; mi < MI; ++mi) {
+            const int m = min(m0 + wr * 16 * MI + mi * 16 + fr, g.M - 1);
+            r4[mi] = *reinterpret_cast<const float4*>(g.resid + (size_t)m * g.ldr + enc);
+        }
+    }
+
+    const int srow = lane >> 3;
+    const int schunk = (lane & 7) ^ srow;
+    const T* src[PER];
+#pragma unroll
+    for (int i = 0; i < PER; ++i) {
+        if (i * 4 < ACH) {
+            int am = m0 + (i * 4 + wave) * 8 + srow;
+            am = am < g.M ? am : g.M - 1;
+            src[i] = A + (size_t)am * g.lda + schunk * EPC;
+        } else {
+            int wn = n0 + (i * 4 + wave - ACH) * 8 + srow;
+            wn = wn < g.N ? wn : g.N - 1;
+            src[i] = W + (size_t)wn * g.ldw + schunk * EPC;
+        }
+    }
+    const int nk = g.K / EPB;
+    auto stage = [&](int buf, int kt) {
+        char* base = smem + buf * STAGE + wave * 1024;
+#pragma unroll
+        for (int i = 0; i < PER; ++i)
+            __builtin_amdgcn_global_load_lds((const __attribute__((address_space(1))) void*)(src[i] + (size_t)kt * EPB),
+                                             (__attribute__((address_space(3))) void*)(base + i * 4096), 16, 0, 0);
+    };
+
+    f32x4_v acc[MI];
+#pragma unroll
+    for (int mi = 0; mi < MI; ++mi) acc[mi] = f32x4_v{0.f, 0.f, 0.f, 0.f};
+
+    for (int s = 0; s < CR_STAGES - 1 && s < nk; ++s) stage(s, s);
+
+    int cur = 0, nxt = CR_STAGES - 1;
+    for (int kt = 0; kt < nk; ++kt) {
+        cr_wait_ahead<CR_STAGES - 2, PER>(nk - 1 - kt);
+        __builtin_amdgcn_s_barrier();
+        if (kt + CR_STAGES - 1 < nk) stage(nxt, kt + CR_STAGES - 1);
+        const char* base = smem + cur * STAGE;
+#pragma unroll
+        for (int ks = 0; ks < 2; ++ks) {
+            const int coff = ((ks * 4 + fg) ^ sw) << 4;
+            const u32x4_v wf = *reinterpret_cast<const u32x4_v*>(base + w_off + coff);
+#pragma unroll
+            for (int mi = 0; mi < MI; ++mi) {
+                const u32x4_v af = *reinterpret_cast<const u32x4_v*>(base + a_off[mi] + coff);
+                acc[mi] = mfma16<T>(wf, af, acc[mi]);
+            }
+        }
+        asm volatile("s_waitcnt lgkmcnt(0)" ::: "memory");
+        cur = cur + 1 == CR_STAGES ? 0 : cur + 1;
+        nxt = nxt + 1 == CR_STAGES ? 0 : nxt + 1;
+    }
+
+    if (en >= g.N) return;
+    OutT* out = static_cast<OutT*>(g.out);
+#pragma unroll
+    for (int mi = 0; mi < MI; ++mi) {
+        const int m = m0 + wr * 16 * MI + mi * 16 + fr;
+        if (m >= g.M) continue;
+        float v[4] = {acc[mi][0], acc[mi][1], acc[mi][2], acc[mi][3]};
+        if (g.bias) {
+            v[0] += b4.x; v[1] += b4.y; v[2] += b4.z; v[3] += b4.w;
+        }
+#pragma unroll
+        for (int j = 0; j < 4; ++j) v[j] = apply_act<ACT, true>(v[j]);
+        if constexpr (RESID) {
+            v[0] += r4[mi].x; v[1] += r4[mi].y; v[2] += r4[mi].z; v[3] += r4[mi].w;
+        }
+        store4(out + (size_t)m * g.ldo + en, v[0], v[1], v[2], v[3]);
+    }
+}
+
+template <typename T, typename OutT, int ACT, bool RESID, int MI>
+static int launch_instance(const GemmArgs& g, hipStream_t stream) {
+    auto kern = clsrows_kernel<T, OutT, ACT, RESID, MI>;
+    constexpr int lds_bytes = CR_STAGES * cr_stage_bytes(MI);
+    if constexpr (lds_bytes > 64 * 1024) {
+        static bool attr_set[64] = {};
+        int dev = 0;
+        ARP_HIP_OK(hipGetDevice(&dev));
+        if (dev < 0 || dev >= 64 || !attr_set[dev]) {
+            ARP_HIP_OK(hipFuncSetAttribute(reinterpret_cast<const void*>(kern), hipFuncAttributeMaxDynamicSharedMemorySize, lds_bytes));
+            if (dev >= 0 && dev < 64) attr_set[dev] = true;
+        }
+    }
+    constexpr int BM = 32 * MI;
+    const int m_tiles = (g.M + BM - 1) / BM, n_tiles = (g.N + CR_BN - 1) / CR_BN;
+    hipLaunchKernelGGL(kern, dim3(m_tiles * n_tiles), dim3(CR_THREADS), lds_bytes, stream, g);
+    ARP_HIP_OK(hipGetLastError());
+    return 0;
+}
+
+template <typename T, typename OutT, int ACT, bool RESID>
+static int launch_tile(const GemmArgs& g, hipStream_t stream) {
+    const long wg64 = (long)((g.M + 63) / 64) * ((g.N + CR_BN - 1) / CR_BN);
+    return wg64 >= 192 ? launch_instance<T, OutT, ACT, RESID, 2>(g, stream) : launch_instance<T, OutT, ACT, RESID, 1>(g, stream);
+}
+
+#define ARP_CR_COMBOS(X) X(1, ACT_NONE, 1) X(1, ACT_NONE, 0) X(0, ACT_NONE, 0) X(0, ACT_QGELU, 0) X(0, ACT_GELU_TANH, 0)
+
+bool clsrows_has(int tcode, int out_f32, int act, int resid) {
+    if (tcode != 1 && tcode != 2) return false;
+#define X(o, a, r) \
+    if (out_f32 == o && act == a && resid == r) return true;
+    ARP_CR_COMBOS(X)
+#undef X
+    return false;
+}
+
+template <typename T>
+static int dispatch(int out_f32, int act, int resid, const GemmArgs& g, hipStream_t stream) {
+#define X(o, a, r) \
+    if (out_f32 == o && act == a && resid == r) return launch_tile<T, std::conditional_t<o != 0, float, T>, a, r != 0>(g, stream);
+    ARP_CR_COMBOS(X)
+#undef X
+    return fail("clsrows: epilogue not instantiated");
+}
+
+int launch_clsrows_dyn(int tcode, int out_f32, int act, int resid, const GemmArgs& g, hipStream_t stream) {
+    if (!clsrows_supported(g, out_f32 != 0, resid != 0))
+        return fail("clsrows: unsupported geometry M=" + std::to_string(g.M) + " N=" + std::to_string(g.N) + " K=" + std::to_string(g.K));
+    if (resid && !g.resid) return fail("clsrows: the residual epilogue without a residual");
+    if (tcode == 1) return dispatch<bf16_t>(out_f32, act, resid, g, stream);
+    if (tcode == 2) return dispatch<f16_t>(out_f32, act, resid, g, stream);
+    return fail("clsrows: 16-bit operand types only");
+}
+
+}
diff --git a/arp_amd/csrc/rowops.h b/arp_amd/csrc/rowops.h
--- a/arp_amd/csrc/rowops.h
+++ b/arp_amd/csrc/rowops.h
@@ -104,11 +104,12 @@
     return 0;
 }
 
-template <int NV>
+template <int NV, typename HT = void>
 __global__ __launch_bounds__(256) void vit_assemble_lnpre_kernel(const float* __restrict__ patch, const float* __restrict__ cls,
                                                                  const float* __restrict__ pos, const float* __restrict__ w,
                                                                  const float* __restrict__ b, float* __restrict__ x, int rows,
-                                                                 int ntok, int D, float eps) {
+                                                                 int ntok, int D, float eps, HT* __restrict__ h = nullptr,
+                                                                 const float* __restrict__ w1 = nullptr, const float* __restrict__ b1 = nullptr) {
     const int lane = threadIdx.x & 63;
     const int row = blockIdx.x * 4 + (threadIdx.x >> 6);
     if (row >= rows) return;
@@ -127,7 +128,42 @@
             for (int j = 0; j < 4; ++j) v[i][j] += p4[j];
         }
     }
-    ln_row_store<float, NV>(v, D, lane, w, b, eps, x + (size_t)row * D);
+    if constexpr (__is_same(HT, void)) {
+        ln_row_store<float, NV>(v, D, lane, w, b, eps, x + (size_t)row * D);
+    } else {
+        float s = 0.f;
+#pragma unroll
+        for (int i = 0; i < NV; ++i) {
+            const int c = (i * 64 + lane) * 4;
+            if (c < D) s += (v[i][0] + v[i][1]) + (v[i][2] + v[i][3]);
+        }
+        const float mean = wave_sum(s) / (float)D;
+        float q = 0.f;
+#pragma unroll
+        for (int i = 0; i < NV; ++i) {
+            const int c = (i * 64 + lane) * 4;
+            if (c < D) {
+#pragma unroll
+                for (int j = 0; j < 4; ++j) {
+                    const float d = v[i][j] - mean;
+                    q += d * d;
+                }
+            }
+        }
+        const float rstd = 1.0f / sqrtf(wave_sum(q) / (float)D + eps);
+#pragma unroll
+        for (int i = 0; i < NV; ++i) {
+            const int c = (i * 64 + lane) * 4;
+            if (c < D) {
+                const float4 ww = *reinterpret_cast<const float4*>(w + c);
+                const float4 bb = *reinterpret_cast<const float4*>(b + c);
+                v[i][0] = (v[i][0] - mean) * rstd * ww.x + bb.x; v[i][1] = (v[i][1] - mean) * rstd * ww.y + bb.y;
+                v[i][2] = (v[i][2] - mean) * rstd * ww.z + bb.z; v[i][3] = (v[i][3] - mean) * rstd * ww.w + bb.w;
+                store4(x + (size_t)row * D + c, v[i][0], v[i][1], v[i][2], v[i][3]);
+            }
+        }
+        ln_row_store<HT, NV>(v, D, lane, w1, b1, eps, h + (size_t)row * D);
+    }
 }
 
 static int launch_vit_assemble_lnpre(hipStream_t stream, const float* patch, const float* cls, const float* pos, const float* w, const float* b, float* x,
@@ -137,6 +173,19 @@
     hipLaunchKernelGGL((vit_assemble_lnpre_kernel<NV>), dim3((rows + 3) / 4), dim3(256), 0, stream, patch, cls, pos, w, b, x, rows, ntok, D, eps)
     ARP_NV_DISPATCH(D, ARP_ASM_CALL);
 #undef ARP_ASM_CALL
+    ARP_HIP_OK(hipGetLastError());
+    return 0;
+}
+template <typename T>
+static int launch_vit_assemble_lnpre_ln1(hipStream_t stream, const float* patch, const float* cls, const float* pos, const float* w, const float* b, float* x,
+                                         T* h, const float* w1, const float* b1, int rows, int ntok, int D, float eps) {
+    if (D % 4 || D > ROW_MAX_V4 * 256) return fail("vit_assemble_lnpre: unsupported width " + std::to_string(D));
+    if (!h || !w1 || !b1) return fail("vit_assemble_lnpre: the ln_1 tail needs h, w1 and b1");
+#define ARP_ASM1_CALL(NV)                                                                                                                                  \
+    hipLaunchKernelGGL((vit_assemble_lnpre_kernel<NV, T>), dim3((rows + 3) / 4), dim3(256), 0, stream, patch, cls, pos, w, b, x, rows, ntok, D, eps, h, w1, \
+                       b1)
+    ARP_NV_DISPATCH(D, ARP_ASM1_CALL);
+#undef ARP_ASM1_CALL
     ARP_HIP_OK(hipGetLastError());
     return 0;
 }
diff --git a/arp_amd/csrc/tower.h b/arp_amd/csrc/tower.h
--- a/arp_amd/csrc/tower.h
+++ b/arp_amd/csrc/tower.h
@@ -3,6 +3,7 @@
 #include <vector>
 
 #include "attention.h"
+#include "clsrows.h"
 #include "common.h"
 #include "gemm.h"
 #include "gemm256.h"
@@ -117,6 +118,7 @@
     bool cls_only_last = false;
     int attn_impl = 0;
     int gemm_force = 0;
+    bool cls_rows = true;
     bool fp8_mlp = false;
     bool fp8_attn = false;
     bool qkv_fused = true;
@@ -151,6 +153,10 @@
     return launch_rows_gather(c.stream, x, D, c.ms_rows, N, c.ms_out, c.ms_ld, layer * D, B);
 }
 
+template <typename T> static inline bool cls_rows_fit(int M, int N, int K) {
+    return sizeof(T) == 2 && M >= 1 && M <= CR_MAX_M && N >= 16 && (N & 15) == 0 && K >= 64 && (K & 63) == 0;
+}
+
 template <typename T, typename OutT, int ACT, bool RESID, int SITE>
 static int tower_gemm(TowerCtx& c, const char* site, const void* A, const void* W, const float* bias, const float* resid, void* out,
                 int M, int N, int K, const GemmFold* f = nullptr, int lda = 0, int ldr = 0, int ldo = 0) {
@@ -171,6 +177,13 @@
             k.act = ACT; k.out_f32 = sizeof(OutT) == 4;
             return launch_skinny_gemm(__is_same(T, bf16_t) ? 1 : 2, k, c.stream);
         }
+    }
+    if (force == 4) {
+        int rc = 0;
+        if (!f && try_clsrows<T, OutT, ACT, RESID>(g, c.stream, rc)) return rc;
+        return fail(std::string(site) + ": the class-rows kernel was forced outside its domain (M <= " + std::to_string(CR_MAX_M) +
+                    ", N % 16 == 0, K % 64 == 0, 16-bit operands, no fold / side outputs): M=" + std::to_string(M) + " N=" + std::to_string(N) +
+                    " K=" + std::to_string(K));
     }
     if constexpr (SITE == SITE_FC1 && sizeof(T) == 2 && sizeof(OutT) == 2 && ACT == ACT_QGELU && !RESID) {
         if (c.clock_acc && !f && !c.skinny && force != 1 && force != 3 && (long)((M + 255) / 256) * ((N + 255) / 256) >= 192) {
@@ -442,6 +455,7 @@
     const std::string s_red2 = t + ".out_reduce_ln_2", s_red1 = t + ".proj_reduce_ln_1";
     const bool fold = lat && tw.lat_folded && c.lat_stats && c.lat_fold0 && (D & 15) == 0 && skinny_supported(M, D, 4 * D, 4 * D, 4 * D);
     bool h_ready = lat && !fold && c.h_ready0;
+    bool h_ready_tp = !lat && c.h_ready0;
     bool qkv_ready = false;
     for (int i = 0; i < tw.layers; ++i) {
         const LayerW& L = tw.L[i];
@@ -502,17 +516,20 @@
             const std::string s_attn1 = t + ".attn_cls", s_out1 = t + ".out_proj_cls", s_ln21 = t + ".ln_2_cls", s_fc11 = t + ".c_fc_cls",
                               s_fc21 = t + ".c_proj_cls";
             const int ND = N * D;
+            TowerCtx cc = c;
+            if (c.cls_rows && !c.skinny && c.gemm_force == 0 && cls_rows_fit<T>(B, D, D)) cc.gemm_force = 4;
             if (qkv_ready) {
                 ProfScope ps(*c.prof, c.stream, s_attn1.c_str());
                 ARP_TRY(launch_attention<T>(c.stream, c.attn_impl, qkv, ao, B, N, D, tw.heads, causal, 1));
             } else {
-                if (!h_ready) ARP_TRY(tower_layernorm<T>(c, s_ln1.c_str(), x, D, h, D, L.ln1_w, L.ln1_b, M, D, eps));
+                if (!h_ready && !(h_ready_tp && i == 0))
+                    ARP_TRY(tower_layernorm<T>(c, s_ln1.c_str(), x, D, h, D, L.ln1_w, L.ln1_b, M, D, eps));
                 ARP_TRY((tower_qkv_attention<T, SB + SITE_QKV>(c, tw, L, s_qkv.c_str(), s_attn1.c_str(), s_qa1.c_str(), h, qkv, ao, B, N, causal, 1)));
             }
-            ARP_TRY((tower_gemm<T, float, ACT_NONE, true, SB + SITE_OUT>(c, s_out1.c_str(), ao, L.w_out, L.b_out, x, x, B, D, D, nullptr, ND, ND, ND)));
+            ARP_TRY((tower_gemm<T, float, ACT_NONE, true, SB + SITE_OUT>(cc, s_out1.c_str(), ao, L.w_out, L.b_out, x, x, B, D, D, nullptr, ND, ND, ND)));
             ARP_TRY(tower_layernorm<T>(c, s_ln21.c_str(), x, ND, h, D, L.ln2_w, L.ln2_b, B, D, eps));
-            ARP_TRY((tower_gemm<T, T, ACT, false, SB + SITE_FC1>(c, s_fc11.c_str(), h, L.w_fc, L.b_fc, nullptr, fc, B, 4 * D, D)));
-            ARP_TRY((tower_gemm<T, float, ACT_NONE, true, SB + SITE_FC2>(c, s_fc21.c_str(), fc, L.w_proj, L.b_proj, x, x, B, D, 4 * D, nullptr, 0, ND, ND)));
+            ARP_TRY((tower_gemm<T, T, ACT, false, SB + SITE_FC1>(cc, s_fc11.c_str(), h, L.w_fc, L.b_fc, nullptr, fc, B, 4 * D, D)));
+            ARP_TRY((tower_gemm<T, float, ACT_NONE, true, SB + SITE_FC2>(cc, s_fc21.c_str(), fc, L.w_proj, L.b_proj, x, x, B, D, 4 * D, nullptr, 0, ND, ND)));
             ARP_TRY(tower_export_rows(c, x, D, i, B, N));
             break;
         }
@@ -526,7 +543,7 @@
             }
         }
         if (!attn_done) {
-            ARP_TRY(tower_layernorm<T>(c, s_ln1.c_str(), x, D, h, D, L.ln1_w, L.ln1_b, M, D, eps));
+            if (!(h_ready_tp && i == 0)) ARP_TRY(tower_layernorm<T>(c, s_ln1.c_str(), x, D, h, D, L.ln1_w, L.ln1_b, M, D, eps));
             ARP_TRY((tower_qkv_attention<T, SB + SITE_QKV>(c, tw, L, s_qkv.c_str(), s_attn.c_str(), s_qa.c_str(), h, qkv, ao, B, N, causal, 0)));
             ARP_TRY((tower_gemm<T, float, ACT_NONE, true, SB + SITE_OUT>(c, s_out.c_str(), ao, L.w_out, L.b_out, x, x, M, D, D)));
         }
diff --git a/include/arp_hip.h b/include/arp_hip.h
--- a/include/arp_hip.h
+++ b/include/arp_hip.h
@@ -332,6 +332,7 @@
 #define ARP_ASM_LNPRE 0
 #define ARP_ASM_LAT_LN1 1
 #define ARP_ASM_LAT_STATS 2
+#define ARP_ASM_LNPRE_LN1 3
 int arp_op_vit_assemble(int mode, int tail, const float* patch, size_t patch_floats, int S, size_t slice_stride, const float* cls, size_t cls_floats,
                         const float* pos, const float* w, const float* b, const float* w1, const float* b1, void* x, size_t x_bytes, void* h, size_t h_bytes,
                         void* stats, size_t stats_bytes, int B, int ntok, int D, float eps);
```
